# yinjunbo/IS-Fusion

Measured on AMD Instinct MI355X. Metric: nuScenes frames/sec forward (0.075 voxel), LiDAR branch voxelize+spconv->BEV, higher is better.
Workload: dtype f32 (f16x3 split-precision MFMA, fp32 accumulate); 1 GPU; BASELINE configs[1]: isfusion_0075voxel LiDAR-only branch (dynamic voxelize + DynamicVFE + 21-layer SparseEncoder -> BEV [B,512,180,180]), synthetic nuScenes-shaped 300000-pt sweeps, batch=4/GPU, random-init weights, eval BN, fp32; points_per_frame=300000, batch_per_gpu=4, parallelism=dp1, collectives=none (1 rank)

## Files before the change

include/isf_hip.h:

```cpp
#ifndef ISF_HIP_H
#define ISF_HIP_H

#include <stddef.h>
#include <stdint.h>

#ifdef __cplusplus
extern "C" {
#endif

#define ISF_OK 0
#define ISF_ERR_ARG (-1)
#define ISF_ERR_HIP (-2)
#define ISF_ERR_NOMEM (-3)
#define ISF_ERR_UNSUPPORTED (-4)
#define ISF_ERR_CAPACITY (-5)

#define ISF_REDUCE_SUM 0
#define ISF_REDUCE_MEAN 1
#define ISF_REDUCE_MAX 2

#define ISF_CONV_SUBM 0
#define ISF_CONV_SPARSE 1

typedef void* isf_stream_t;
// ... 162 lines not shown
int isf_sparse_conv_forward_dma_lines(const void* features_split, int num_in, int c_in, const void* packed16, int num_taps,
                                      int taps_per_line, int c_out, const int32_t* lines, const uint32_t* mask,
                                      int nbr_stride, int num_out, const float* scale, const float* shift,
                                      const void* residual_split, int relu, void* out_split, int mode,
                                      isf_stream_t stream);
typedef struct isf_conv_cu_plan {
  const int32_t* group_masks;
  const int32_t* units;
  const int32_t* num_units;
  int max_units;
  int num_out;
  int variant;
  int cap;
} isf_conv_cu_plan;
int isf_sparse_conv_cu_plan_ints(int num_out, size_t* num_ints);
int isf_sparse_conv_cu_plan(const int32_t* nbr, int nbr_stride, int num_taps, int num_out, int32_t* plan_buf,
                            isf_conv_cu_plan* plan, isf_stream_t stream);
int isf_sparse_conv_forward_cu(const void* features_split, int num_in, int c_in, const void* packed16, int num_taps,
                               int c_out, const int32_t* nbr, int nbr_stride, int num_out, const float* scale,
                               const float* shift, const void* residual_split, int relu, void* out_split,
                               const isf_conv_cu_plan* plan, isf_stream_t stream);
int isf_sparse_conv_cu_plan_host(const int32_t* work, int num_groups, int cus, int32_t* units, int max_units,
                                 int* num_units);
int isf_sparse_conv_cu_max_units(int num_groups, int cus);
int isf_stage_unit_rows(void);
int isf_stage_unit_cap(void);
int isf_rulebook_stage_tables(const int32_t* nbr, int nbr_stride, int num_taps, uint16_t* slots, int32_t* ulist,
                              int32_t* ucount, isf_stream_t stream);
int isf_sparse_conv_forward_staged(const void* features_split, int num_in, int c_in, const void* packed16,
                                   int num_taps, int c_out, const uint16_t* slots, int nbr_stride,
                                   const int32_t* ulist, const int32_t* ucount, int num_out, const float* scale,
                                   const float* shift, const void* residual_split, int relu, void* out_split,
                                   int stage_rows, int mode, isf_stream_t stream);
int isf_sparse_to_dense_bev(const float* features, const int32_t* indices, int num_rows, int channels,
                            int batch_size, int D, int H, int W, float* out, isf_stream_t stream);

typedef struct isf_conv_layer {
  int conv_type;
  int ksize[3], stride[3], padding[3];
  int c_in, c_out;
  const float* packed;
  const void* packed16;
  const float* scale;
  const float* shift;
  int relu;
  int residual_from;
} isf_conv_layer;

typedef struct isf_encoder_stats {
  int num_layers;
  int num_in[32], num_out[32];
  long long pairs[32];
  float ms[32];
  int precision;
} isf_encoder_stats;

#define ISF_ENC_DIAG_NO_GATHER 2
#define ISF_ENC_DIAG_NO_WEIGHTS 4
#define ISF_ENC_DIAG_NO_LOOP 8
#define ISF_ENC_DIAG_NO_SHARING 16
#define ISF_ENC_DIAG_UNIFORM_TILES 32
#define ISF_ENC_DIAG_LAUNCH_ORDER 64
#define ISF_ENC_DIAG_NARROW_GATHER 128
#define ISF_ENC_DIAG_VFE_FP32_ROWS 256
#define ISF_ENC_DIAG_CU_KERNEL 512
#define ISF_ENC_DIAG_CU_VARIANT_SHIFT 10
#define ISF_ENC_DIAG_CU_VARIANT_MASK 15360
#define ISF_ENC_DIAG_DENSE_TABLES 16384
#define ISF_ENC_DIAG_TILE_TABLES 32768
#define ISF_ENC_DIAG_VOXELIZE_PER_FRAME 65536
#define ISF_ENC_DIAG_COUNTS_MEMCPY 131072
#define ISF_ENC_DIAG_ONE_BLOCK_4W 262144
#define ISF_ENC_DIAG_ONE_BLOCK_8W 524288
#define ISF_ENC_DIAG_STAGGER 1048576
#define ISF_ENC_DIAG_R4_ISSUE 2097152
#define ISF_ENC_DIAG_TWO_AHEAD 4194304
#define ISF_ENC_DIAG_DEEP 8388608
#define ISF_ENC_DIAG_BAND_ORDER 16777216
#define ISF_ENC_DIAG_NO_ROW_SORT 33554432
#define ISF_ENC_DIAG_NARROW_ROW_SORT 67108864
#define ISF_ENC_DIAG_SORT_KEY_AB 134217728
#define ISF_ENC_DIAG_NARROW_TILES 268435456
#define ISF_ENC_DIAG_CHUNK_SPLIT 536870912
typedef struct isf_encoder_options {
  int precision;
  int diagnostic;
  int stage_rows;
  int stage_mask;
  int bev_format;
} isf_encoder_options;

int isf_sparse_encoder_forward(const float* voxel_features, const int32_t* coors, int num_voxels,
                               int batch_size, const int sparse_shape_host[3],
                               const isf_conv_layer* layers_host, int num_layers,
                               float* spatial_features,
                               int out_shape_host[4],
                               isf_encoder_stats* stats_host , int time_layers,
                               const isf_encoder_options* options , isf_stream_t stream);

typedef struct isf_vfe_params {
  int in_channels, c1, c2;
  const float *w1, *scale1, *shift1, *w2, *scale2, *shift2;
  float voxel_size[3], coors_range[6];
} isf_vfe_params;

int isf_lidar_branch_forward(const float* points, const int64_t* point_offsets_host, int batch_size,
                             const isf_vfe_params* vfe_host, const int sparse_shape_host[3],
                             const isf_conv_layer* layers_host, int num_layers,
                             float* spatial_features, int out_shape_host[4],
                             isf_encoder_stats* stats_host, int time_layers,
                             const isf_encoder_options* options , isf_stream_t stream);


size_t isf_packed_linear_bytes(int out_features, int in_features);
int isf_pack_linear(const float* weight, int out_features, int in_features, void* packed, isf_stream_t stream);
int isf_pack_linear_transposed(const float* weight_t, int out_features, int in_features, void* packed, isf_stream_t stream);
int isf_linear_forward(const float* x, int num_rows, int in_features, int ldx, const void* packed_weight,
                       int out_features, const float* bias, const float* row_table, const int32_t* row_table_index,
                       int activation, const float* residual, const float* ln_gamma, const float* ln_beta,
                       float ln_eps, float* y, int ldy, int x_hw, int residual_hw, int y_hw, isf_stream_t stream);

size_t isf_packed_window_block_bytes(int embed_dims);
int isf_pack_window_block(const float* in_proj_weight, const float* out_proj_weight, int embed_dims, int num_heads,
                          void* packed, isf_stream_t stream);
int isf_window_block_forward(const float* x, int batch_size, int grid_size, int embed_dims, int num_heads, int window,
                             int shift, const void* packed, const float* in_proj_bias, const float* pos_table,
                             const float* out_proj_bias, const float* ln_gamma, const float* ln_beta, float ln_eps,
                             float* y, isf_stream_t stream);

int isf_window_attention_forward(const float* qkv, int batch_size, int grid_size, int embed_dims, int num_heads,
                                 int window, int shift, float* out, isf_stream_t stream);

int isf_attention_forward(const float* q, int ldq, const float* k, const float* v, int ldkv, int batch_size,
                          int num_queries, int num_keys, int embed_dims, int num_heads, float* out, int ldo,
                          isf_stream_t stream);
int isf_attention_forward_dropout(const float* q, int ldq, const float* k, const float* v, int ldkv, int batch_size,
                                  int num_queries, int num_keys, int embed_dims, int num_heads, float dropout_p,
                                  unsigned long long seed, float* out, int ldo, isf_stream_t stream);

int isf_channel_attention_forward(const float* query_scene, const float* query_ins, int num_maps, int size,
                                  float* out, isf_stream_t stream);

int isf_p2g_forward(const float* pillars, int pillar_ld, int slots, const int32_t* pillar_coors, int num_pillars,
                    const float* img_nhwc, int batch_size, int num_cam, int feat_h, int feat_w, int channels,
                    const float* cam_params, int input_h, int input_w, int bev_size, float* out,
                    isf_stream_t stream);
int isf_p2g_forward_split(const float* pillars, int pillar_ld, int slots, const int32_t* pillar_coors, int num_pillars,
                          const float* img_nhwc, int batch_size, int num_cam, int feat_h, int feat_w, int channels,
                          const float* cam_params, int input_h, int input_w, int bev_size, void* out_split,
                          isf_stream_t stream);

int isf_instance_topk(const float* heatmap, int batch_size, int num_classes, int height, int width, int k,
                      unsigned pool1_class_mask, int32_t* top_index, int32_t* top_index_raw, float* masked_heatmap,
                      isf_stream_t stream);

int isf_ms_deform_attn_forward(const float* value, const int64_t* spatial_shapes, const int64_t* level_start_index,
                               const float* sampling_loc, const float* attn_weight, int batch_size, int num_keys,
                               int num_heads, int head_dim, int num_queries, int num_levels, int num_points,
                               float* out, isf_stream_t stream);

int isf_ms_deform_attn_backward(const float* value, const int64_t* spatial_shapes, const int64_t* level_start_index,
                                const float* sampling_loc, const float* attn_weight, const float* grad_output,
                                int batch_size, int num_keys, int num_heads, int head_dim, int num_queries,
                                int num_levels, int num_points, float* grad_value, float* grad_sampling_loc,
                                float* grad_attn_weight, isf_stream_t stream);

int isf_ingroup_indices(const int64_t* group_inds, int num, int64_t* out_inds, isf_stream_t stream);

int isf_msda_forward(const float* value, const float* sampling_offsets, const float* attention_logits,
                     const float* reference_points, int batch_size, int num_queries, int num_heads, int head_dim,
                     int num_points, int height, int width, float* out, isf_stream_t stream);

int isf_decode_boxes(const float* heatmap, const float* query_score, const int64_t* query_labels, const float* center,
                     const float* height, const float* dim, const float* rot, const float* vel, int batch_size,
                     int num_classes, int num_proposals, int ld, const float* coder, float* boxes, float* scores,
                     int32_t* labels, int32_t* counts, isf_stream_t stream);

int isf_head_query_init(const int32_t* top_index, const int32_t* top_raw, int batch_size, int num_proposals, int hw,
                        int embed, int num_classes, const float* feat_tok, const int64_t* tok_of_cell,
                        const float* class_table, const float* qpe_table, const float* bev_pos, const float* masked,
                        float* query, float* qpe, float* x, float* query_pos, int64_t* top_index64,
                        int64_t* query_labels, float* query_score, isf_stream_t stream);
int isf_head_scatter_predictions(int num_heads, const float* const* src, const int* src_ld, const int* col0,
                                 const int* channels, float* const* dst, int center_head, const float* query_pos,
                                 float* query_pos_next, int batch_size, int num_proposals, isf_stream_t stream);

int isf_instance_gather(const int32_t* top, int batch_size, int num_instances, int bev_size, int embed,
                        const float* scene, const float* qpe_table, int64_t* top64, int64_t* cell64, float* tokens,
                        float* qpe, float* tokens_pos, float* query_pos, float* ref, isf_stream_t stream);

int isf_transpose_rulebook(const int32_t* nbr, int nbr_stride, int num_out, int num_taps, int num_in,
                           int32_t* nbr_t, int nbr_t_stride, isf_stream_t stream);
int isf_sparse_conv_backward_input(const float* grad_out, int num_out, int c_out, const float* filters, int num_taps,
                                   int c_in, const int32_t* nbr_t, int nbr_t_stride, int num_in, float* grad_in,
// ... 231 lines not shown
```

is-fusion_amd/_lib.py:

```python
import ctypes
import os

_HERE = os.path.dirname(os.path.abspath(__file__))
LIB_PATH = os.path.join(_HERE, "libisf_hip.so")

c_int = ctypes.c_int
c_void_p = ctypes.c_void_p
c_float_p = ctypes.POINTER(ctypes.c_float)
c_int_p = ctypes.POINTER(ctypes.c_int)

ISF_OK = 0
REDUCE = {"sum": 0, "mean": 1, "max": 2}
CONV_SUBM, CONV_SPARSE = 0, 1


class ConvLayer(ctypes.Structure):
    _fields_ = [
        ("conv_type", c_int),
        ("ksize", c_int * 3), ("stride", c_int * 3), ("padding", c_int * 3),
        ("c_in", c_int), ("c_out", c_int),
        ("packed", c_void_p), ("packed16", c_void_p), ("scale", c_void_p), ("shift", c_void_p),
        ("relu", c_int), ("residual_from", c_int),
    ]

# ... 28 lines not shown
    _fields_ = [
        ("in_channels", c_int), ("c1", c_int), ("c2", c_int),
        ("w1", c_void_p), ("scale1", c_void_p), ("shift1", c_void_p),
        ("w2", c_void_p), ("scale2", c_void_p), ("shift2", c_void_p),
        ("voxel_size", ctypes.c_float * 3), ("coors_range", ctypes.c_float * 6),
    ]


class Sweep(ctypes.Structure):
    _fields_ = [
        ("first_point", ctypes.c_int64), ("num_points", ctypes.c_int32), ("sample", ctypes.c_int32),
        ("is_sweep", ctypes.c_int32), ("remove_close", ctypes.c_int32), ("close_radius", ctypes.c_float),
        ("time_lag", ctypes.c_float), ("rotation", ctypes.c_double * 9), ("translation", ctypes.c_double * 3),
    ]


class PointAug(ctypes.Structure):
    _fields_ = [
        ("enabled", ctypes.c_int32), ("rot_mat_T", ctypes.c_float * 9), ("translation", ctypes.c_float * 3),
        ("scale", ctypes.c_float), ("flip_horizontal", ctypes.c_int32), ("flip_vertical", ctypes.c_int32),
    ]


class ImageView(ctypes.Structure):
    _fields_ = [
        ("src_offset", ctypes.c_int64), ("src_w", ctypes.c_int32), ("src_h", ctypes.c_int32),
        ("resize_w", ctypes.c_int32), ("resize_h", ctypes.c_int32), ("crop_x", ctypes.c_int32),
        ("crop_y", ctypes.c_int32), ("flip", ctypes.c_int32), ("rotate", ctypes.c_int32), ("rot", ctypes.c_int32 * 6),
        ("h_bounds", ctypes.c_int32), ("h_coeffs", ctypes.c_int32), ("h_ksize", ctypes.c_int32),
        ("v_bounds", ctypes.c_int32), ("v_coeffs", ctypes.c_int32), ("v_ksize", ctypes.c_int32),
    ]


class PasteView(ctypes.Structure):
    _fields_ = [
        ("src_offset", ctypes.c_int64), ("width", ctypes.c_int32), ("height", ctypes.c_int32),
        ("op_begin", ctypes.c_int32), ("op_end", ctypes.c_int32), ("box_x0", ctypes.c_int32),
        ("box_y0", ctypes.c_int32), ("box_x1", ctypes.c_int32), ("box_y1", ctypes.c_int32),
    ]


class PasteOp(ctypes.Structure):
    _fields_ = [
        ("patch_offset", ctypes.c_int64), ("kind", ctypes.c_int32), ("x0", ctypes.c_int32), ("y0", ctypes.c_int32),
        ("x1", ctypes.c_int32), ("y1", ctypes.c_int32), ("mask_x0", ctypes.c_int32), ("mask_y0", ctypes.c_int32),
        ("mask_x1", ctypes.c_int32), ("mask_y1", ctypes.c_int32), ("patch_pitch", ctypes.c_int32),
    ]


SWEEP_PASTED = 2
PASTE_MIX, PASTE_PATCH = 0, 1
PASTE_MAX_BOXES, PASTE_MAX_OPS = 64, 256


class SwinA(ctypes.Structure):
    _fields_ = [("x", c_void_p), ("x2", c_void_p), ("ln_stats", c_void_p), ("ln_gamma", c_void_p), ("ln_beta", c_void_p),
                ("mode", c_int), ("ldx", c_int), ("n", c_int), ("c", c_int), ("h", c_int), ("w", c_int),
                ("c2", c_int), ("h2", c_int), ("w2", c_int)]


SWIN_A_ROWS, SWIN_A_PATCH, SWIN_A_MERGE, SWIN_A_UPCAT = 0, 1, 2, 3


class AdamWHp(ctypes.Structure):
    _fields_ = [("decay", ctypes.c_float), ("w1", ctypes.c_float), ("b2", ctypes.c_float), ("w2", ctypes.c_float),
                ("eps", ctypes.c_float), ("neg_step_size", ctypes.c_float), ("bc2_sqrt", ctypes.c_float),
                ("pad", ctypes.c_float)]


OPTIM_CHUNK, OPTIM_MAX_HP_ARGS = 32768, 16
OPTIM_NO_CLIP, OPTIM_CLIP, OPTIM_SCALE_GRADS = 0, 1, 2

CONV_MODE_F16, CONV_MODE_NO_GATHER, CONV_MODE_NO_WEIGHTS, CONV_MODE_NO_LOOP, CONV_MODE_NO_SHARING = 1, 2, 4, 8, 16
CONV_MODE_UNIFORM_TILES, CONV_MODE_F16_ROWS, CONV_MODE_F16_STORAGE, CONV_MODE_DMA_PLAN = 32, 256, 257, 2048
CONV_MODE_ONE_BLOCK_4W, CONV_MODE_ONE_BLOCK_8W, CONV_MODE_DEEP, CONV_MODE_STAGGER = 4096, 8192, 32768, 65536
CONV_MODE_R4_ISSUE, CONV_MODE_TWO_AHEAD, CONV_MODE_CHUNK_SPLIT = 131072, 262144, 524288
ENC_DIAG_NO_GATHER, ENC_DIAG_NO_WEIGHTS, ENC_DIAG_NO_LOOP, ENC_DIAG_NO_SHARING, ENC_DIAG_UNIFORM_TILES = 2, 4, 8, 16, 32
ENC_DIAG_LAUNCH_ORDER, ENC_DIAG_NARROW_GATHER, ENC_DIAG_VFE_FP32_ROWS, ENC_DIAG_CU_KERNEL = 64, 128, 256, 512
ENC_DIAG_CU_VARIANT_SHIFT, ENC_DIAG_CU_VARIANT_MASK = 10, 15 << 10
ENC_DIAG_DENSE_TABLES, ENC_DIAG_TILE_TABLES, ENC_DIAG_VOXELIZE_PER_FRAME, ENC_DIAG_COUNTS_MEMCPY = 16384, 32768, 65536, 131072
ENC_DIAG_ONE_BLOCK_4W, ENC_DIAG_ONE_BLOCK_8W, ENC_DIAG_STAGGER, ENC_DIAG_R4_ISSUE = 262144, 524288, 1048576, 2097152
ENC_DIAG_TWO_AHEAD, ENC_DIAG_DEEP, ENC_DIAG_BAND_ORDER, ENC_DIAG_NO_ROW_SORT = 4194304, 8388608, 16777216, 33554432
ENC_DIAG_NARROW_ROW_SORT, ENC_DIAG_SORT_KEY_AB, ENC_DIAG_NARROW_TILES, ENC_DIAG_CHUNK_SPLIT = 67108864, 134217728, 268435456, 536870912
WGRAD_F16, WGRAD_FULL_TAPS = 1, 2


_F3 = ctypes.c_float * 3
_F6 = ctypes.c_float * 6
_I3 = c_int * 3
_I4 = c_int * 4
SIGNATURES = {
    "isf_version": (c_int, []),
    "isf_last_error": (ctypes.c_char_p, []),
    "isf_device_count": (c_int, [c_int_p]),
    "isf_release_workspace": (c_int, []),
    "isf_workspace_bytes": (c_int, [ctypes.POINTER(ctypes.c_size_t)]),
    "isf_debug_workspace_blocks": (c_int, [ctypes.POINTER(ctypes.c_ulonglong), c_int, c_int_p]),
    "isf_dynamic_voxelize": (c_int, [c_void_p, c_int, c_int, _F3, _F6, c_void_p, c_void_p]),
    "isf_dynamic_voxelize_batched": (c_int, [c_void_p, ctypes.POINTER(ctypes.c_int64), c_int, c_int, _F3,
                                             _F6, c_void_p, c_void_p]),
    "isf_hard_voxelize": (c_int, [c_void_p, c_int, c_int, _F3, _F6, c_int, c_int, c_void_p, c_void_p,
                                  c_void_p, c_int_p, c_void_p]),
    "isf_hard_voxelize_device": (c_int, [c_void_p, c_int, c_int, _F3, _F6, c_int, c_int, c_void_p, c_void_p,
                                         c_void_p, c_void_p, c_void_p]),
    "isf_hard_voxelize_batched_device": (c_int, [c_void_p, ctypes.POINTER(ctypes.c_int64), c_int, c_int, _F3, _F6, c_int,
                                                 c_int, c_void_p, c_void_p, c_void_p, c_void_p, c_void_p]),
    "isf_dynamic_point_to_voxel_forward": (c_int, [c_void_p, c_void_p, c_int, c_int, c_int, c_void_p,
                                                   c_void_p, c_void_p, c_void_p, c_int_p, c_void_p]),
    "isf_dynamic_point_to_voxel_backward": (c_int, [c_void_p, c_void_p, c_void_p, c_void_p, c_void_p,
                                                    c_void_p, c_int, c_int, c_int, c_int, c_void_p]),
    "isf_dynamic_vfe_forward": (c_int, [c_void_p, c_void_p, c_int, c_int, c_int, _F3, _F6, c_void_p,
                                        c_void_p, c_void_p, c_int, c_void_p, c_void_p, c_void_p, c_int,
                                        c_void_p, c_void_p, c_void_p, c_int_p, c_void_p]),
    "isf_hard_simple_vfe": (c_int, [c_void_p, c_void_p, c_int, c_int, c_int, c_int, c_void_p, c_void_p]),
    "isf_nbr_stride": (c_int, [c_int]),
    "isf_conv_out_shape": (c_int, [_I3, _I3, _I3, _I3, _I3]),
    "isf_build_rulebook": (c_int, [c_void_p, c_int, c_int, _I3, _I3, _I3, _I3, c_int, c_void_p, c_int,
                                   c_void_p, c_int, c_int_p, c_void_p]),
    "isf_rulebook_to_indice_pairs": (c_int, [c_void_p, c_int, c_int, c_int, c_int, c_void_p, c_void_p,
                                             c_void_p]),
    "isf_indice_pairs_to_rulebook": (c_int, [c_void_p, c_void_p, c_int, c_int, c_int, c_void_p, c_int,
                                             c_void_p]),
    "isf_sparse_conv_forward": (c_int, [c_void_p, c_int, c_int, c_void_p, c_int, c_int, c_void_p, c_int,
                                        c_int, c_void_p, c_void_p, c_void_p, c_int, c_void_p, c_void_p]),
    "isf_packed_filter_elems": (ctypes.c_size_t, [c_int, c_int, c_int]),
    "isf_pack_filters": (c_int, [c_void_p, c_int, c_int, c_int, c_void_p, c_void_p]),
    "isf_sparse_conv_forward_packed": (c_int, [c_void_p, c_int, c_int, c_void_p, c_int, c_int, c_void_p,
                                               c_int, c_int, c_void_p, c_void_p, c_void_p, c_int, c_void_p,
                                               c_void_p]),
    "isf_packed_filter16_bytes": (ctypes.c_size_t, [c_int, c_int, c_int]),
    "isf_pack_filters_f16x3": (c_int, [c_void_p, c_int, c_int, c_int, c_void_p, c_void_p]),
    "isf_pack_filters_f16x3_transposed": (c_int, [c_void_p, c_int, c_int, c_int, c_void_p, c_void_p]),
    "isf_f32_to_split": (c_int, [c_void_p, ctypes.c_size_t, c_void_p, c_void_p]),
    "isf_split_to_f32": (c_int, [c_void_p, ctypes.c_size_t, c_void_p, c_void_p]),
    "isf_f32_to_half": (c_int, [c_void_p, ctypes.c_size_t, c_void_p, c_void_p]),
    "isf_half_to_f32": (c_int, [c_void_p, ctypes.c_size_t, c_void_p, c_void_p]),
    "isf_sparse_conv_forward_f16x3": (c_int, [c_void_p, c_int, c_int, c_void_p, c_int, c_int, c_void_p, c_int,
                                              c_int, c_void_p, c_void_p, c_void_p, c_int, c_void_p, c_int, c_void_p]),
    "isf_sparse_conv_tile_order": (c_int, [c_void_p, c_int, c_int, c_int, c_int, c_int, c_int, c_void_p, c_void_p,
                                           ctypes.POINTER(c_int), c_void_p]),
    "isf_sparse_conv_forward_f16x3_ordered": (c_int, [c_void_p, c_int, c_int, c_void_p, c_int, c_int, c_void_p, c_int,
                                                      c_int, c_void_p, c_void_p, c_void_p, c_int, c_void_p, c_int,
                                                      c_void_p, c_void_p]),
    "isf_sparse_conv_forward_dma": (c_int, [c_void_p, c_int, c_int, c_void_p, c_int, c_int, c_void_p, c_int, c_int,
                                            c_void_p, c_void_p, c_void_p, c_int, c_void_p, c_int, c_void_p, c_void_p]),
    "isf_sparse_conv_tile_table": (c_int, [c_void_p, c_int, c_int, c_int, c_int, c_int, c_int, c_void_p, c_void_p,
                                           ctypes.POINTER(c_int), c_void_p]),
    "isf_sparse_conv_forward_f16x3_tiled": (c_int, [c_void_p, c_int, c_int, c_void_p, c_int, c_int, c_void_p, c_int,
                                                    c_int, c_void_p, c_void_p, c_void_p, c_int, c_void_p, c_int,
                                                    c_void_p, c_void_p]),
    "isf_sparse_conv_tile_table_host": (c_int, [c_void_p, c_int, c_int, c_int, c_int, c_int, c_int, c_void_p,
                                                ctypes.POINTER(c_int)]),
    "isf_sparse_conv_trace": (c_int, [c_void_p, c_int, c_int, c_void_p, c_int, c_int, c_void_p, c_int, c_int, c_void_p,
                                      c_void_p, c_void_p, c_int, c_void_p, c_void_p, c_void_p, c_int,
                                      ctypes.POINTER(c_int), c_void_p]),
    "isf_sparse_conv_phase_trace": (c_int, [c_void_p, c_int, c_int, c_void_p, c_int, c_int, c_void_p, c_int, c_int,
                                            c_void_p, c_void_p, c_void_p, c_int, c_void_p, c_void_p, c_void_p,
                                            ctypes.c_size_t, c_int_p, c_int_p, c_int_p, c_void_p]),
    "isf_rulebook_to_lines": (c_int, [c_void_p, c_int, c_int, c_int, c_int, c_void_p, c_void_p, c_void_p, c_void_p]),
    "isf_lines_to_rulebook": (c_int, [c_void_p, c_void_p, c_int, c_int, c_int, c_void_p, c_void_p]),
    "isf_sparse_conv_forward_dma_lines": (c_int, [c_void_p, c_int, c_int, c_void_p, c_int, c_int, c_int, c_void_p, c_void_p,
                                                  c_int, c_int, c_void_p, c_void_p, c_void_p, c_int, c_void_p, c_int,
                                                  c_void_p]),
    "isf_sparse_conv_cu_plan_ints": (c_int, [c_int, ctypes.POINTER(ctypes.c_size_t)]),
    "isf_sparse_conv_cu_plan": (c_int, [c_void_p, c_int, c_int, c_int, c_void_p, ctypes.POINTER(ConvCuPlan), c_void_p]),
    "isf_sparse_conv_forward_cu": (c_int, [c_void_p, c_int, c_int, c_void_p, c_int, c_int, c_void_p, c_int, c_int,
                                           c_void_p, c_void_p, c_void_p, c_int, c_void_p, ctypes.POINTER(ConvCuPlan),
                                           c_void_p]),
    "isf_sparse_conv_cu_plan_host": (c_int, [c_void_p, c_int, c_int, c_void_p, c_int, ctypes.POINTER(c_int)]),
    "isf_sparse_conv_cu_max_units": (c_int, [c_int, c_int]),
    "isf_stage_unit_rows": (c_int, []),
    "isf_stage_unit_cap": (c_int, []),
    "isf_rulebook_stage_tables": (c_int, [c_void_p, c_int, c_int, c_void_p, c_void_p, c_void_p, c_void_p]),
    "isf_sparse_conv_forward_staged": (c_int, [c_void_p, c_int, c_int, c_void_p, c_int, c_int, c_void_p, c_int,
                                               c_void_p, c_void_p, c_int, c_void_p, c_void_p, c_void_p, c_int, c_void_p,
                                               c_int, c_int, c_void_p]),
    "isf_ms_deform_attn_forward": (c_int, [c_void_p, c_void_p, c_void_p, c_void_p, c_void_p, c_int, c_int, c_int, c_int,
                                           c_int, c_int, c_int, c_void_p, c_void_p]),
    "isf_ms_deform_attn_backward": (c_int, [c_void_p, c_void_p, c_void_p, c_void_p, c_void_p, c_void_p, c_int, c_int,
                                            c_int, c_int, c_int, c_int, c_int, c_void_p, c_void_p, c_void_p, c_void_p]),
    "isf_ingroup_indices": (c_int, [c_void_p, c_int, c_void_p, c_void_p]),
    "isf_packed_window_block_bytes": (ctypes.c_size_t, [c_int]),
    "isf_pack_window_block": (c_int, [c_void_p, c_void_p, c_int, c_int, c_void_p, c_void_p]),
    "isf_window_block_forward": (c_int, [c_void_p, c_int, c_int, c_int, c_int, c_int, c_int, c_void_p, c_void_p,
                                         c_void_p, c_void_p, c_void_p, c_void_p, ctypes.c_float, c_void_p, c_void_p]),
    "isf_p2g_backward": (c_int, [c_void_p, c_int, c_int, c_void_p, c_int, c_int, c_int, c_int, c_int, c_int, c_void_p,
                                 c_int, c_int, c_int, c_void_p, c_void_p, c_void_p]),
    "isf_sparse_to_dense_bev": (c_int, [c_void_p, c_void_p, c_int, c_int, c_int, c_int, c_int, c_int,
                                        c_void_p, c_void_p]),
    "isf_sparse_encoder_forward": (c_int, [c_void_p, c_void_p, c_int, c_int, _I3,
                                           ctypes.POINTER(ConvLayer), c_int, c_void_p, _I4,
                                           ctypes.POINTER(EncoderStats), c_int, ctypes.POINTER(EncoderOptions),
                                           c_void_p]),
    "isf_lidar_branch_forward": (c_int, [c_void_p, ctypes.POINTER(ctypes.c_int64), c_int,
                                         ctypes.POINTER(VfeParams), _I3, ctypes.POINTER(ConvLayer), c_int,
                                         c_void_p, _I4, ctypes.POINTER(EncoderStats), c_int,
                                         ctypes.POINTER(EncoderOptions), c_void_p]),
    "isf_packed_linear_bytes": (ctypes.c_size_t, [c_int, c_int]),
    "isf_pack_linear": (c_int, [c_void_p, c_int, c_int, c_void_p, c_void_p]),
    "isf_pack_linear_transposed": (c_int, [c_void_p, c_int, c_int, c_void_p, c_void_p]),
    "isf_linear_forward": (c_int, [c_void_p, c_int, c_int, c_int, c_void_p, c_int, c_void_p, c_void_p, c_void_p,
                                   c_int, c_void_p, c_void_p, c_void_p, ctypes.c_float, c_void_p, c_int, c_int, c_int,
                                   c_int, c_void_p]),
    "isf_window_attention_forward": (c_int, [c_void_p, c_int, c_int, c_int, c_int, c_int, c_int, c_void_p,
                                             c_void_p]),
    "isf_attention_forward": (c_int, [c_void_p, c_int, c_void_p, c_void_p, c_int, c_int, c_int, c_int, c_int,
                                      c_int, c_void_p, c_int, c_void_p]),
    "isf_attention_forward_dropout": (c_int, [c_void_p, c_int, c_void_p, c_void_p, c_int, c_int, c_int, c_int, c_int,
                                              c_int, ctypes.c_float, ctypes.c_uint64, c_void_p, c_int, c_void_p]),
    "isf_channel_attention_forward": (c_int, [c_void_p, c_void_p, c_int, c_int, c_void_p, c_void_p]),
    "isf_p2g_forward": (c_int, [c_void_p, c_int, c_int, c_void_p, c_int, c_void_p, c_int, c_int, c_int, c_int,
                                c_int, c_void_p, c_int, c_int, c_int, c_void_p, c_void_p]),
    "isf_p2g_forward_split": (c_int, [c_void_p, c_int, c_int, c_void_p, c_int, c_void_p, c_int, c_int, c_int, c_int,
                                      c_int, c_void_p, c_int, c_int, c_int, c_void_p, c_void_p]),
    "isf_instance_topk": (c_int, [c_void_p, c_int, c_int, c_int, c_int, c_int, ctypes.c_uint, c_void_p, c_void_p,
                                  c_void_p, c_void_p]),
    "isf_msda_forward": (c_int, [c_void_p, c_void_p, c_void_p, c_void_p, c_int, c_int, c_int, c_int, c_int,
                                 c_int, c_int, c_void_p, c_void_p]),
    "isf_decode_boxes": (c_int, [c_void_p] * 8 + [c_int, c_int, c_int, c_int, ctypes.POINTER(ctypes.c_float)]
                         + [c_void_p] * 5),
    "isf_sparse_conv_dma_trace": (c_int, [c_void_p, c_int, c_int, c_void_p, c_int, c_int, c_int, c_void_p, c_void_p, c_int,
                                         c_int, c_void_p, c_void_p, c_void_p, c_int, c_void_p, c_void_p, c_int,
                                         ctypes.POINTER(c_int), c_void_p]),
    "isf_sparse_conv_dma_trace_parts": (c_int, [c_void_p, c_int, c_int, c_void_p, c_int, c_int, c_int, c_void_p, c_void_p,
                                               c_int, c_int, c_void_p, c_void_p, c_void_p, c_int, c_void_p, c_void_p,
                                               c_void_p, c_int, ctypes.POINTER(c_int), c_void_p]),
    "isf_sparse_conv_part_table": (c_int, [c_void_p, c_void_p, c_int, c_int, c_int, c_int, c_int, c_int, c_int, c_void_p,
                                           c_int, c_void_p, c_int, c_int * 4, c_void_p]),
    "isf_sparse_conv_forward_parts": (c_int, [c_void_p, c_int, c_int, c_void_p, c_int, c_int, c_int, c_void_p, c_void_p,
                                              c_int, c_int, c_void_p, c_void_p, c_void_p, c_int, c_void_p, c_int, c_void_p,
                                              c_void_p]),
    "isf_instance_gather": (c_int, [c_void_p, c_int, c_int, c_int, c_int] + [c_void_p] * 10),
    "isf_head_query_init": (c_int, [c_void_p, c_void_p, c_int, c_int, c_int, c_int, c_int] + [c_void_p] * 14),
    "isf_head_scatter_predictions": (c_int, [c_int, ctypes.POINTER(c_void_p), ctypes.POINTER(c_int),
                                            ctypes.POINTER(c_int), ctypes.POINTER(c_int), ctypes.POINTER(c_void_p),
                                            c_int, c_void_p, c_void_p, c_int, c_int, c_void_p]),
    "isf_assemble_points": (c_int, [c_void_p, ctypes.POINTER(Sweep), c_int, c_int, ctypes.POINTER(PointAug),
                                    ctypes.POINTER(ctypes.c_float), c_void_p, c_void_p,
                                    ctypes.POINTER(ctypes.c_int32), c_void_p]),
    "isf_image_prepass": (c_int, [c_void_p, c_void_p, c_int, c_void_p, c_void_p, c_int, c_int, c_void_p, c_void_p]),
    "isf_assemble_points_paste": (c_int, [c_void_p, ctypes.POINTER(Sweep), c_int, c_int, ctypes.POINTER(PointAug),
                                          ctypes.POINTER(ctypes.c_float), ctypes.POINTER(ctypes.c_float),
                                          ctypes.POINTER(ctypes.c_int32), c_void_p, c_void_p,
                                          ctypes.POINTER(ctypes.c_int32), c_void_p]),
    "isf_image_paste": (c_int, [c_void_p, c_void_p, c_int, c_void_p, c_int, c_int, c_int, ctypes.c_double,
                                ctypes.c_double, ctypes.c_float, c_void_p]),
    "isf_transpose_rulebook": (c_int, [c_void_p, c_int, c_int, c_int, c_int, c_void_p, c_int, c_void_p]),
    "isf_sparse_conv_backward_input": (c_int, [c_void_p, c_int, c_int, c_void_p, c_int, c_int, c_void_p, c_int, c_int,
                                               c_void_p, c_void_p]),
    "isf_sparse_conv_backward_filter": (c_int, [c_void_p, c_int, c_int, c_void_p, c_int, c_int, c_void_p, c_int,
                                                c_int, c_void_p, c_void_p]),
    "isf_bn1d_stats": (c_int, [c_void_p, c_int, c_int, c_void_p, c_void_p]),
    "isf_bn1d_apply": (c_int, [c_void_p, c_int, c_int, c_void_p, ctypes.c_float, c_void_p, c_void_p, ctypes.c_float,
                               ctypes.c_float, c_int, c_void_p, c_void_p, c_void_p, c_int, c_void_p, c_void_p, c_void_p]),
    "isf_bn1d_stats_pivot": (c_int, [c_void_p, c_int, c_int, c_void_p, c_void_p, c_void_p]),
    "isf_bn1d_apply_pivot": (c_int, [c_void_p, c_int, c_int, c_void_p, c_void_p, ctypes.c_float, c_void_p, c_void_p,
                                     ctypes.c_float, ctypes.c_float, c_int, c_void_p, c_void_p, c_void_p, c_int, c_void_p,
                                     c_void_p, c_void_p]),
    "isf_bn1d_apply_pivot_counted": (c_int, [c_void_p, c_int, c_int, c_void_p, c_void_p, ctypes.c_float, c_void_p, c_void_p,
                                             ctypes.c_float, ctypes.c_float, c_int, c_void_p, c_void_p, c_void_p, c_void_p,
                                             c_int, c_void_p, c_void_p, c_void_p]),
    "isf_bn1d_backward_sums": (c_int, [c_void_p, c_void_p, c_void_p, c_int, c_int, c_void_p, c_void_p, c_void_p]),
    "isf_bn1d_backward_apply": (c_int, [c_void_p, c_void_p, c_void_p, c_int, c_int, c_void_p, c_void_p, c_void_p,
                                        ctypes.c_float, c_void_p, c_void_p, c_void_p, c_void_p, c_void_p]),
    "isf_pair_list_capacity": (c_int, [c_int, c_int]),
    "isf_rulebook_pair_lists": (c_int, [c_void_p, c_int, c_int, c_int, c_int, c_void_p, c_void_p, c_void_p]),
    "isf_grad_to_split": (c_int, [c_void_p, ctypes.c_size_t, c_void_p, c_void_p, c_void_p]),
    "isf_grad_rescale": (c_int, [c_void_p, ctypes.c_size_t, c_void_p, c_void_p, c_void_p]),
    "isf_split_to_f32_scaled": (c_int, [c_void_p, ctypes.c_size_t, c_void_p, c_void_p, c_void_p]),
    "isf_sparse_conv_backward_filter_f16x3": (c_int, [c_void_p, c_int, c_int, c_void_p, c_int, c_int, c_void_p, c_void_p,
                                                      c_int, c_int, c_void_p, c_void_p, c_int, c_void_p]),
    "isf_msda_backward": (c_int, [c_void_p] * 5 + [c_int] * 7 + [c_void_p] * 4),
    "isf_attention_backward": (c_int, [c_void_p, c_int, c_void_p, c_void_p, c_int, c_void_p, c_void_p, c_int, c_int,
                                       c_int, c_int, c_int, c_int, c_void_p, c_int, c_void_p, c_void_p, c_int,
                                       c_void_p]),
    "isf_attention_backward_dropout": (c_int, [c_void_p, c_int, c_void_p, c_void_p, c_int, c_void_p, c_void_p, c_int, c_int,
                                               c_int, c_int, c_int, c_int, ctypes.c_float, ctypes.c_uint64, c_void_p, c_int,
                                               c_void_p, c_void_p, c_int, c_void_p]),
    "isf_window_attention_backward": (c_int, [c_void_p, c_void_p, c_int, c_int, c_int, c_int, c_int, c_int, c_void_p,
                                              c_void_p]),
# ... 121 lines not shown
```

is-fusion_amd/csrc/isf_common.h:

```cpp
#pragma once
#include <hip/hip_runtime.h>
#include <stdint.h>
#include <stdio.h>
#include <stdarg.h>
#include <string.h>
#include <vector>

#include "isf_hip.h"

namespace isf {

void set_error(const char* fmt, ...);

#define ISF_HIP_TRY(expr)                                                                   \
  do {                                                                                      \
    hipError_t _e = (expr);                                                                 \
    if (_e != hipSuccess) {                                                                 \
      ::isf::set_error("%s:%d: %s -> %s", __FILE__, __LINE__, #expr, hipGetErrorString(_e)); \
      return ISF_ERR_HIP;                                                                   \
    }                                                                                       \
  } while (0)

#define ISF_REQUIRE(cond, code, ...)  \
  do {                                \
    if (!(cond)) {                    \
      ::isf::set_error(__VA_ARGS__);  \
      return (code);                  \
    }                                 \
  } while (0)

#define ISF_TRY(expr)          \
  do {                         \
    int _r = (expr);           \
    if (_r != ISF_OK) return _r; \
  } while (0)

#define ISF_LAUNCH_CHECK() ISF_HIP_TRY(hipGetLastError())

struct ByteMaps {
  unsigned char* fine = nullptr;
  unsigned char* coarse = nullptr;
  size_t words = 0;
};

class Arena {
 public:
  int reset();
  int alloc(void** out, size_t bytes);
  template <typename T>
  int alloc_n(T** out, size_t n) { return alloc(reinterpret_cast<void**>(out), n * sizeof(T)); }
  int release();
  size_t capacity() const;
  int list_blocks(unsigned long long* base_cap, int max_pairs, int* num_pairs) const;
  hipStream_t side = nullptr;
  std::vector<hipEvent_t> events;
  size_t next_event = 0;
  ByteMaps bytemaps;
  int* mailbox_host = nullptr;
  int* mailbox_dev = nullptr;
  unsigned mailbox_seq = 0;
  int* zero_pool = nullptr;
  float* ks_scratch = nullptr;
  size_t ks_scratch_bytes = 0;
  unsigned* ks_count = nullptr;
  int ks_count_cap = 0;
 private:
  struct Block { char* base; size_t cap; size_t off; };
  std::vector<Block> blocks_;
};

Arena& arena_for_stream(hipStream_t st);

static inline hipStream_t as_stream(isf_stream_t s) { return reinterpret_cast<hipStream_t>(s); }
static inline int ceil_div(long long a, long long b) { return (int)((a + b - 1) / b); }
static inline size_t round_up(size_t a, size_t b) { return (a + b - 1) / b * b; }

struct OccIndex {
  int B, D, H, W;
  unsigned long long ncells;
  size_t nwords;
  unsigned long long* bits;
  uint32_t* prefix;
  int* total;
};

int occ_create(Arena& a, OccIndex* occ, int B, int D, int H, int W, hipStream_t st, bool zero = true);
size_t occ_bits_bytes(const OccIndex& occ);
int occ_mark_coords4_bytemap(Arena& a, const OccIndex& occ, const int32_t* coors4, int n, hipStream_t st);
int scan_u32_exclusive(Arena& a, const uint32_t* in, uint32_t* out, size_t n, hipStream_t st);
int occ_scan(Arena& a, const OccIndex& occ, hipStream_t st);
int occ_mark_coords4(const OccIndex& occ, const int32_t* coors4, int n, hipStream_t st);
int occ_compact_coords4(const OccIndex& occ, int32_t* out, hipStream_t st);
int fill_many(hipStream_t st, int n, void* const* ptrs, const size_t* bytes, const unsigned char* byte_values);
int read_int(const int* dev, int* host, hipStream_t st);
int post_int(Arena& a, const int* dev, hipStream_t st, unsigned* ticket);
int wait_int(Arena& a, unsigned ticket, hipStream_t st, int* value);
int side_stream(Arena& a, hipStream_t* out);
static constexpr int kZeroInts = 256;
int zero_ints(Arena& a, int** out);
int ksplit_buffers(Arena& a, size_t scratch_bytes, int counters, float** scratch, unsigned** count, hipStream_t st);
int stream_wait_stream(Arena& a, hipStream_t waiter, hipStream_t producer);
int pooled_event(Arena& a, hipEvent_t* out);

__device__ __forceinline__ int occ_lookup(const unsigned long long* __restrict__ bits,
                                          const uint32_t* __restrict__ prefix,
                                          unsigned long long cell) {
  const size_t w = (size_t)(cell >> 6);
  const unsigned long long word = bits[w];
  const unsigned long long bit = 1ull << (cell & 63);
  if (!(word & bit)) return -1;
  return (int)(prefix[w] + (uint32_t)__popcll(word & (bit - 1)));
}

struct AttnDrop {
  unsigned long long seed;
  unsigned thresh;
  float inv_keep;
};
__host__ __device__ inline bool attn_keep(unsigned long long seed, unsigned bh, unsigned i, unsigned j, unsigned thresh) {
  unsigned long long x = seed ^ (((unsigned long long)bh << 48) | ((unsigned long long)(i & 0xffffffu) << 24) |
                                 (unsigned long long)(j & 0xffffffu));
  x ^= x >> 33;
  x *= 0xff51afd7ed558ccdULL;
  x ^= x >> 33;
  x *= 0xc4ceb9fe1a85ec53ULL;
  x ^= x >> 33;
  return (unsigned)(x >> 32) >= thresh;
}
static inline AttnDrop attn_drop_of(float p, unsigned long long seed) {
  AttnDrop d{seed, 0u, 1.f};
  if (p > 0.f) {
    const double t = (double)p * 4294967296.0;
    d.thresh = t >= 4294967295.0 ? 4294967295u : (unsigned)t;
    d.inv_keep = 1.f / (1.f - p);
  }
  return d;
}

__host__ __device__ inline size_t split_hi_index(size_t row, int c_units, int u) {
  return (row * (size_t)c_units + (size_t)(u & ~3)) * 2 + (size_t)(u & 3);
}

__device__ __forceinline__ bool voxel_of_point(const float* __restrict__ p, float vx, float vy, float vz,
                                               float x0, float y0, float z0, int gx, int gy, int gz,
                                               int& cx, int& cy, int& cz) {
  const float fx = floorf(__fdiv_rn(__fsub_rn(p[0], x0), vx));
  const float fy = floorf(__fdiv_rn(__fsub_rn(p[1], y0), vy));
  const float fz = floorf(__fdiv_rn(__fsub_rn(p[2], z0), vz));
  if (!(fx >= 0.f && fx < (float)gx && fy >= 0.f && fy < (float)gy && fz >= 0.f && fz < (float)gz))
    return false;
  cx = (int)fx; cy = (int)fy; cz = (int)fz;
  return true;
}

struct VoxGeom {
  float vx, vy, vz, x0, y0, z0;
  int gx, gy, gz;
};

static inline VoxGeom make_geom(const float vs[3], const float range[6]) {
  VoxGeom g;
  g.vx = vs[0]; g.vy = vs[1]; g.vz = vs[2];
  g.x0 = range[0]; g.y0 = range[1]; g.z0 = range[2];
  g.gx = (int)roundf((range[3] - range[0]) / vs[0]);
  g.gy = (int)roundf((range[4] - range[1]) / vs[1]);
  g.gz = (int)roundf((range[5] - range[2]) / vs[2]);
  return g;
}


static constexpr int kVoxMaxBatch = 8;
struct VoxBatch {
  long long off[kVoxMaxBatch + 1];
  int B;
};
int occ_voxelize_mark_bytemap(Arena& a, const OccIndex& occ, const float* points, int P, int C, const VoxGeom& g,
                              const VoxBatch& vb, int32_t* coors4, hipStream_t st);

int dynamic_voxelize_impl(const float* points, int P, int C, const float vs[3], const float range[6],
                          int32_t* coors, int coors_stride, int coors_col0, int batch_idx,
                          hipStream_t st);
int dynamic_vfe_impl(Arena& a, const float* points, const int32_t* coors4, int P, int Cin, int B,
                     const float vs[3], const float range[6], const float* w1, const float* scale1,
                     const float* shift1, int c1, const float* w2, const float* scale2,
                     const float* shift2, int c2, float* voxel_feats, int32_t* voxel_coors,
                     int32_t* pt2vox, int* num_voxels_host, OccIndex* occ_out, int grid_d_alloc,
                     hipStream_t st, hipEvent_t* coords_ready = nullptr,
                     void* voxel_feats_split = nullptr ,
                     const VoxBatch* voxelize = nullptr );
int build_perm(Arena& a, const OccIndex& occ, const int32_t* coors4, int n, int32_t** perm_out,
               hipStream_t st);
int launch_nbr(Arena& a, const int32_t* out_coors4, int n_out, const int in_shape[3], const int ks[3],
               const int st[3], const int pd[3], bool subm, const OccIndex& in_occ, const int32_t* perm,
               int32_t* nbr, int nbr_stride, unsigned long long* pair_count, hipStream_t st_);
int launch_nbr_lines(Arena& a, const int32_t* out_coors4, int n_out, const int in_shape[3], const int ks[3],
                     const int st[3], const int pd[3], bool subm, const OccIndex& in_occ, int32_t* lines, uint32_t* mask,
                     int stride, unsigned long long* pair_count, hipStream_t st_);
int launch_mark_out(const int32_t* in_coors4, int n_in, const int in_shape[3], const int ks[3],
                    const int st[3], const int pd[3], const OccIndex& out_occ, hipStream_t st_);
bool sparse_conv_mfma_supported(int c_in, int c_out);
int pack_filters_impl(const float* w, int K, int cin, int cout, float* packed, hipStream_t st);
int sparse_conv_forward_packed_impl(const float* x, int n_in, int c_in, const float* packed, int K,
                                    int c_out, const int32_t* nbr, int nbr_stride, int n_out,
                                    const float* scale, const float* shift, const float* residual,
                                    int relu, float* y, hipStream_t st);
int sparse_conv_forward_generic_impl(const float* x, int c_in, const float* w, int K, int c_out,
                                     const int32_t* nbr, int nbr_stride, int n_out, const float* scale,
                                     const float* shift, const float* residual, int relu, float* y,
                                     hipStream_t st);
bool sparse_conv_f16x3_supported(int c_in, int c_out);
int sparse_conv_forward_f16x3_impl(const void* xs, int c_in, const void* packed16, int K, int c_out,
                                   const int32_t* nbr, int nbr_stride, int n_out, const float* scale,
                                   const float* shift, const void* residual, int relu, void* ys,
                                   int mode , hipStream_t st,
                                   const int32_t* order = nullptr, struct Conv16LaunchInfo* query = nullptr,
                                   const int32_t* rowmap = nullptr );
struct Conv16LaunchInfo {
  int full, half, part_rows;
  int TM, ncb, wgs_per_cu, cus_per_xcd;
};
static inline int conv16_order_parts(const Conv16LaunchInfo& i) { return i.ncb == 2 ? 4 : 8; }
static inline int conv16_order_tiles(const Conv16LaunchInfo& i) { return i.full + i.half; }
static inline bool conv16_order_applies(const Conv16LaunchInfo& i) {
  const int t = i.full + i.half;
  return t > i.cus_per_xcd && t <= i.wgs_per_cu * i.cus_per_xcd && t <= 255 && i.cus_per_xcd <= 64;
}
static inline bool conv16_table_applies(const Conv16LaunchInfo& i) {
  return i.TM > 0 && i.cus_per_xcd > 0 && i.part_rows / 16 <= i.cus_per_xcd * i.wgs_per_cu * (i.TM / 16);
}
static inline int conv16_table_ints(const Conv16LaunchInfo& i) {
  return conv16_order_parts(i) * 2 * i.wgs_per_cu * i.cus_per_xcd;
}
int conv16_tile_table_impl(const int32_t* group_work, int n_out, const Conv16LaunchInfo& info, int32_t* table,
                           hipStream_t st);
int conv_group_masks_impl(const int32_t* nbr, int nbr_stride, int K, int n_out, int32_t* masks, int32_t* work,
                          hipStream_t st);
bool sparse_conv_dma_supported(int c_in, int c_out);
int sparse_conv_forward_dma_impl(const void* xs, int c_in, const void* packed16, int K, int c_out, const int32_t* nbr,
                                 int nbr_stride, int n_out, const float* scale, const float* shift,
                                 const void* residual, int relu, void* ys, int mode, hipStream_t st,
                                 const int32_t* order = nullptr, Conv16LaunchInfo* query = nullptr,
                                 const uint32_t* lmask = nullptr , int nx = 0,
                                 const int32_t* rowmap = nullptr ,
                                 long long* trace = nullptr );
int conv16_tile_order_impl(const int32_t* nbr, int nbr_stride, int K, int n_out, const Conv16LaunchInfo& info,
                           int32_t* work , int32_t* order ,
                           hipStream_t st, const uint32_t* lmask = nullptr );
bool conv16_parts_apply(const Conv16LaunchInfo& info, bool several_rounds = false);
int conv16_part_table_impl(const int32_t* nbr, const uint32_t* lmask, int nbr_stride, int K, int n_out, int c_in, int c_out,
                           const Conv16LaunchInfo& info, bool raster, int32_t* work, int32_t* table, hipStream_t st,
                           bool equal_rows = false );
int stable_sort_u32_impl(Arena& a, const uint32_t* keys, int n, int key_bits, int* idx_sorted, hipStream_t st);
int conv_row_sort_impl(Arena& a, const int32_t* nbr, int nbr_stride, int K, int n_out, int part_rows, int32_t* rowmap,
                       int32_t* nbr_sorted, hipStream_t st,
                       int key_mode = 1 );
int conv_row_sort_lines_impl(Arena& a, const int32_t* lines, const uint32_t* lmask, int nbr_stride, int num_lines, int n_out,
                             int part_rows, bool full_key, int32_t* rowmap, int32_t* lines_sorted, uint32_t* lmask_sorted,
                             hipStream_t st);
bool conv16_band_order_applies(const Conv16LaunchInfo& info);
int conv16_band_order_impl(const int32_t* coors4, int n_out, const Conv16LaunchInfo& info, int band, int32_t* order ,
                           hipStream_t st);
bool sparse_conv_deep_supported(int c_in, int c_out);
int sparse_conv_forward_deep_impl(bool balance, bool table, const uint4* xs, int c_in, const uint4* wpk, const float* winv,
                                  int K, int c_out, const int32_t* nbr, int nbr_stride, int n_out, const float* scale,
                                  const float* shift, const uint4* residual, int relu, uint4* ys, hipStream_t st,
                                  const int32_t* order, Conv16LaunchInfo* query);
struct ConvCuPlan {
  const int32_t* group_masks = nullptr;
  const int2* units = nullptr;
  const int32_t* num_units = nullptr;
  int max_units = 0;
  int n_out = 0;
  int variant = 0;
  int cap = 16;
};
int conv_cu_variant_cap(int variant);
bool sparse_conv_cu_supported(int c_in, int c_out);
size_t conv_cu_plan_ints(int n_out);
int conv_cu_plan_impl(const int32_t* nbr, int nbr_stride, int K, int n_out, int32_t* buf ,
                      ConvCuPlan* plan, hipStream_t st, int cap = 16);
int sparse_conv_forward_cu_impl(const void* xs, int c_in, const void* packed16, int K, int c_out, const int32_t* nbr,
                                int nbr_stride, int n_out, const float* scale, const float* shift, const void* residual,
                                int relu, void* ys, const ConvCuPlan& plan, hipStream_t st);
int stage_tables_impl(const int32_t* nbr, int nbr_stride, int K, uint16_t* slots, int32_t* ulist, int32_t* ucount,
                      hipStream_t st);
int sparse_conv_forward_staged_impl(const void* xs, int c_in, const void* packed16, int K, int c_out,
                                    const uint16_t* slots, int nbr_stride, const int32_t* ulist,
                                    const int32_t* ucount, int n_out, const float* scale, const float* shift,
                                    const void* residual, int relu, void* ys, int stage_rows, int mode,
                                    hipStream_t st);
int pack_filters16_impl(Arena& a, const float* w, int K, int cin, int cout, void* packed16, hipStream_t st,
                        bool transposed = false );
int f32_to_split_impl(const float* x, size_t n_elems, void* xs, hipStream_t st);
int split_to_f32_impl(const void* xs, size_t n_elems, float* x, hipStream_t st);
int f32_to_half_impl(const float* x, size_t n_elems, void* xh, hipStream_t st);
int half_to_f32_impl(const void* xh, size_t n_elems, float* x, hipStream_t st);
int sparse_to_dense_bev_impl(Arena& a, const void* feats, int fmt, const int32_t* indices, int n, int C,
                             int B, int D, int H, int W, float* out, const OccIndex* occ,
                             hipStream_t st);

}
```

is-fusion_amd/csrc/isf_encoder.hip:

```cpp
#include "isf_common.h"
#include "isf_spconv16.h"

#include <algorithm>

namespace isf {

static constexpr int kDenseX = 64;

template <int FMT>
__global__ __launch_bounds__(256) void dense_bev_kernel(const void* __restrict__ feats_v, int C, int D,
                                                        int H, int W,
                                                        const unsigned long long* __restrict__ bits,
                                                        const uint32_t* __restrict__ prefix,
                                                        const int32_t* __restrict__ perm,
                                                        float* __restrict__ out) {
  __shared__ float tile[64][kDenseX + 1];
  __shared__ int rows[kDenseX];
  const int xt = blockIdx.x, y = blockIdx.y, b = blockIdx.z;
  const int x0 = xt * kDenseX;
  const int t = threadIdx.x;
  for (int z = 0; z < D; ++z) {
    __syncthreads();
    if (t < kDenseX) {
      int r = -1;
      const int x = x0 + t;
      if (x < W) {
        r = occ_lookup(bits, prefix, (((unsigned long long)b * D + z) * H + y) * W + x);
        if (r >= 0 && perm) r = perm[r];
      }
      rows[t] = r;
    }
    __syncthreads();
    for (int c0 = 0; c0 < C; c0 += 64) {
      if (FMT != 0) {
        const uint4* fs = reinterpret_cast<const uint4*>(feats_v);
        const int u = t & 7;
#pragma unroll
        for (int j = 0; j < 2; ++j) {
          const int xx = (t >> 3) + 32 * j;
          const int r = rows[xx];
          float v[8] = {0.f, 0.f, 0.f, 0.f, 0.f, 0.f, 0.f, 0.f};
          if (r >= 0 && c0 + u * 8 < C) {
            const size_t o = FMT == 2 ? (size_t)r * (C >> 3) + (c0 >> 3) + u : split_hi_index((size_t)r, C >> 3, (c0 >> 3) + u);
            const uint4 hi = fs[o], lo = FMT == 2 ? make_uint4(0, 0, 0, 0) : fs[o + 4];
            const _Float16* h = reinterpret_cast<const _Float16*>(&hi);
            const _Float16* l = reinterpret_cast<const _Float16*>(&lo);
#pragma unroll
            for (int q = 0; q < 8; ++q) v[q] = (float)h[q] + (float)l[q];
          }
#pragma unroll
          for (int q = 0; q < 8; ++q) tile[u * 8 + q][xx] = v[q];
        }
      } else {
        const float* feats = reinterpret_cast<const float*>(feats_v);
        const int c4 = (t & 15) * 4;
#pragma unroll
        for (int j = 0; j < 4; ++j) {
          const int xx = (t >> 4) + 16 * j;
          const int r = rows[xx];
          float4 v = make_float4(0.f, 0.f, 0.f, 0.f);
          if (r >= 0 && c0 + c4 < C) v = *reinterpret_cast<const float4*>(feats + (size_t)r * C + c0 + c4);
          tile[c4 + 0][xx] = v.x;
          tile[c4 + 1][xx] = v.y;
          tile[c4 + 2][xx] = v.z;
          tile[c4 + 3][xx] = v.w;
        }
      }
      __syncthreads();
      const int lane = t & 63, wv = t >> 6;
      if (x0 + lane < W) {
        for (int cc = wv; cc < 64 && c0 + cc < C; cc += 4) {
          const size_t ch = (size_t)(c0 + cc) * D + z;
          out[(((size_t)b * C * D + ch) * H + y) * W + x0 + lane] = tile[cc][lane];
        }
      }
      __syncthreads();
    }
  }
}

int sparse_to_dense_bev_impl(Arena& a, const void* feats, int fmt, const int32_t* indices, int n, int C,
                             int B, int D, int H, int W, float* out, const OccIndex* occ_in, hipStream_t st) {
  ISF_REQUIRE(C % (fmt ? 32 : 4) == 0, ISF_ERR_UNSUPPORTED, "dense: channels %d not a multiple of %d", C,
              fmt ? 32 : 4);
  OccIndex occ;
  const int32_t* perm = nullptr;
  if (occ_in) {
    occ = *occ_in;
  } else {
    ISF_TRY(occ_create(a, &occ, B, D, H, W, st));
    ISF_TRY(occ_mark_coords4(occ, indices, n, st));
    ISF_TRY(occ_scan(a, occ, st));
    int32_t* p = nullptr;
    ISF_TRY(build_perm(a, occ, indices, n, &p, st));
    perm = p;
  }
  dim3 grid(ceil_div(W, kDenseX), H, B);
  if (fmt == 1)
    hipLaunchKernelGGL(dense_bev_kernel<1>, grid, dim3(256), 0, st, feats, C, D, H, W, occ.bits, occ.prefix,
                       perm, out);
  else if (fmt == 2)
    hipLaunchKernelGGL(dense_bev_kernel<2>, grid, dim3(256), 0, st, feats, C, D, H, W, occ.bits, occ.prefix,
                       perm, out);
  else
    hipLaunchKernelGGL(dense_bev_kernel<0>, grid, dim3(256), 0, st, feats, C, D, H, W, occ.bits, occ.prefix,
                       perm, out);
  ISF_LAUNCH_CHECK();
  return ISF_OK;
}

__global__ __launch_bounds__(256) void bev_split_kernel(const uint4* __restrict__ fs, int C, int D, int H, int W,
                                                        const unsigned long long* __restrict__ bits,
                                                        const uint32_t* __restrict__ prefix, long long ntok,
                                                        uint4* __restrict__ out) {
  const int upt = C * D / 8;
  const long long t = (long long)blockIdx.x * 256 + threadIdx.x;
  if (t >= ntok * upt) return;
  const long long tok = t / upt;
  const int j = (int)(t - tok * upt);
  const int hw = H * W;
  const int b = (int)(tok / hw), pos = (int)(tok - (long long)b * hw);
  const int y = pos / W, x = pos - y * W;
  _Float16 hi[8], lo[8];
  if (D == 2) {
    const int r0 = occ_lookup(bits, prefix, (((unsigned long long)b * 2 + 0) * H + y) * W + x);
    const int r1 = occ_lookup(bits, prefix, (((unsigned long long)b * 2 + 1) * H + y) * W + x);
    uint2 h0 = make_uint2(0, 0), l0 = h0, h1 = h0, l1 = h0;
    const int uc = j >> 1, e = j & 1;
    if (r0 >= 0) {
      const uint2* p = reinterpret_cast<const uint2*>(fs + split_hi_index((size_t)r0, C >> 3, uc));
      h0 = p[e];
      l0 = p[8 + e];
    }
    if (r1 >= 0) {
      const uint2* p = reinterpret_cast<const uint2*>(fs + split_hi_index((size_t)r1, C >> 3, uc));
      h1 = p[e];
      l1 = p[8 + e];
    }
    const _Float16 *a0 = reinterpret_cast<const _Float16*>(&h0), *a1 = reinterpret_cast<const _Float16*>(&h1);
    const _Float16 *b0 = reinterpret_cast<const _Float16*>(&l0), *b1 = reinterpret_cast<const _Float16*>(&l1);
#pragma unroll
    for (int q = 0; q < 4; ++q) {
      hi[2 * q] = a0[q]; hi[2 * q + 1] = a1[q];
      lo[2 * q] = b0[q]; lo[2 * q + 1] = b1[q];
    }
  } else {
    for (int q = 0; q < 8; ++q) {
      const int ch = 8 * j + q, c = ch / D, z = ch - c * D;
      const int r = occ_lookup(bits, prefix, (((unsigned long long)b * D + z) * H + y) * W + x);
      hi[q] = lo[q] = (_Float16)0.f;
      if (r >= 0) {
        const _Float16* p = reinterpret_cast<const _Float16*>(fs + split_hi_index((size_t)r, C >> 3, c >> 3));
        hi[q] = p[c & 7];
        lo[q] = p[32 + (c & 7)];
      }
    }
  }
  const int g = j >> 5, ju = j & 31;
  uint4* o = out + (size_t)g * ntok * 64 + split_hi_index((size_t)tok, 32, ju);
  o[0] = *reinterpret_cast<const uint4*>(hi);
  o[4] = *reinterpret_cast<const uint4*>(lo);
}

int sparse_to_bev_split_impl(const void* feats_split, int C, int B, int D, int H, int W, const OccIndex& occ, void* out,
                             hipStream_t st) {
  ISF_REQUIRE(C % 32 == 0 && (C * D) % 256 == 0, ISF_ERR_UNSUPPORTED,
              "bev (split token matrices): %d x %d channels are not whole 256-channel groups", C, D);
  const long long ntok = (long long)B * H * W, total = ntok * (C * D / 8);
  hipLaunchKernelGGL(bev_split_kernel, dim3(ceil_div(total, 256)), dim3(256), 0, st, reinterpret_cast<const uint4*>(feats_split),
                     C, D, H, W, occ.bits, occ.prefix, ntok, reinterpret_cast<uint4*>(out));
  ISF_LAUNCH_CHECK();
  return ISF_OK;
}

__global__ void check_rank_order_kernel(const int32_t* __restrict__ coors4, int n, int B, int D, int H, int W,
                                        const unsigned long long* __restrict__ bits,
                                        const uint32_t* __restrict__ prefix, int* __restrict__ flag) {
  const int i = blockIdx.x * blockDim.x + threadIdx.x;
  if (i >= n) return;
  const int4 c = reinterpret_cast<const int4*>(coors4)[i];
  int r = -1;
// ... 69 lines not shown
      ISF_TRY(a.alloc_n(&work, (size_t)2 * T));
      ISF_TRY(a.alloc_n(&table, (size_t)conv16_part_table_ints(parts, conv16_parts_cap(T, parts))));
      ISF_TRY(conv16_part_table_impl(nbr, lmask, stride, K, n_out, ly.c_in, ly.c_out, info, !order_ok, work, table, sg,
                                     (mode & ISF_CONV_MODE_UNIFORM_TILES) != 0));
      *order = table;
      *kind = kOrderParts;
      return ISF_OK;
    }
  }
  if (!order_ok) return ISF_OK;
  if (dma)
    ISF_TRY(sparse_conv_forward_dma_impl(nullptr, ly.c_in, ly.packed16, K, ly.c_out, nbr, stride, n_out, nullptr,
                                         nullptr, nullptr, 0, nullptr, mode, sg, nullptr, &info));
  else
    ISF_TRY(sparse_conv_forward_f16x3_impl(nullptr, ly.c_in, ly.packed16, K, ly.c_out, nbr, stride, n_out, nullptr,
                                           nullptr, nullptr, 0, nullptr, mode, sg, nullptr, &info));
  if (!dma && kind && tables && !lmask && conv16_table_applies(info) && n_out >= 16 * info.cus_per_xcd) {
    const int ng = ceil_div(n_out, 16);
    int32_t *masks = nullptr, *work = nullptr, *table = nullptr;
    ISF_TRY(a.alloc_n(&masks, (size_t)ng));
    ISF_TRY(a.alloc_n(&work, (size_t)ng));
    ISF_TRY(a.alloc_n(&table, (size_t)conv16_table_ints(info)));
    ISF_TRY(conv_group_masks_impl(nbr, stride, K, n_out, masks, work, sg));
    ISF_TRY(conv16_tile_table_impl(work, n_out, info, table, sg));
    *order = table;
    *kind = kOrderTable;
    return ISF_OK;
  }
  if (!conv16_order_applies(info)) {
    if (band > 0 && coors_out && conv16_band_order_applies(info)) {
      int32_t* ord = nullptr;
      ISF_TRY(a.alloc_n(&ord, (size_t)conv16_order_parts(info) * conv16_order_tiles(info)));
      ISF_TRY(conv16_band_order_impl(coors_out, n_out, info, band, ord, sg));
      *order = ord;
    }
    return ISF_OK;
  }
  const size_t n = (size_t)conv16_order_parts(info) * conv16_order_tiles(info);
  int32_t *work = nullptr, *ord = nullptr;
  ISF_TRY(a.alloc_n(&work, n));
  ISF_TRY(a.alloc_n(&ord, n));
  ISF_TRY(conv16_tile_order_impl(nbr, stride, K, n_out, info, work, ord, sg, lmask));
  *order = ord;
  return ISF_OK;
}

static int build_stage_tables(Arena& a, const int32_t* nbr, int stride, int K, StageTables* t, hipStream_t sg) {
  const int units = stride / isf_stage_unit_rows();
  ISF_TRY(a.alloc_n(&t->slots, (size_t)K * stride));
  ISF_TRY(a.alloc_n(&t->ulist, (size_t)units * isf_stage_unit_cap()));
  ISF_TRY(a.alloc_n(&t->ucount, (size_t)units));
  return stage_tables_impl(nbr, stride, K, t->slots, t->ulist, t->ucount, sg);
}

static int default_stage_rows(const isf_conv_layer& ly) {
  (void)ly;
  return 0;
}

static int ensure_occ(Arena& a, LevelState& L, int B, hipStream_t st) {
  if (L.has_occ) return ISF_OK;
  ISF_TRY(occ_create(a, &L.occ, B, L.shape[0], L.shape[1], L.shape[2], st));
  ISF_TRY(occ_mark_coords4(L.occ, L.coors, L.n, st));
  ISF_TRY(occ_scan(a, L.occ, st));
  L.has_occ = true;
  return ISF_OK;
}

static constexpr int kKnockoutBits = ISF_ENC_DIAG_NO_GATHER | ISF_ENC_DIAG_NO_WEIGHTS | ISF_ENC_DIAG_NO_LOOP | ISF_ENC_DIAG_NO_SHARING;
static constexpr int kDeepOptBits = ISF_CONV_MODE_STAGGER | ISF_CONV_MODE_R4_ISSUE | ISF_CONV_MODE_TWO_AHEAD | ISF_CONV_MODE_DEEP | kConvModeNarrowTiles;
static constexpr struct { int diag, mode; } kDiagToConvMode[] = {
    {ISF_ENC_DIAG_NO_GATHER, ISF_CONV_MODE_NO_GATHER},       {ISF_ENC_DIAG_NO_WEIGHTS, ISF_CONV_MODE_NO_WEIGHTS},
    {ISF_ENC_DIAG_NO_LOOP, ISF_CONV_MODE_NO_LOOP},           {ISF_ENC_DIAG_NO_SHARING, ISF_CONV_MODE_NO_SHARING},
    {ISF_ENC_DIAG_UNIFORM_TILES, ISF_CONV_MODE_UNIFORM_TILES}, {ISF_ENC_DIAG_CHUNK_SPLIT, ISF_CONV_MODE_CHUNK_SPLIT},
    {ISF_ENC_DIAG_ONE_BLOCK_4W, ISF_CONV_MODE_ONE_BLOCK_4W}, {ISF_ENC_DIAG_ONE_BLOCK_8W, ISF_CONV_MODE_ONE_BLOCK_8W},
    {ISF_ENC_DIAG_STAGGER, ISF_CONV_MODE_STAGGER},           {ISF_ENC_DIAG_R4_ISSUE, ISF_CONV_MODE_R4_ISSUE},
    {ISF_ENC_DIAG_TWO_AHEAD, ISF_CONV_MODE_TWO_AHEAD},       {ISF_ENC_DIAG_DEEP, ISF_CONV_MODE_DEEP},
    {ISF_ENC_DIAG_NARROW_TILES, kConvModeNarrowTiles}};
static constexpr int kEncDiagKnown =
    kKnockoutBits | ISF_ENC_DIAG_UNIFORM_TILES | ISF_ENC_DIAG_CHUNK_SPLIT | ISF_ENC_DIAG_ONE_BLOCK_4W | ISF_ENC_DIAG_ONE_BLOCK_8W |
    ISF_ENC_DIAG_STAGGER | ISF_ENC_DIAG_R4_ISSUE | ISF_ENC_DIAG_TWO_AHEAD | ISF_ENC_DIAG_DEEP | ISF_ENC_DIAG_NARROW_TILES |
    ISF_ENC_DIAG_LAUNCH_ORDER | ISF_ENC_DIAG_NARROW_GATHER | ISF_ENC_DIAG_CU_KERNEL | ISF_ENC_DIAG_CU_VARIANT_MASK |
    ISF_ENC_DIAG_DENSE_TABLES | ISF_ENC_DIAG_TILE_TABLES | ISF_ENC_DIAG_COUNTS_MEMCPY | ISF_ENC_DIAG_BAND_ORDER | ISF_ENC_DIAG_NO_ROW_SORT |
    ISF_ENC_DIAG_NARROW_ROW_SORT | ISF_ENC_DIAG_SORT_KEY_AB | ISF_ENC_DIAG_VFE_FP32_ROWS | ISF_ENC_DIAG_VOXELIZE_PER_FRAME;

int sparse_encoder_forward_impl(Arena& a, const float* x0, const int32_t* coors0, int n0, int B,
                                const int shape0[3], const OccIndex* occ0, const isf_conv_layer* layers,
                                int num_layers, float* spatial_features, int out_shape[4],
                                isf_encoder_stats* stats, int time_layers, const isf_encoder_options* opt,
                                hipStream_t st, hipEvent_t geometry_ready = nullptr,
                                const void* x0_split = nullptr ) {
  const int precision = opt ? opt->precision : 0, diagnostic = opt ? opt->diagnostic : 0;
  const int dg = diagnostic & kKnockoutBits;
  ISF_REQUIRE(precision >= 0 && precision <= 2 && diagnostic >= 0 && (diagnostic & ~kEncDiagKnown) == 0 &&
                  (dg == 0 || conv_mode_is_knockout(dg) || dg == ISF_ENC_DIAG_NO_SHARING) && !(precision == 2 && dg != 0),
              ISF_ERR_ARG, "sparse_encoder: options (precision %d, diagnostic %d)", precision, diagnostic);
  int translated = 0;
  for (const auto& t : kDiagToConvMode)
    if (diagnostic & t.diag) translated |= t.mode;
  const bool f16io = precision == 2;
  const bool fp32_class = dg == 0 && !f16io;
  const int conv_mode = (f16io ? ISF_CONV_MODE_F16_STORAGE : dg) | (translated & ISF_CONV_MODE_UNIFORM_TILES);
  const int one_block = translated & (ISF_CONV_MODE_ONE_BLOCK_4W | ISF_CONV_MODE_ONE_BLOCK_8W);
  const int deep_opts = translated & kDeepOptBits;
  const bool chunk_split = (translated & ISF_CONV_MODE_CHUNK_SPLIT) && fp32_class && one_block == 0 && deep_opts == 0;
  auto on = [&](int bit) { return (diagnostic & bit) != 0; };
  const bool tile_order = !on(ISF_ENC_DIAG_LAUNCH_ORDER), dma_gather = !on(ISF_ENC_DIAG_NARROW_GATHER);
  const bool line_tables = !on(ISF_ENC_DIAG_DENSE_TABLES), mailbox = !on(ISF_ENC_DIAG_COUNTS_MEMCPY), row_sort = !on(ISF_ENC_DIAG_NO_ROW_SORT);
  const bool tile_tables = on(ISF_ENC_DIAG_TILE_TABLES), band_order = on(ISF_ENC_DIAG_BAND_ORDER);
  const bool narrow_sort = on(ISF_ENC_DIAG_NARROW_ROW_SORT), cu_units = on(ISF_ENC_DIAG_CU_KERNEL);
  const int sort_key = on(ISF_ENC_DIAG_SORT_KEY_AB) ? 2 : 1;
  const int cu_variant = (diagnostic & ISF_ENC_DIAG_CU_VARIANT_MASK) >> ISF_ENC_DIAG_CU_VARIANT_SHIFT;
  auto band_of = [&](const int shape[3]) -> int { return band_order ? std::max(8, shape[1] / 45) : 0; };
  constexpr int sort_min_rows = 4096;
  const int cu_cap = conv_cu_variant_cap(cu_variant);
  const int stage_opt = opt ? opt->stage_rows : 0;
  const unsigned stage_mask = opt ? (unsigned)opt->stage_mask : 0u;
  ISF_REQUIRE(stage_opt >= -1, ISF_ERR_ARG, "sparse_encoder: stage_rows %d", stage_opt);
  ISF_REQUIRE(num_layers > 0 && num_layers <= 32, ISF_ERR_ARG, "sparse_encoder: %d layers (1..32)", num_layers);
  hipStream_t sg = nullptr;
  ISF_TRY(side_stream(a, &sg));
  if (geometry_ready) ISF_HIP_TRY(hipStreamWaitEvent(sg, geometry_ready, 0));
  else ISF_TRY(stream_wait_stream(a, sg, st));
  LevelState L;
  for (int j = 0; j < 3; ++j) L.shape[j] = shape0[j];
  L.n = n0;
  L.coors = coors0;
  L.has_occ = false;
  if (occ0) { L.occ = *occ0; L.has_occ = true; }
  L.cache_nbr = nullptr;
  L.cache_order = nullptr;
  L.cache_order_cin = L.cache_order_cout = 0;
  L.cache_order_kind = kOrderPerm;
  L.cache_cu = ConvCuPlan();
  L.cache_lmask = nullptr;
  L.cache_rowmap = L.cache_nbr_sorted = nullptr;
  L.cache_lmask_sorted = nullptr;
  L.cache_sort_part_rows = 0;
  bool use16 = precision != 1;
  for (int i = 0; i < num_layers; ++i)
    use16 = use16 && layers[i].packed16 && sparse_conv_f16x3_supported(layers[i].c_in, layers[i].c_out);
  const void* outputs[32];
  int out_rows[32];
  const void* x = x0;
  const void* x_in0 = x0;
  ISF_REQUIRE(!x0_split || (use16 && !f16io), ISF_ERR_ARG, "sparse_encoder: split input without the split kernels");
  if (x0_split) {
    x = x0_split;
    x_in0 = x0_split;
  } else if (use16) {
    void* xs0 = nullptr;
    ISF_TRY(a.alloc(&xs0, (size_t)std::max(n0, 1) * layers[0].c_in * 4));
    if (f16io) ISF_TRY(f32_to_half_impl(x0, (size_t)n0 * layers[0].c_in, xs0, st));
    else ISF_TRY(f32_to_split_impl(x0, (size_t)n0 * layers[0].c_in, xs0, st));
    x = xs0;
    x_in0 = xs0;
  }
  unsigned long long* pair_counts = nullptr;
  if (stats) {
    ISF_TRY(a.alloc_n(&pair_counts, 32));
    ISF_HIP_TRY(hipMemsetAsync(pair_counts, 0, 32 * sizeof(unsigned long long), sg));
  }
  std::vector<hipEvent_t> ev;
  if (time_layers && stats) {
    ev.resize((size_t)num_layers * 2);
    for (auto& e : ev) ISF_HIP_TRY(hipEventCreate(&e));
  }
  int c_last = layers[0].c_in;
  for (int i = 0; i < num_layers; ++i) {
    const isf_conv_layer& ly = layers[i];
    const int K = ly.ksize[0] * ly.ksize[1] * ly.ksize[2];
    ISF_REQUIRE(K >= 1 && K <= 27, ISF_ERR_UNSUPPORTED, "sparse_encoder: layer %d has %d taps", i, K);
    ISF_REQUIRE(ly.c_in == c_last, ISF_ERR_ARG, "sparse_encoder: layer %d expects %d channels, got %d", i, ly.c_in, c_last);
    int32_t* nbr = nullptr;
    int stride = 0;
    int n_out = L.n;
    int n_in = L.n;
    int srows = 0;
    if (use16 && dg == 0 && !f16io && stage_opt >= 0 && sparse_conv_f16x3_supported(ly.c_in, ly.c_out))
      srows = stage_opt == 0 ? default_stage_rows(ly)
                             : ((stage_mask == 0 || ((stage_mask >> i) & 1u)) ? stage_opt : 0);
    StageTables stg;
    const int32_t* order = nullptr;
    int order_kind = kOrderPerm;
    const bool cu = use16 && cu_units && srows == 0 && conv_mode == 0 && sparse_conv_cu_supported(ly.c_in, ly.c_out);
    ConvCuPlan cu_plan;
    const bool plan_ok = use16 && srows == 0 && !cu;
    const bool want_tile_order = plan_ok && tile_order;
    const int layer_mode = conv_mode | (fp32_class && ly.c_out >= 128 ? deep_opts : 0) |
                           (chunk_split && use16 && !cu && srows == 0 && ly.c_out == 256 && ly.c_in >= 128 ? ISF_CONV_MODE_CHUNK_SPLIT : 0);
    const bool dma = use16 && dma_gather && srows == 0 && dg == 0 && sparse_conv_dma_supported(ly.c_in, ly.c_out);
    const bool parts_ok = plan_ok && dg == 0 && !((conv_mode & ISF_CONV_MODE_UNIFORM_TILES) && !tile_order) && !band_order && !(dma && narrow_sort) &&
                          (dma || (layer_mode & (ISF_CONV_MODE_DEEP | ISF_CONV_MODE_CHUNK_SPLIT)) == 0);
    const bool want_order = want_tile_order || parts_ok;
    const uint32_t* lmask = nullptr;
    const int nx = ly.ksize[2];
    auto lines_ok = [&](int first) -> bool {
      if (!use16 || !dma_gather || !line_tables || dg != 0 || stage_opt > 0 || (nx != 1 && nx != 3) ||
          ly.ksize[0] * ly.ksize[1] > 9)
        return false;
      for (int j = first; j < num_layers; ++j) {
        const isf_conv_layer& q = layers[j];
        if (q.conv_type != ISF_CONV_SUBM) break;
        if (q.ksize[0] != ly.ksize[0] || q.ksize[1] != ly.ksize[1] || q.ksize[2] != ly.ksize[2]) continue;
        if (!sparse_conv_dma_supported(q.c_in, q.c_out)) return false;
      }
      return true;
    };
    const bool sort_mode_ok = dg == 0 && one_block == 0 && (deep_opts & ~kConvModeNarrowTiles) == 0;
    const bool sort_ok = row_sort && use16 && !cu && srows == 0 && ly.conv_type == ISF_CONV_SUBM && K == 27 &&
                         sort_mode_ok && L.n >= sort_min_rows && (dma ? narrow_sort : ly.c_out >= 128);
    const int32_t* rowmap = nullptr;
    auto launch_info = [&](const int32_t* table, int tstride, int rows, Conv16LaunchInfo* info) -> int {
      if (dma)
        return sparse_conv_forward_dma_impl(nullptr, ly.c_in, ly.packed16, K, ly.c_out, table, tstride, rows, nullptr, nullptr,
                                            nullptr, 0, nullptr, conv_mode, sg, nullptr, info);
      return sparse_conv_forward_f16x3_impl(nullptr, ly.c_in, ly.packed16, K, ly.c_out, table, tstride, rows, nullptr, nullptr,
                                            nullptr, 0, nullptr, layer_mode, sg, nullptr, info);
    };
    auto ensure_row_sort = [&](const int32_t* table, int tstride, int rows, bool* built) -> int {
      *built = false;
      if (!sort_ok || L.cache_rowmap) return ISF_OK;
      Conv16LaunchInfo info;
      ISF_TRY(launch_info(table, tstride, rows, &info));
// ... 95 lines not shown
          ISF_TRY(build_cu_plan(a, nbr, stride, K, n_out, &L.cache_cu, sg, cu_cap));
          ISF_TRY(stream_wait_stream(a, st, sg));
        }
      }
      cu_plan = L.cache_cu;
      lmask = L.cache_lmask;
      if (sort_applies(nbr, stride, n_out)) {
        nbr = const_cast<int32_t*>(L.cache_nbr_sorted);
        if (lmask) lmask = L.cache_lmask_sorted;
        rowmap = L.cache_rowmap;
      }
      ISF_REQUIRE(!lmask || dma, ISF_ERR_UNSUPPORTED, "sparse_encoder: layer %d cannot read a line-compressed table", i);
      stg = L.cache_stage;
      if (want_order) {
        order = L.cache_order;
        order_kind = L.cache_order_kind;
      }
      if (stats) stats->pairs[i] = hit ? L.cache_pairs : -(long long)i - 1;
    } else {
      ISF_TRY(ensure_occ(a, L, B, sg));
      LevelState Nx;
      ISF_TRY(isf_conv_out_shape(L.shape, ly.ksize, ly.stride, ly.padding, Nx.shape));
      ISF_REQUIRE(Nx.shape[0] > 0 && Nx.shape[1] > 0 && Nx.shape[2] > 0, ISF_ERR_ARG,
                  "sparse_encoder: layer %d output shape empty", i);
      ISF_TRY(occ_create(a, &Nx.occ, B, Nx.shape[0], Nx.shape[1], Nx.shape[2], sg));
      ISF_TRY(launch_mark_out(L.coors, L.n, L.shape, ly.ksize, ly.stride, ly.padding, Nx.occ, sg));
      ISF_TRY(occ_scan(a, Nx.occ, sg));
      if (mailbox) {
        unsigned ticket = 0;
        ISF_TRY(post_int(a, Nx.occ.total, sg, &ticket));
        ISF_TRY(wait_int(a, ticket, sg, &Nx.n));
      } else {
        ISF_TRY(read_int(Nx.occ.total, &Nx.n, sg));
      }
      Nx.has_occ = true;
      int32_t* nc = nullptr;
      ISF_TRY(a.alloc_n(&nc, (size_t)std::max(Nx.n, 1) * 4));
      if (Nx.n > 0) ISF_TRY(occ_compact_coords4(Nx.occ, nc, sg));
      Nx.coors = nc;
      stride = isf_nbr_stride(Nx.n);
      if (dma && lines_ok(num_layers)) {
        uint32_t* lm = nullptr;
        ISF_TRY(a.alloc_n(&nbr, (size_t)ly.ksize[0] * ly.ksize[1] * stride));
        ISF_TRY(a.alloc_n(&lm, (size_t)stride));
        ISF_TRY(launch_nbr_lines(a, Nx.coors, Nx.n, L.shape, ly.ksize, ly.stride, ly.padding, false, L.occ, nbr, lm, stride,
                                 stats ? pair_counts + i : nullptr, sg));
        lmask = lm;
      } else {
        ISF_TRY(a.alloc_n(&nbr, (size_t)K * stride));
        ISF_TRY(launch_nbr(a, Nx.coors, Nx.n, L.shape, ly.ksize, ly.stride, ly.padding, false, L.occ, nullptr, nbr,
                           stride, stats ? pair_counts + i : nullptr, sg));
      }
      if (srows > 0) ISF_TRY(build_stage_tables(a, nbr, stride, K, &stg, sg));
      if (row_sort && use16 && !dma && !cu && srows == 0 && !lmask && ly.c_out >= 128 && K == 27 && sort_mode_ok &&
          Nx.n >= sort_min_rows) {
        Conv16LaunchInfo info;
        ISF_TRY(sparse_conv_forward_f16x3_impl(nullptr, ly.c_in, ly.packed16, K, ly.c_out, nbr, stride, Nx.n, nullptr, nullptr,
                                               nullptr, 0, nullptr, layer_mode, sg, nullptr, &info));
        int32_t *rm = nullptr, *ns = nullptr;
        ISF_TRY(a.alloc_n(&rm, (size_t)stride));
        ISF_TRY(a.alloc_n(&ns, (size_t)K * stride));
        ISF_TRY(conv_row_sort_impl(a, nbr, stride, K, Nx.n, info.part_rows, rm, ns, sg, 1));
        nbr = ns;
        rowmap = rm;
      }
      if (want_order)
        ISF_TRY(build_tile_order(a, ly, K, nbr, stride, Nx.n, layer_mode, dma, &order, sg, lmask, &order_kind, tile_tables,
                                 Nx.coors, band_of(Nx.shape), tile_order, parts_ok));
      if (cu && Nx.n > 0) ISF_TRY(build_cu_plan(a, nbr, stride, K, Nx.n, &cu_plan, sg, cu_cap));
      if (stats) stats->pairs[i] = -(long long)i - 1;
      Nx.cache_cu = ConvCuPlan();
      Nx.cache_lmask = nullptr;
      Nx.cache_rowmap = Nx.cache_nbr_sorted = nullptr;
      Nx.cache_lmask_sorted = nullptr;
      Nx.cache_sort_part_rows = 0;
      Nx.cache_nbr = nullptr;
      Nx.cache_order = nullptr;
      Nx.cache_order_cin = Nx.cache_order_cout = 0;
      Nx.cache_order_kind = kOrderPerm;
      n_out = Nx.n;
      L = Nx;
      ISF_TRY(stream_wait_stream(a, st, sg));
    }
    void* y = nullptr;
    ISF_TRY(a.alloc(&y, (size_t)std::max(n_out, 1) * ly.c_out * 4));
    const void* res = nullptr;
    if (ly.residual_from == -1) res = x_in0;
    else if (ly.residual_from >= 0) {
      ISF_REQUIRE(ly.residual_from < i && out_rows[ly.residual_from] == n_out, ISF_ERR_ARG,
                  "sparse_encoder: layer %d residual source %d incompatible", i, ly.residual_from);
      res = outputs[ly.residual_from];
    }
    if (!ev.empty()) ISF_HIP_TRY(hipEventRecord(ev[2 * i], st));
    if (use16 && srows > 0)
      ISF_TRY(sparse_conv_forward_staged_impl(x, ly.c_in, ly.packed16, K, ly.c_out, stg.slots, stride, stg.ulist,
                                              stg.ucount, n_out, ly.scale, ly.shift, res, ly.relu, y, srows, conv_mode,
                                              st));
    else if (cu && n_out > 0 && ((cu_plan.variant = cu_variant), true))
      ISF_TRY(sparse_conv_forward_cu_impl(x, ly.c_in, ly.packed16, K, ly.c_out, nbr, stride, n_out, ly.scale, ly.shift, res,
                                          ly.relu, y, cu_plan, st));
    else if (dma)
      ISF_TRY(sparse_conv_forward_dma_impl(x, ly.c_in, ly.packed16, K, ly.c_out, nbr, stride, n_out, ly.scale, ly.shift,
                                           res, ly.relu, y, conv_mode | order_mode_bit(order_kind), st, order, nullptr, lmask,
                                           nx, rowmap));
    else if (use16)
      ISF_TRY(sparse_conv_forward_f16x3_impl(x, ly.c_in, ly.packed16, K, ly.c_out, nbr, stride, n_out, ly.scale,
                                             ly.shift, res, ly.relu, y,
                                             layer_mode | order_mode_bit(order_kind) |
                                                 (ly.c_out == 256 && fp32_class ? one_block : 0),
                                             st, order, nullptr, rowmap));
    else if (sparse_conv_mfma_supported(ly.c_in, ly.c_out))
      ISF_TRY(sparse_conv_forward_packed_impl(reinterpret_cast<const float*>(x), n_in, ly.c_in, ly.packed, K,
                                              ly.c_out, nbr, stride, n_out, ly.scale, ly.shift,
                                              reinterpret_cast<const float*>(res), ly.relu,
                                              reinterpret_cast<float*>(y), st));
    else
      ISF_TRY(sparse_conv_forward_generic_impl(reinterpret_cast<const float*>(x), ly.c_in, ly.packed, K, ly.c_out,
                                               nbr, stride, n_out, ly.scale, ly.shift,
                                               reinterpret_cast<const float*>(res), ly.relu,
                                               reinterpret_cast<float*>(y), st));
    if (!ev.empty()) ISF_HIP_TRY(hipEventRecord(ev[2 * i + 1], st));
    outputs[i] = y;
    out_rows[i] = n_out;
    if (stats) { stats->num_in[i] = n_in; stats->num_out[i] = n_out; stats->ms[i] = 0.f; }
    x = y;
    c_last = ly.c_out;
  }
  ISF_TRY(ensure_occ(a, L, B, sg));
  ISF_TRY(stream_wait_stream(a, st, sg));
  if (opt && opt->bev_format == 1) {
    ISF_REQUIRE(use16 && !f16io, ISF_ERR_UNSUPPORTED, "sparse_encoder: bev_format 1 needs the split-precision path");
    ISF_TRY(sparse_to_bev_split_impl(x, c_last, B, L.shape[0], L.shape[1], L.shape[2], L.occ, spatial_features, st));
  } else {
    ISF_REQUIRE(!opt || opt->bev_format == 0, ISF_ERR_ARG, "sparse_encoder: bev_format %d (0 fp32 map, 1 split token matrices)",
                opt->bev_format);
    ISF_TRY(sparse_to_dense_bev_impl(a, x, use16 ? (f16io ? 2 : 1) : 0, L.coors, L.n, c_last, B, L.shape[0], L.shape[1],
                                     L.shape[2], spatial_features, &L.occ, st));
  }
  if (stats) stats->precision = use16 ? 1 : 0;
  if (out_shape) { out_shape[0] = c_last * L.shape[0]; out_shape[1] = L.shape[1]; out_shape[2] = L.shape[2]; out_shape[3] = L.n; }
  if (stats) {
    unsigned long long h_pairs[32];
    ISF_HIP_TRY(hipMemcpyAsync(h_pairs, pair_counts, sizeof(h_pairs), hipMemcpyDeviceToHost, st));
    ISF_HIP_TRY(hipStreamSynchronize(st));
    stats->num_layers = num_layers;
    for (int i = 0; i < num_layers; ++i)
      if (stats->pairs[i] < 0) stats->pairs[i] = (long long)h_pairs[-(stats->pairs[i] + 1)];
    for (int i = 0; i < num_layers && !ev.empty(); ++i)
      ISF_HIP_TRY(hipEventElapsedTime(&stats->ms[i], ev[2 * i], ev[2 * i + 1]));
  }
  for (auto& e : ev) (void)hipEventDestroy(e);
  return ISF_OK;
}

}

extern "C" {

int isf_sparse_to_dense_bev(const float* features, const int32_t* indices, int num_rows, int channels,
                            int batch_size, int D, int H, int W, float* out, isf_stream_t stream) {
  ISF_REQUIRE(num_rows >= 0 && channels > 0 && batch_size > 0 && D > 0 && H > 0 && W > 0 && out, ISF_ERR_ARG,
              "sparse_to_dense_bev: bad arguments");
  ISF_REQUIRE(num_rows == 0 || (features && indices), ISF_ERR_ARG, "sparse_to_dense_bev: null pointer");
  isf::Arena& a = isf::arena_for_stream(isf::as_stream(stream));
  ISF_TRY(a.reset());
  return isf::sparse_to_dense_bev_impl(a, features, 0, indices, num_rows, channels, batch_size, D, H, W, out,
                                       nullptr, isf::as_stream(stream));
}

int isf_sparse_encoder_forward(const float* voxel_features, const int32_t* coors, int num_voxels,
                               int batch_size, const int sparse_shape_host[3],
                               const isf_conv_layer* layers_host, int num_layers, float* spatial_features,
                               int out_shape_host[4], isf_encoder_stats* stats_host, int time_layers,
                               const isf_encoder_options* options, isf_stream_t stream) {
  using namespace isf;
  ISF_REQUIRE(num_voxels > 0 && batch_size > 0 && sparse_shape_host && layers_host && spatial_features &&
                  voxel_features && coors && num_layers > 0,
              ISF_ERR_ARG, "sparse_encoder_forward: bad arguments");
  hipStream_t st = as_stream(stream);
  Arena& a = arena_for_stream(as_stream(stream));
  ISF_TRY(a.reset());
  OccIndex occ0;
  ISF_TRY(occ_create(a, &occ0, batch_size, sparse_shape_host[0], sparse_shape_host[1], sparse_shape_host[2], st));
  ISF_TRY(occ_mark_coords4(occ0, coors, num_voxels, st));
  ISF_TRY(occ_scan(a, occ0, st));
  int* flag = nullptr;
  ISF_TRY(a.alloc_n(&flag, 64));
  ISF_HIP_TRY(hipMemsetAsync(flag, 0, sizeof(int), st));
  hipLaunchKernelGGL(check_rank_order_kernel, dim3(ceil_div(num_voxels, 256)), dim3(256), 0, st, coors,
                     num_voxels, occ0.B, occ0.D, occ0.H, occ0.W, occ0.bits, occ0.prefix, flag);
  ISF_LAUNCH_CHECK();
  int h[2] = {0, 0};
  ISF_HIP_TRY(hipMemcpyAsync(&h[0], flag, sizeof(int), hipMemcpyDeviceToHost, st));
  ISF_HIP_TRY(hipMemcpyAsync(&h[1], occ0.total, sizeof(int), hipMemcpyDeviceToHost, st));
  ISF_HIP_TRY(hipStreamSynchronize(st));
  const float* x = voxel_features;
  const int32_t* c = coors;
  int n = num_voxels;
  if (h[0] != 0 || h[1] != num_voxels) {
    n = h[1];
    ISF_REQUIRE(n > 0, ISF_ERR_ARG, "sparse_encoder_forward: no coordinate inside sparse_shape");
    int32_t* perm = nullptr;
    ISF_TRY(build_perm(a, occ0, coors, num_voxels, &perm, st));
    int32_t* cs = nullptr;
    float* xs = nullptr;
    const int C = layers_host[0].c_in;
    ISF_TRY(a.alloc_n(&cs, (size_t)n * 4));
    ISF_TRY(a.alloc_n(&xs, (size_t)n * C));
    ISF_TRY(occ_compact_coords4(occ0, cs, st));
    hipLaunchKernelGGL(gather_rows_kernel, dim3(ceil_div((long long)n * C, 256)), dim3(256), 0, st,
                       voxel_features, perm, n, C, xs);
    ISF_LAUNCH_CHECK();
    x = xs;
    c = cs;
  }
  return sparse_encoder_forward_impl(a, x, c, n, batch_size, sparse_shape_host, &occ0, layers_host, num_layers,
                                     spatial_features, out_shape_host, stats_host, time_layers, options, st);
}

static bool encoder_takes_split_input(const isf_conv_layer* layers, int num_layers, const isf_encoder_options* opt) {
  if ((opt ? opt->precision : 0) != 0 || num_layers <= 0 || num_layers > 32) return false;
  for (int i = 0; i < num_layers; ++i)
    if (!layers[i].packed16 || !isf::sparse_conv_f16x3_supported(layers[i].c_in, layers[i].c_out)) return false;
  return true;
}

int isf_lidar_branch_forward(const float* points, const int64_t* point_offsets_host, int batch_size,
                             const isf_vfe_params* vfe_host, const int sparse_shape_host[3],
                             const isf_conv_layer* layers_host, int num_layers, float* spatial_features,
                             int out_shape_host[4], isf_encoder_stats* stats_host, int time_layers,
                             const isf_encoder_options* options, isf_stream_t stream) {
  using namespace isf;
  ISF_REQUIRE(points && point_offsets_host && batch_size > 0 && vfe_host && sparse_shape_host && layers_host &&
                  spatial_features,
              ISF_ERR_ARG, "lidar_branch_forward: bad arguments");
  hipStream_t st = as_stream(stream);
  Arena& a = arena_for_stream(as_stream(stream));
  ISF_TRY(a.reset());
  const int64_t P64 = point_offsets_host[batch_size];
  ISF_REQUIRE(P64 > 0 && P64 < (1ll << 31), ISF_ERR_ARG, "lidar_branch_forward: bad point count");
  const int P = (int)P64;
  const int Cin = vfe_host->in_channels;
  int32_t* coors4 = nullptr;
  ISF_TRY(a.alloc_n(&coors4, (size_t)P * 4));
  VoxBatch vb;
  vb.B = batch_size;
  const bool fused_vox = batch_size <= kVoxMaxBatch && !(options && (options->diagnostic & ISF_ENC_DIAG_VOXELIZE_PER_FRAME));
  for (int b = 0; b < batch_size; ++b) {
    const int64_t lo = point_offsets_host[b], hi = point_offsets_host[b + 1];
    ISF_REQUIRE(hi >= lo, ISF_ERR_ARG, "lidar_branch_forward: bad offsets");
    if (fused_vox) {
      vb.off[b] = lo;
      vb.off[b + 1] = hi;
    } else {
      ISF_TRY(dynamic_voxelize_impl(points + lo * Cin, (int)(hi - lo), Cin, vfe_host->voxel_size,
                                    vfe_host->coors_range, coors4 + lo * 4, 4, 1, b, st));
    }
  }
  float* vf = nullptr;
  int32_t* vc = nullptr;
  ISF_TRY(a.alloc_n(&vf, (size_t)P * vfe_host->c2));
  ISF_TRY(a.alloc_n(&vc, (size_t)P * 4));
  int n0 = 0;
  OccIndex occ0;
  hipEvent_t coords_ready = nullptr;
  void* vf_split = nullptr;
  if (encoder_takes_split_input(layers_host, num_layers, options) && vfe_host->c2 == layers_host[0].c_in &&
      !(options && (options->diagnostic & ISF_ENC_DIAG_VFE_FP32_ROWS)))
    ISF_TRY(a.alloc(&vf_split, (size_t)P * vfe_host->c2 * 4));
  ISF_TRY(dynamic_vfe_impl(a, points, coors4, P, Cin, batch_size, vfe_host->voxel_size, vfe_host->coors_range,
                           vfe_host->w1, vfe_host->scale1, vfe_host->shift1, vfe_host->c1, vfe_host->w2,
                           vfe_host->scale2, vfe_host->shift2, vfe_host->c2, vf, vc, nullptr, &n0, &occ0,
                           sparse_shape_host[0], st, &coords_ready, vf_split, fused_vox ? &vb : nullptr));
  ISF_REQUIRE(n0 > 0, ISF_ERR_ARG, "lidar_branch_forward: no point falls inside the voxel grid");
  const bool occ_ok = occ0.D == sparse_shape_host[0] && occ0.H == sparse_shape_host[1] &&
                      occ0.W == sparse_shape_host[2];
  return sparse_encoder_forward_impl(a, vf, vc, n0, batch_size, sparse_shape_host, occ_ok ? &occ0 : nullptr,
                                     layers_host, num_layers, spatial_features, out_shape_host, stats_host,
                                     time_layers, options, st, occ_ok ? coords_ready : nullptr, vf_split);
}

}
```

is-fusion_amd/csrc/isf_runtime.hip:

```cpp
#include <atomic>
#include <thread>

#include "isf_common.h"

#include <map>
#include <memory>
#include <mutex>

namespace isf {

static thread_local char g_err[512] = "";

void set_error(const char* fmt, ...) {
  va_list ap;
  va_start(ap, fmt);
  vsnprintf(g_err, sizeof(g_err), fmt, ap);
  va_end(ap);
}

static const size_t kMinBlock = (size_t)64 << 20;

int Arena::reset() {
  if (blocks_.size() > 1) {
    size_t total = 0;
// ... 239 lines not shown
#pragma unroll
  for (int d = 1; d < 64; d <<= 1) {
    uint32_t t = __shfl_up(inc, d, 64);
    if (lane >= d) inc += t;
  }
  if (lane == 63) lds[wave] = inc;
  __syncthreads();
  uint32_t base = 0, tot = 0;
#pragma unroll
  for (int w = 0; w < kScanThreads / 64; ++w) {
    uint32_t s = lds[w];
    if (w < wave) base += s;
    tot += s;
  }
  __syncthreads();
  *total = tot;
  return base + inc - v;
}

__global__ __launch_bounds__(kScanThreads) void occ_block_count_kernel(
    const unsigned long long* __restrict__ bits, size_t nwords, uint32_t* __restrict__ block_sums) {
  __shared__ uint32_t lds[kScanThreads / 64];
  const size_t w0 = (size_t)blockIdx.x * kWordsPerBlock + (size_t)threadIdx.x * kWordsPerThread;
  uint32_t c = 0;
  if (w0 + kWordsPerThread <= nwords) {
    const ulonglong2* p = reinterpret_cast<const ulonglong2*>(bits + w0);
    ulonglong2 a = p[0], b = p[1];
    c = __popcll(a.x) + __popcll(a.y) + __popcll(b.x) + __popcll(b.y);
  } else {
    for (int i = 0; i < kWordsPerThread; ++i)
      if (w0 + i < nwords) c += __popcll(bits[w0 + i]);
  }
  uint32_t tot;
  (void)block_exclusive_scan(c, lds, &tot);
  if (threadIdx.x == 0) block_sums[blockIdx.x] = tot;
}

__global__ __launch_bounds__(1024) void occ_scan_sums_kernel(uint32_t* __restrict__ block_sums,
                                                             int nblocks, int* __restrict__ total) {
  __shared__ uint32_t lds[1024];
  __shared__ uint32_t carry_s;
  if (threadIdx.x == 0) carry_s = 0;
  __syncthreads();
  for (int base = 0; base < nblocks; base += 1024) {
    const int i = base + threadIdx.x;
    uint32_t v = i < nblocks ? block_sums[i] : 0;
    lds[threadIdx.x] = v;
    __syncthreads();
    for (int d = 1; d < 1024; d <<= 1) {
      uint32_t t = threadIdx.x >= d ? lds[threadIdx.x - d] : 0;
      __syncthreads();
      lds[threadIdx.x] += t;
      __syncthreads();
    }
    const uint32_t carry = carry_s;
    const uint32_t inc = lds[threadIdx.x];
    if (i < nblocks) block_sums[i] = carry + inc - v;
    __syncthreads();
    if (threadIdx.x == 1023) carry_s = carry + inc;
    __syncthreads();
  }
  if (threadIdx.x == 0) *total = (int)carry_s;
}

static constexpr int kLookBehindBlocks = 2048;
__device__ __forceinline__ uint32_t scan_look_behind(const uint32_t* __restrict__ block_sums, uint32_t* lds) {
  uint32_t s = 0;
  for (int i = threadIdx.x; i < (int)blockIdx.x; i += kScanThreads) s += block_sums[i];
#pragma unroll
  for (int d = 32; d >= 1; d >>= 1) s += __shfl_xor(s, d, 64);
  __syncthreads();
  if ((threadIdx.x & 63) == 0) lds[threadIdx.x >> 6] = s;
  __syncthreads();
  uint32_t t = 0;
#pragma unroll
  for (int w = 0; w < kScanThreads / 64; ++w) t += lds[w];
  __syncthreads();
  return t;
}

template <bool SUMS>
__global__ __launch_bounds__(kScanThreads) void occ_write_prefix_kernel(
    const unsigned long long* __restrict__ bits, size_t nwords,
    const uint32_t* __restrict__ block_offsets, uint32_t* __restrict__ prefix, int* __restrict__ total) {
  __shared__ uint32_t lds[kScanThreads / 64];
  const size_t w0 = (size_t)blockIdx.x * kWordsPerBlock + (size_t)threadIdx.x * kWordsPerThread;
  uint32_t pc[kWordsPerThread];
#pragma unroll
  for (int i = 0; i < kWordsPerThread; ++i) pc[i] = (w0 + i < nwords) ? __popcll(bits[w0 + i]) : 0;
  uint32_t c = pc[0] + pc[1] + pc[2] + pc[3];
  uint32_t tot;
  const uint32_t base = SUMS ? scan_look_behind(block_offsets, lds) : block_offsets[blockIdx.x];
  uint32_t ex = block_exclusive_scan(c, lds, &tot) + base;
  if (SUMS && blockIdx.x == gridDim.x - 1 && threadIdx.x == 0) *total = (int)(base + tot);
#pragma unroll
  for (int i = 0; i < kWordsPerThread; ++i) {
    if (w0 + i < nwords) prefix[w0 + i] = ex;
    ex += pc[i];
  }
}

size_t occ_bits_bytes(const OccIndex& occ) {
  return round_up(occ.nwords, kWordsPerBlock) * sizeof(unsigned long long);
}

int occ_create(Arena& a, OccIndex* occ, int B, int D, int H, int W, hipStream_t st, bool zero) {
  occ->B = B; occ->D = D; occ->H = H; occ->W = W;
  occ->ncells = (unsigned long long)B * D * H * W;
  occ->nwords = (size_t)((occ->ncells + 63) / 64);
  const size_t alloc_words = round_up(occ->nwords, kWordsPerBlock);
  ISF_TRY(a.alloc_n(&occ->bits, alloc_words));
  ISF_TRY(a.alloc_n(&occ->prefix, alloc_words));
  ISF_TRY(a.alloc_n(&occ->total, 64));
  if (zero) ISF_HIP_TRY(hipMemsetAsync(occ->bits, 0, alloc_words * sizeof(unsigned long long), st));
  return ISF_OK;
}


__global__ void occ_bytemap_mark_kernel(const int32_t* __restrict__ coors4, int n, int B, int D, int H, int W,
                                        unsigned char* __restrict__ fine, unsigned char* __restrict__ coarse) {
  const int i = blockIdx.x * blockDim.x + threadIdx.x;
  if (i >= n) return;
  const int4 c = reinterpret_cast<const int4*>(coors4)[i];
  if (c.x < 0 || c.y < 0 || c.z < 0 || c.w < 0 || c.x >= B || c.y >= D || c.z >= H || c.w >= W) return;
  const unsigned long long cell = (((unsigned long long)c.x * D + c.y) * H + c.z) * W + c.w;
  fine[cell] = 1;
  coarse[cell >> 6] = 1;
}

__global__ __launch_bounds__(256) void occ_bytemap_pack_kernel(unsigned char* __restrict__ fine,
                                                               unsigned char* __restrict__ coarse,
                                                               size_t nwords_alloc,
                                                               unsigned long long* __restrict__ bits) {
  const size_t w0 = ((size_t)blockIdx.x * blockDim.x + threadIdx.x) * 4;
  if (w0 >= nwords_alloc) return;
  const unsigned int c4 = *reinterpret_cast<const unsigned int*>(coarse + w0);
  unsigned long long out[4] = {0ull, 0ull, 0ull, 0ull};
  if (c4) {
#pragma unroll
    for (int j = 0; j < 4; ++j) {
      if (!((c4 >> (8 * j)) & 0xffu)) continue;
      uint4* f = reinterpret_cast<uint4*>(fine + (w0 + j) * 64);
      unsigned long long m = 0;
#pragma unroll
      for (int q = 0; q < 4; ++q) {
        const uint4 v = f[q];
        const unsigned int d[4] = {v.x, v.y, v.z, v.w};
#pragma unroll
        for (int e = 0; e < 4; ++e)
#pragma unroll
          for (int b = 0; b < 4; ++b)
            if ((d[e] >> (8 * b)) & 0xffu) m |= 1ull << (q * 16 + e * 4 + b);
        f[q] = make_uint4(0, 0, 0, 0);
      }
      out[j] = m;
    }
    *reinterpret_cast<unsigned int*>(coarse + w0) = 0u;
  }
  reinterpret_cast<ulonglong2*>(bits + w0)[0] = make_ulonglong2(out[0], out[1]);
  reinterpret_cast<ulonglong2*>(bits + w0)[1] = make_ulonglong2(out[2], out[3]);
}

__global__ __launch_bounds__(256) void occ_voxelize_mark_kernel(const float* __restrict__ points, int P, int C, VoxGeom g,
                                                                VoxBatch vb, int D, int32_t* __restrict__ coors4,
                                                                unsigned char* __restrict__ fine,
                                                                unsigned char* __restrict__ coarse) {
  const int i = blockIdx.x * blockDim.x + threadIdx.x;
  if (i >= P) return;
  int b = 0;
#pragma unroll
  for (int k = 1; k < kVoxMaxBatch; ++k) b += (k < vb.B && (long long)i >= vb.off[k]) ? 1 : 0;
  int cx, cy, cz;
  const bool ok = voxel_of_point(points + (size_t)i * C, g.vx, g.vy, g.vz, g.x0, g.y0, g.z0, g.gx, g.gy, g.gz, cx, cy, cz);
  reinterpret_cast<int4*>(coors4)[i] = ok ? make_int4(b, cz, cy, cx) : make_int4(b, -1, -1, -1);
  if (ok && cz < D) {
    const unsigned long long cell = (((unsigned long long)b * D + cz) * g.gy + cy) * g.gx + cx;
    fine[cell] = 1;
    coarse[cell >> 6] = 1;
  }
}

static int occ_bytemaps_ensure(Arena& a, const OccIndex& occ, hipStream_t st, size_t* alloc_words_out) {
  ByteMaps& bm = a.bytemaps;
  const size_t alloc_words = round_up(occ.nwords, kWordsPerBlock);
  *alloc_words_out = alloc_words;
  if (bm.words < alloc_words) {
    ISF_HIP_TRY(hipStreamSynchronize(st));
    if (bm.fine) { ISF_HIP_TRY(hipFree(bm.fine)); ISF_HIP_TRY(hipFree(bm.coarse)); bm = ByteMaps(); }
    if (hipMalloc(&bm.fine, alloc_words * 64) != hipSuccess || hipMalloc(&bm.coarse, alloc_words) != hipSuccess) {
      (void)hipGetLastError();
      set_error("occupancy byte maps: hipMalloc(%zu) failed", alloc_words * 65);
      return ISF_ERR_NOMEM;
    }
    ISF_HIP_TRY(hipMemsetAsync(bm.fine, 0, alloc_words * 64, st));
    ISF_HIP_TRY(hipMemsetAsync(bm.coarse, 0, alloc_words, st));
    bm.words = alloc_words;
  }
  return ISF_OK;
}

int occ_voxelize_mark_bytemap(Arena& a, const OccIndex& occ, const float* points, int P, int C, const VoxGeom& g,
                              const VoxBatch& vb, int32_t* coors4, hipStream_t st) {
  ISF_REQUIRE(vb.B >= 1 && vb.B <= kVoxMaxBatch && vb.B == occ.B && g.gy == occ.H && g.gx == occ.W && g.gz <= occ.D,
              ISF_ERR_ARG, "voxelize + mark: %d frames, grid %d x %d x %d vs index %d x %d x %d", vb.B, g.gz, g.gy, g.gx,
              occ.D, occ.H, occ.W);
  size_t alloc_words = 0;
  ISF_TRY(occ_bytemaps_ensure(a, occ, st, &alloc_words));
  ByteMaps& bm = a.bytemaps;
  if (P > 0)
    hipLaunchKernelGGL(occ_voxelize_mark_kernel, dim3(ceil_div(P, 256)), dim3(256), 0, st, points, P, C, g, vb, occ.D, coors4,
                       bm.fine, bm.coarse);
  hipLaunchKernelGGL(occ_bytemap_pack_kernel, dim3(ceil_div((long long)(alloc_words / 4), 256)), dim3(256), 0, st,
                     bm.fine, bm.coarse, alloc_words, occ.bits);
  ISF_LAUNCH_CHECK();
  return ISF_OK;
}

int occ_mark_coords4_bytemap(Arena& a, const OccIndex& occ, const int32_t* coors4, int n, hipStream_t st) {
  ByteMaps& bm = a.bytemaps;
  const size_t alloc_words = round_up(occ.nwords, kWordsPerBlock);
  if (bm.words < alloc_words) {
    ISF_HIP_TRY(hipStreamSynchronize(st));
    if (bm.fine) { ISF_HIP_TRY(hipFree(bm.fine)); ISF_HIP_TRY(hipFree(bm.coarse)); bm = ByteMaps(); }
    if (hipMalloc(&bm.fine, alloc_words * 64) != hipSuccess || hipMalloc(&bm.coarse, alloc_words) != hipSuccess) {
      (void)hipGetLastError();
      set_error("occupancy byte maps: hipMalloc(%zu) failed", alloc_words * 65);
      return ISF_ERR_NOMEM;
    }
    ISF_HIP_TRY(hipMemsetAsync(bm.fine, 0, alloc_words * 64, st));
    ISF_HIP_TRY(hipMemsetAsync(bm.coarse, 0, alloc_words, st));
    bm.words = alloc_words;
  }
  if (n > 0)
    hipLaunchKernelGGL(occ_bytemap_mark_kernel, dim3(ceil_div(n, 256)), dim3(256), 0, st, coors4, n, occ.B, occ.D,
                       occ.H, occ.W, bm.fine, bm.coarse);
  hipLaunchKernelGGL(occ_bytemap_pack_kernel, dim3(ceil_div((long long)(alloc_words / 4), 256)), dim3(256), 0, st,
                     bm.fine, bm.coarse, alloc_words, occ.bits);
  ISF_LAUNCH_CHECK();
  return ISF_OK;
}

struct FillJobs {
  unsigned long long* ptr[4];
  unsigned long long words[4];
  unsigned long long value[4];
  unsigned long long first[5];
};
__global__ __launch_bounds__(256) void fill_many_kernel(FillJobs j) {
  const unsigned long long total = j.first[4];
  for (unsigned long long i = (unsigned long long)blockIdx.x * blockDim.x + threadIdx.x; i < total;
       i += (unsigned long long)gridDim.x * blockDim.x) {
    int k = 0;
#pragma unroll
    for (int q = 1; q < 4; ++q) k += i >= j.first[q] ? 1 : 0;
    j.ptr[k][i - j.first[k]] = j.value[k];
  }
}

int fill_many(hipStream_t st, int n, void* const* ptrs, const size_t* bytes, const unsigned char* byte_values) {
  ISF_REQUIRE(n >= 1 && n <= 4, ISF_ERR_ARG, "fill_many: %d jobs (1..4)", n);
  FillJobs j;
  unsigned long long at = 0;
  for (int k = 0; k < 4; ++k) {
    const bool on = k < n && bytes[k] > 0;
    j.ptr[k] = on ? reinterpret_cast<unsigned long long*>(ptrs[k]) : nullptr;
    j.words[k] = on ? (bytes[k] + 7) / 8 : 0;
    j.value[k] = on ? 0x0101010101010101ull * byte_values[k] : 0;
    j.first[k] = at;
    at += j.words[k];
  }
  j.first[4] = at;
  if (at == 0) return ISF_OK;
  const unsigned long long blocks = (at + 256 * 8 - 1) / (256 * 8);
  hipLaunchKernelGGL(fill_many_kernel, dim3((unsigned)(blocks < 4096 ? blocks : 4096)), dim3(256), 0, st, j);
  ISF_LAUNCH_CHECK();
  return ISF_OK;
}

int occ_scan(Arena& a, const OccIndex& occ, hipStream_t st) {
  const int nblocks = ceil_div((long long)occ.nwords, kWordsPerBlock);
  uint32_t* sums = nullptr;
  ISF_TRY(a.alloc_n(&sums, (size_t)nblocks + 1));
  hipLaunchKernelGGL(occ_block_count_kernel, dim3(nblocks), dim3(kScanThreads), 0, st, occ.bits,
                     occ.nwords, sums);
  if (nblocks <= kLookBehindBlocks) {
    hipLaunchKernelGGL(occ_write_prefix_kernel<true>, dim3(nblocks), dim3(kScanThreads), 0, st, occ.bits, occ.nwords, sums,
                       occ.prefix, occ.total);
  } else {
    hipLaunchKernelGGL(occ_scan_sums_kernel, dim3(1), dim3(1024), 0, st, sums, nblocks, occ.total);
    hipLaunchKernelGGL(occ_write_prefix_kernel<false>, dim3(nblocks), dim3(kScanThreads), 0, st, occ.bits, occ.nwords, sums,
                       occ.prefix, occ.total);
  }
  ISF_LAUNCH_CHECK();
  return ISF_OK;
}

__global__ __launch_bounds__(kScanThreads) void scan_u32_block_kernel(const uint32_t* __restrict__ in, size_t n,
                                                                      uint32_t* __restrict__ block_sums) {
  __shared__ uint32_t lds[kScanThreads / 64];
  const size_t i0 = (size_t)blockIdx.x * kWordsPerBlock + (size_t)threadIdx.x * kWordsPerThread;
  uint32_t c = 0;
#pragma unroll
  for (int i = 0; i < kWordsPerThread; ++i)
    if (i0 + i < n) c += in[i0 + i];
  uint32_t tot;
  (void)block_exclusive_scan(c, lds, &tot);
  if (threadIdx.x == 0) block_sums[blockIdx.x] = tot;
}

template <bool SUMS>
__global__ __launch_bounds__(kScanThreads) void scan_u32_write_kernel(const uint32_t* __restrict__ in, size_t n,
                                                                      const uint32_t* __restrict__ block_offsets,
                                                                      uint32_t* __restrict__ out) {
  __shared__ uint32_t lds[kScanThreads / 64];
  const size_t i0 = (size_t)blockIdx.x * kWordsPerBlock + (size_t)threadIdx.x * kWordsPerThread;
  uint32_t v[kWordsPerThread];
#pragma unroll
  for (int i = 0; i < kWordsPerThread; ++i) v[i] = (i0 + i < n) ? in[i0 + i] : 0;
  uint32_t tot;
  const uint32_t base = SUMS ? scan_look_behind(block_offsets, lds) : block_offsets[blockIdx.x];
  uint32_t ex = block_exclusive_scan(v[0] + v[1] + v[2] + v[3], lds, &tot) + base;
#pragma unroll
  for (int i = 0; i < kWordsPerThread; ++i) {
    if (i0 + i < n) out[i0 + i] = ex;
    ex += v[i];
    if (i0 + i + 1 == n) out[n] = ex;
  }
}

int scan_u32_exclusive(Arena& a, const uint32_t* in, uint32_t* out, size_t n, hipStream_t st) {
  if (n == 0) {
    ISF_HIP_TRY(hipMemsetAsync(out, 0, sizeof(uint32_t), st));
    return ISF_OK;
  }
  const int nblocks = ceil_div((long long)n, kWordsPerBlock);
  uint32_t* sums = nullptr;
  int* total = nullptr;
  ISF_TRY(a.alloc_n(&sums, (size_t)nblocks + 1));
  ISF_TRY(a.alloc_n(&total, 64));
  hipLaunchKernelGGL(scan_u32_block_kernel, dim3(nblocks), dim3(kScanThreads), 0, st, in, n, sums);
  if (nblocks <= kLookBehindBlocks) {
    hipLaunchKernelGGL(scan_u32_write_kernel<true>, dim3(nblocks), dim3(kScanThreads), 0, st, in, n, sums, out);
  } else {
    hipLaunchKernelGGL(occ_scan_sums_kernel, dim3(1), dim3(1024), 0, st, sums, nblocks, total);
    hipLaunchKernelGGL(scan_u32_write_kernel<false>, dim3(nblocks), dim3(kScanThreads), 0, st, in, n, sums, out);
  }
  ISF_LAUNCH_CHECK();
  return ISF_OK;
}

__global__ void occ_mark_coords4_kernel(unsigned long long* __restrict__ bits,
                                        const int32_t* __restrict__ coors4, int n, int B, int D, int H,
                                        int W) {
  const int i = blockIdx.x * blockDim.x + threadIdx.x;
  if (i >= n) return;
  const int4 c = reinterpret_cast<const int4*>(coors4)[i];
  if (c.x < 0 || c.y < 0 || c.z < 0 || c.w < 0 || c.x >= B || c.y >= D || c.z >= H || c.w >= W) return;
  const unsigned long long cell = (((unsigned long long)c.x * D + c.y) * H + c.z) * W + c.w;
  const unsigned long long bit = 1ull << (cell & 63);
  unsigned long long* p = bits + (cell >> 6);
  if (!(__builtin_nontemporal_load(p) & bit)) atomicOr(p, bit);
}

int occ_mark_coords4(const OccIndex& occ, const int32_t* coors4, int n, hipStream_t st) {
  if (n <= 0) return ISF_OK;
  hipLaunchKernelGGL(occ_mark_coords4_kernel, dim3(ceil_div(n, 256)), dim3(256), 0, st, occ.bits,
                     coors4, n, occ.B, occ.D, occ.H, occ.W);
  ISF_LAUNCH_CHECK();
  return ISF_OK;
}

__global__ void occ_compact_coords4_kernel(const unsigned long long* __restrict__ bits,
                                           const uint32_t* __restrict__ prefix, size_t nwords, int D,
                                           int H, int W, int32_t* __restrict__ out) {
// ... 102 lines not shown
```

is-fusion_amd/csrc/isf_vfe.hip:

```cpp
#include "isf_common.h"

namespace isf {

typedef _Float16 h8 __attribute__((ext_vector_type(8)));
typedef float f32x4 __attribute__((ext_vector_type(4)));
typedef float f32x8 __attribute__((ext_vector_type(8)));

static constexpr int kC = 64;
static constexpr int kL1Threads = 128;
static constexpr double kFix = 16777216.0;

struct VfeGeom {
  float vx, vy, vz, ox, oy, oz;
};

__device__ __forceinline__ void vfe_split2(float x0, float x1, uint32_t& hi, uint32_t& lo) {
  asm("v_cvt_pk_f16_f32 %0, %2, %3\n\t"
      "v_fma_mixlo_f16 %1, %0, -1.0, %2 op_sel_hi:[1,0,0]\n\t"
      "v_fma_mixhi_f16 %1, %0, -1.0, %3 op_sel:[1,0,0] op_sel_hi:[1,0,0]"
      : "=&v"(hi), "=&v"(lo)
      : "v"(x0), "v"(x1));
}

__device__ __forceinline__ void vfe_split8(const f32x8 v, uint4& hi, uint4& lo) {
// ... 12 lines not shown
                                uint4* __restrict__ w2p, float* __restrict__ sc2) {
  __shared__ float amax_s;
  __shared__ float amax1_s;
  const int t = threadIdx.x;
  {
    float m1 = 0.f;
    for (int i = t; i < kC * F; i += 256) m1 = fmaxf(m1, fabsf(w1[i]));
#pragma unroll
    for (int d = 32; d >= 1; d >>= 1) m1 = fmaxf(m1, __shfl_xor(m1, d, 64));
    if (t == 0) amax1_s = 0.f;
    __syncthreads();
    if ((t & 63) == 0) atomicMax(reinterpret_cast<unsigned*>(&amax1_s), __float_as_uint(m1));
    __syncthreads();
    int e1 = 0;
    if (amax1_s > 0.f) (void)frexpf(amax1_s, &e1);
    const int sw1 = amax1_s > 0.f ? 13 - e1 : 0;
    const float s1 = ldexpf(1.f, sw1), inv1 = ldexpf(1.f, -sw1);
    if (t < kC) sc1[t] = scale1[t] * inv1;
    for (int i = t; i < 4 * 64; i += 256) {
      const int lane = i & 63, nt = i >> 6;
      _Float16 hi[4], lo[4];
#pragma unroll
      for (int jj = 0; jj < 4; ++jj) {
        const int k = 4 * (lane >> 4) + jj;
        const float x = k < F ? w1[(size_t)(16 * nt + (lane & 15)) * F + k] * s1 : 0.f;
        hi[jj] = (_Float16)x;
        lo[jj] = (_Float16)(x - (float)hi[jj]);
      }
      w1p[(nt * 2 + 0) * 64 + lane] = *reinterpret_cast<const uint2*>(hi);
      w1p[(nt * 2 + 1) * 64 + lane] = *reinterpret_cast<const uint2*>(lo);
    }
  }
  float m = 0.f;
  for (int i = t; i < kC * 2 * kC; i += 256) m = fmaxf(m, fabsf(w2[i]));
#pragma unroll
  for (int d = 32; d >= 1; d >>= 1) m = fmaxf(m, __shfl_xor(m, d, 64));
  if (t == 0) amax_s = 0.f;
  __syncthreads();
  if ((t & 63) == 0) atomicMax(reinterpret_cast<unsigned*>(&amax_s), __float_as_uint(m));
  __syncthreads();
  const float amax = amax_s;
  int e = 0;
  if (amax > 0.f) (void)frexpf(amax, &e);
  const int sw = amax > 0.f ? 13 - e : 0;
  const float s = ldexpf(1.f, sw), inv = ldexpf(1.f, -sw);
  if (t < kC) sc2[t] = scale2[t] * inv;
  for (int i = t; i < 4 * 4 * 64; i += 256) {
    const int lane = i & 63, nt = (i >> 6) & 3, kc = i >> 8;
    f32x8 v;
#pragma unroll
    for (int jj = 0; jj < 8; ++jj)
      v[jj] = w2[(size_t)(16 * nt + (lane & 15)) * (2 * kC) + vfe_k2(kc, lane >> 4, jj)] * s;
    uint4 hi, lo;
    vfe_split8(v, hi, lo);
    w2p[(size_t)(kc * 4 + nt) * 128 + lane] = hi;
    w2p[(size_t)(kc * 4 + nt) * 128 + 64 + lane] = lo;
  }
}

__global__ __launch_bounds__(256) void vfe_count_kernel(const int32_t* __restrict__ coors4, int P, int D,
                                                        int H, int W,
                                                        const unsigned long long* __restrict__ bits,
                                                        const uint32_t* __restrict__ prefix,
                                                        int32_t* __restrict__ pt2vox,
                                                        int32_t* __restrict__ slot,
                                                        uint32_t* __restrict__ cnt,
                                                        int32_t* __restrict__ voxel_coors) {
  const int i = blockIdx.x * blockDim.x + threadIdx.x;
  if (i >= P) return;
  const int4 c = reinterpret_cast<const int4*>(coors4)[i];
  int v = -1;
  if (c.y >= 0 && c.z >= 0 && c.w >= 0)
    v = occ_lookup(bits, prefix, (((unsigned long long)c.x * D + c.y) * H + c.z) * W + c.w);
  pt2vox[i] = v;
  if (v >= 0) {
    const uint32_t s = atomicAdd(&cnt[v], 1u);
    slot[i] = (int32_t)s;
    if (s == 0) reinterpret_cast<int4*>(voxel_coors)[v] = c;
  }
}

static constexpr int kRec = 8;
template <int CIN>
__global__ __launch_bounds__(256) void vfe_order_kernel(const float* __restrict__ points,
                                                        const int32_t* __restrict__ pt2vox,
                                                        const int32_t* __restrict__ slot, int P,
                                                        const uint32_t* __restrict__ start,
                                                        float* __restrict__ recs) {
  static_assert(CIN + 1 <= kRec, "record too small");
  const int i = blockIdx.x * blockDim.x + threadIdx.x;
  if (i >= P) return;
  const int v = pt2vox[i];
  if (v < 0) return;
  float r[kRec];
#pragma unroll
  for (int k = 0; k < kRec; ++k) r[k] = 0.f;
#pragma unroll
  for (int k = 0; k < CIN; ++k) r[k] = points[(size_t)i * CIN + k];
  r[kRec - 1] = __int_as_float(v);
  float4* o = reinterpret_cast<float4*>(recs + (size_t)(start[v] + slot[i]) * kRec);
  o[0] = make_float4(r[0], r[1], r[2], r[3]);
  o[1] = make_float4(r[4], r[5], r[6], r[7]);
}

template <int CIN>
__global__ __launch_bounds__(256) void vfe_mean_kernel(const float* __restrict__ recs,
                                                       const uint32_t* __restrict__ start, int N,
                                                       float4* __restrict__ mean4) {
  const int lane = threadIdx.x & 63;
  const long long j0 = ((long long)blockIdx.x * 4 + (threadIdx.x >> 6)) * 64;
  const long long nv = start[N];
  if (j0 >= nv) return;
  auto load = [&](long long j, int& v, long long& sx, long long& sy, long long& sz) {
    v = -1;
    sx = sy = sz = 0;
    if (j < nv) {
      const float4 a = reinterpret_cast<const float4*>(recs + (size_t)j * kRec)[0];
      v = __float_as_int(recs[(size_t)j * kRec + kRec - 1]);
      sx = __double2ll_rn((double)a.x * kFix);
      sy = __double2ll_rn((double)a.y * kFix);
      sz = __double2ll_rn((double)a.z * kFix);
    }
  };
  auto write = [&](int v, long long sx, long long sy, long long sz) {
    const uint32_t cnt = start[v + 1] - start[v];
    const double d = kFix * (double)cnt;
    mean4[v] = make_float4((float)((double)sx / d), (float)((double)sy / d), (float)((double)sz / d), (float)cnt);
  };
  int v;
  long long sx, sy, sz;
  load(j0 + lane, v, sx, sy, sz);
  const int vprev = j0 > 0 ? __float_as_int(recs[(size_t)(j0 - 1) * kRec + kRec - 1]) : -1;
  const int vnext = j0 + 64 < nv ? __float_as_int(recs[(size_t)(j0 + 64) * kRec + kRec - 1]) : -1;
#pragma unroll
  for (int d = 1; d < 64; d <<= 1) {
    const int ov = __shfl_up(v, d, 64);
    const long long ox = __shfl_up(sx, d, 64), oy = __shfl_up(sy, d, 64), oz = __shfl_up(sz, d, 64);
    if (lane >= d && ov == v) {
      sx += ox;
      sy += oy;
      sz += oz;
    }
  }
  const int v0 = __builtin_amdgcn_readlane(v, 0), v63 = __builtin_amdgcn_readlane(v, 63);
  const int vn = __shfl_down(v, 1, 64);
  const bool end = v >= 0 && (lane == 63 || vn != v);
  const bool owned = !(v == v0 && vprev == v0);
  const bool leaves = lane == 63 && v >= 0 && vnext == v;
  if (end && owned && !leaves) write(v, sx, sy, sz);
  const bool follow = v63 >= 0 && vnext == v63 && !(v63 == v0 && vprev == v0);
  if (!follow) return;
  long long tx = __shfl(sx, 63, 64), ty = __shfl(sy, 63, 64), tz = __shfl(sz, 63, 64);
  for (long long j = j0 + 64; j < nv; j += 64) {
    int w;
    long long ax, ay, az;
    load(j + lane, w, ax, ay, az);
    if (w != v63) ax = ay = az = 0;
#pragma unroll
    for (int d = 32; d >= 1; d >>= 1) {
      ax += __shfl_xor(ax, d, 64);
      ay += __shfl_xor(ay, d, 64);
      az += __shfl_xor(az, d, 64);
    }
    tx += ax;
    ty += ay;
    tz += az;
    if (__builtin_amdgcn_readlane(w, 63) != v63) break;
  }
  if (lane == 0) write(v63, tx, ty, tz);
}

template <int CIN>
__device__ __forceinline__ void vfe_point_features(const float* __restrict__ p, int4 c, float4 mean, VfeGeom g,
                                                   float (&f)[CIN + 6]) {
#pragma unroll
  for (int k = 0; k < CIN; ++k) f[k] = p[k];
  f[CIN + 0] = __fsub_rn(p[0], mean.x);
  f[CIN + 1] = __fsub_rn(p[1], mean.y);
  f[CIN + 2] = __fsub_rn(p[2], mean.z);
  f[CIN + 3] = __fsub_rn(p[0], __fadd_rn(__fmul_rn((float)c.w, g.vx), g.ox));
  f[CIN + 4] = __fsub_rn(p[1], __fadd_rn(__fmul_rn((float)c.z, g.vy), g.oy));
// ... 294 lines not shown

    f32x4 acc[4][4];
#pragma unroll
    for (int pg = 0; pg < 4; ++pg)
#pragma unroll
      for (int ct = 0; ct < 4; ++ct) acc[pg][ct] = f32x4{0.f, 0.f, 0.f, 0.f};

    auto chunk = [&](int c, const uint4 (&bh)[4], const uint4 (&bl)[4]) {
#pragma unroll
      for (int ct = 0; ct < 4; ++ct) {
        const uint4 ahu = w2s[((c * 4 + ct) * 2 + 0) * 64 + lane];
        const uint4 alu = w2s[((c * 4 + ct) * 2 + 1) * 64 + lane];
        const h8 a_h = *reinterpret_cast<const h8*>(&ahu);
        const h8 a_l = *reinterpret_cast<const h8*>(&alu);
#pragma unroll
        for (int pg = 0; pg < 4; ++pg) {
          const h8 b_h = *reinterpret_cast<const h8*>(&bh[pg]);
          const h8 b_l = *reinterpret_cast<const h8*>(&bl[pg]);
          acc[pg][ct] = __builtin_amdgcn_mfma_f32_16x16x32_f16(a_h, b_l, acc[pg][ct], 0, 0, 0);
          acc[pg][ct] = __builtin_amdgcn_mfma_f32_16x16x32_f16(a_l, b_h, acc[pg][ct], 0, 0, 0);
          acc[pg][ct] = __builtin_amdgcn_mfma_f32_16x16x32_f16(a_h, b_h, acc[pg][ct], 0, 0, 0);
        }
      }
    };
#pragma unroll
    for (int c = 0; c < 2; ++c) {
      uint4 bh[4], bl[4];
#pragma unroll
      for (int pg = 0; pg < 4; ++pg) {
        f32x4 c1[2];
        vfe_layer1_pair(stage, pg, lane, w1, c, c1);
        const f32x4 a = bn.relu(c1[0], 2 * c), b = bn.relu(c1[1], 2 * c + 1);
        vfe_split8(f32x8{a[0], a[1], a[2], a[3], b[0], b[1], b[2], b[3]}, bh[pg], bl[pg]);
      }
      chunk(c, bh, bl);
    }
    __builtin_amdgcn_sched_barrier(0);
    int vrow = rn.row();
    asm volatile("" : "+v"(vrow));
    const int vn = rn.live ? vrow : -1;
    const int4 cn = reinterpret_cast<const int4*>(voxel_coors)[vrow];
    const float4 mn = mean4[vrow];
    {
      f32x8 vm3[4];
      vmax_rows(1, vm3);
      __builtin_amdgcn_sched_barrier(0);
      uint4 bh[4], bl[4];
#pragma unroll
      for (int pg = 0; pg < 4; ++pg) vfe_split8(vm2[pg], bh[pg], bl[pg]);
      chunk(2, bh, bl);
#pragma unroll
      for (int pg = 0; pg < 4; ++pg) vfe_split8(vm3[pg], bh[pg], bl[pg]);
      chunk(3, bh, bl);
    }
    __builtin_amdgcn_sched_barrier(0);
    __builtin_amdgcn_fence(__ATOMIC_RELEASE, "wavefront");
    asm volatile("" : "+v"(rn.a.x), "+v"(rn.a.y), "+v"(rn.a.z), "+v"(rn.a.w), "+v"(rn.b.x));
    vfe_stage_record<CIN>(rn, cn, mn, g, stage, lane);

    vfe_segmented_max(v, vfe_record_voxel(recs, (long long)j0 - 1, nv), vfe_record_voxel(recs, (long long)j0 + 64, nv),
                      lane, out,
                      [&](int pg) {
                        switch (pg) {
                          case 0: vfe_store_tile(acc[0], ftile, lane); break;
                          case 1: vfe_store_tile(acc[1], ftile, lane); break;
                          case 2: vfe_store_tile(acc[2], ftile, lane); break;
                          default: vfe_store_tile(acc[3], ftile, lane); break;
                        }
                      },
                      [&](int p) { return fmaxf(fmaf(ftile[(p % kTilePts) * kTileStride + lane], sc, sh), 0.f); },
                      out_split);
    if (!more) break;
    __builtin_amdgcn_fence(__ATOMIC_RELEASE, "wavefront");
    v = vn;
    j0 = jn;
  }
}

template <int CIN>
static int vfe_run(Arena& a, const float* points, const int32_t* coors4, int P, int B, const int grid[3],
                   VfeGeom g, const float* w1, const float* scale1, const float* shift1, const float* w2,
                   const float* scale2, const float* shift2, float* voxel_feats, int32_t* voxel_coors,
                   int32_t* pt2vox_out, int* n_host, OccIndex* occ_out, int d_alloc, hipStream_t st,
                   hipEvent_t* coords_ready, void* voxel_feats_split, const VoxBatch* voxelize, const VoxGeom* vgeom) {
  const int F = CIN + 6;
  OccIndex occ;
  ISF_TRY(occ_create(a, &occ, B, d_alloc > grid[2] ? d_alloc : grid[2], grid[1], grid[0], st, false));
  if (voxelize)
    ISF_TRY(occ_voxelize_mark_bytemap(a, occ, points, P, CIN, *vgeom, *voxelize, const_cast<int32_t*>(coors4), st));
  else
    ISF_TRY(occ_mark_coords4_bytemap(a, occ, coors4, P, st));
  ISF_TRY(occ_scan(a, occ, st));
  float *sc1, *sc2;
  uint2* w1p;
  uint4* w2p;
  ISF_TRY(a.alloc_n(&sc1, (size_t)kC));
  ISF_TRY(a.alloc_n(&sc2, (size_t)kC));
  ISF_TRY(a.alloc_n(&w1p, (size_t)4 * 2 * 64));
  ISF_TRY(a.alloc_n(&w2p, (size_t)4 * 4 * 128));
  hipStream_t sprep = nullptr;
  ISF_TRY(side_stream(a, &sprep));
  ISF_TRY(stream_wait_stream(a, sprep, st));
  hipLaunchKernelGGL(vfe_prep_kernel, dim3(1), dim3(256), 0, sprep, w1, F, w2, scale1, scale2, w1p, sc1, w2p, sc2);
  hipEvent_t prep_done;
  ISF_TRY(pooled_event(a, &prep_done));
  ISF_HIP_TRY(hipEventRecord(prep_done, sprep));
  int N = 0;
  unsigned n_ticket = 0;
  ISF_TRY(post_int(a, occ.total, st, &n_ticket));
  int32_t* pt2vox = pt2vox_out;
  if (!pt2vox) ISF_TRY(a.alloc_n(&pt2vox, (size_t)P));
  int32_t* slot;
  float* recs;
  uint32_t *cnt, *start;
  float4* mean4;
  float* vmax1;
  ISF_TRY(a.alloc_n(&slot, (size_t)P));
  ISF_TRY(a.alloc_n(&recs, (size_t)P * kRec));
  ISF_TRY(a.alloc_n(&cnt, (size_t)P + 1));
  ISF_HIP_TRY(hipMemsetAsync(cnt, 0, ((size_t)P + 1) * sizeof(uint32_t), st));
  hipLaunchKernelGGL(vfe_count_kernel, dim3(ceil_div(P, 256)), dim3(256), 0, st, coors4, P, occ.D, occ.H, occ.W,
                     occ.bits, occ.prefix, pt2vox, slot, cnt, voxel_coors);
  ISF_LAUNCH_CHECK();
  if (coords_ready) {
    ISF_TRY(pooled_event(a, coords_ready));
    ISF_HIP_TRY(hipEventRecord(*coords_ready, st));
  }
  ISF_TRY(wait_int(a, n_ticket, st, &N));
  *n_host = N;
  if (occ_out) *occ_out = occ;
  ISF_HIP_TRY(hipStreamWaitEvent(st, prep_done, 0));
  if (N == 0) return ISF_OK;
  ISF_TRY(a.alloc_n(&start, (size_t)N + 2));
  ISF_TRY(a.alloc_n(&mean4, (size_t)N));
  ISF_TRY(a.alloc_n(&vmax1, (size_t)N * kC));
  ISF_TRY(scan_u32_exclusive(a, cnt, start, (size_t)N, st));
  hipLaunchKernelGGL(vfe_order_kernel<CIN>, dim3(ceil_div(P, 256)), dim3(256), 0, st, points, pt2vox, slot, P, start,
                     recs);
  hipLaunchKernelGGL(vfe_mean_kernel<CIN>, dim3(ceil_div(P, 256)), dim3(256), 0, st, recs, start, N, mean4);
  const int* n_valid = reinterpret_cast<const int*>(start + N);
  static_assert(kRec == 8 && kC == 64, "vfe_zero_cut_rows_kernel indexes records / rows with these sizes");
  hipLaunchKernelGGL(vfe_zero_cut_rows_kernel, dim3(ceil_div(ceil_div(P, 64), 4)), dim3(256), 0, st, recs, n_valid, vmax1,
                     voxel_feats);
  hipLaunchKernelGGL(vfe_layer1_kernel<CIN>, dim3(ceil_div(P, kL1Threads)), dim3(kL1Threads), 0, st, recs,
                     voxel_coors, n_valid, mean4, g, w1p, sc1, shift1, vmax1);
  {
    static bool lds_set[2] = {false, false};
    if (!lds_set[CIN - 4]) {
      ISF_HIP_TRY(hipFuncSetAttribute(reinterpret_cast<const void*>(&vfe_layer2_kernel<CIN>),
                                      hipFuncAttributeMaxDynamicSharedMemorySize, kL2Lds));
      lds_set[CIN - 4] = true;
    }
    const int tiles = ceil_div(P, 64 * kL2Waves);
    hipLaunchKernelGGL(vfe_layer2_kernel<CIN>, dim3(tiles < 512 ? tiles : 512), dim3(64 * kL2Waves), kL2Lds, st, recs,
                       voxel_coors, n_valid, mean4, g, w1p, sc1, shift1, vmax1, w2p, sc2, shift2, voxel_feats,
                       reinterpret_cast<_Float16*>(voxel_feats_split));
  }
  if (voxel_feats_split)
    hipLaunchKernelGGL(vfe_cut_rows_split_kernel, dim3(ceil_div(ceil_div(P, 64), 4)), dim3(256), 0, st, recs, n_valid,
                       voxel_feats, reinterpret_cast<_Float16*>(voxel_feats_split));
  ISF_LAUNCH_CHECK();
  return ISF_OK;
}

int dynamic_vfe_impl(Arena& a, const float* points, const int32_t* coors4, int P, int Cin, int B,
                     const float vs[3], const float range[6], const float* w1, const float* scale1,
                     const float* shift1, int c1, const float* w2, const float* scale2,
                     const float* shift2, int c2, float* voxel_feats, int32_t* voxel_coors,
                     int32_t* pt2vox, int* num_voxels_host, OccIndex* occ_out, int grid_d_alloc,
                     hipStream_t st, hipEvent_t* coords_ready, void* voxel_feats_split, const VoxBatch* voxelize) {
  ISF_REQUIRE(c1 == kC && c2 == kC, ISF_ERR_UNSUPPORTED,
              "dynamic_vfe: feat_channels (%d,%d) not built; this build has (64,64)", c1, c2);
  ISF_REQUIRE(Cin == 4 || Cin == 5, ISF_ERR_UNSUPPORTED, "dynamic_vfe: in_channels %d not built (4|5)", Cin);
  *num_voxels_host = 0;
  if (P <= 0) return ISF_OK;
  int grid[3];
  for (int j = 0; j < 3; ++j) grid[j] = (int)roundf((range[3 + j] - range[j]) / vs[j]);
  VfeGeom g;
  g.vx = vs[0]; g.vy = vs[1]; g.vz = vs[2];
  g.ox = vs[0] / 2 + range[0]; g.oy = vs[1] / 2 + range[1]; g.oz = vs[2] / 2 + range[2];
  const VoxGeom vg = make_geom(vs, range);
  if (Cin == 5)
    return vfe_run<5>(a, points, coors4, P, B, grid, g, w1, scale1, shift1, w2, scale2, shift2,
                      voxel_feats, voxel_coors, pt2vox, num_voxels_host, occ_out, grid_d_alloc, st, coords_ready,
                      voxel_feats_split, voxelize, &vg);
  return vfe_run<4>(a, points, coors4, P, B, grid, g, w1, scale1, shift1, w2, scale2, shift2, voxel_feats,
                    voxel_coors, pt2vox, num_voxels_host, occ_out, grid_d_alloc, st, coords_ready, voxel_feats_split,
                    voxelize, &vg);
}

}

extern "C" {

int isf_dynamic_vfe_forward(const float* points, const int32_t* coors4, int num_points, int in_channels,
                            int batch_size, const float voxel_size_host[3],
                            const float coors_range_host[6], const float* w1, const float* scale1,
                            const float* shift1, int c1, const float* w2, const float* scale2,
                            const float* shift2, int c2, float* voxel_feats, int32_t* voxel_coors,
                            int32_t* pt2vox, int* num_voxels_host, isf_stream_t stream) {
  ISF_REQUIRE(num_points >= 0 && batch_size > 0 && num_voxels_host && voxel_size_host && coors_range_host,
              ISF_ERR_ARG, "dynamic_vfe_forward: bad arguments");
  ISF_REQUIRE(num_points == 0 || (points && coors4 && w1 && scale1 && shift1 && w2 && scale2 && shift2 &&
                                  voxel_feats && voxel_coors),
              ISF_ERR_ARG, "dynamic_vfe_forward: null pointer");
  isf::Arena& a = isf::arena_for_stream(isf::as_stream(stream));
  ISF_TRY(a.reset());
  return isf::dynamic_vfe_impl(a, points, coors4, num_points, in_channels, batch_size, voxel_size_host,
                               coors_range_host, w1, scale1, shift1, c1, w2, scale2, shift2, c2,
                               voxel_feats, voxel_coors, pt2vox, num_voxels_host, nullptr, 0,
                               isf::as_stream(stream));
}

}
```

is-fusion_amd/lidar_branch.py:

```python
import ctypes

import torch
from torch import nn

from . import _lib
from .norm import fold_bn
from .sparse_encoder import SparseEncoder
from .voxel_encoder import DynamicVFE

ISFUSION_0075 = dict(
    voxel_size=[0.075, 0.075, 0.2],
    point_cloud_range=[-54.0, -54.0, -5.0, 54.0, 54.0, 3.0],
    pts_voxel_encoder=dict(in_channels=5, feat_channels=[64, 64], with_distance=False, with_cluster_center=True,
                           with_voxel_center=True, norm_cfg=dict(type="naiveSyncBN1d", eps=1e-3, momentum=0.01)),
    pts_middle_encoder=dict(in_channels=64, sparse_shape=[41, 1440, 1440], base_channels=32, output_channels=256,
                            order=("conv", "norm", "act"),
                            encoder_channels=((32, 32, 64), (64, 64, 128), (128, 128, 256), (256, 256)),
                            encoder_paddings=((0, 0, 1), (0, 0, 1), (0, 0, [0, 1, 1]), (0, 0)),
                            block_type="basicblock"),
)


class LidarBranch(nn.Module):

    def __init__(self, voxel_size=None, point_cloud_range=None, pts_voxel_encoder=None, pts_middle_encoder=None):
        super().__init__()
        cfg = ISFUSION_0075
        self.voxel_size = list(voxel_size or cfg["voxel_size"])
        self.point_cloud_range = list(point_cloud_range or cfg["point_cloud_range"])
        ve = dict(pts_voxel_encoder or cfg["pts_voxel_encoder"])
        ve.pop("type", None)
        ve.setdefault("voxel_size", self.voxel_size)
        ve.setdefault("point_cloud_range", self.point_cloud_range)
        me = dict(pts_middle_encoder or cfg["pts_middle_encoder"])
        me.pop("type", None)
        self.pts_voxel_encoder = DynamicVFE(**ve)
        self.pts_middle_encoder = SparseEncoder(**me)
        self.last_stats = None
        self._vfe_cache = None
        self._vfe_key = None

    def randomize_bn_(self, seed=0):
        g = torch.Generator().manual_seed(seed)
        for m in self.modules():
            if isinstance(m, nn.modules.batchnorm._BatchNorm):
                with torch.no_grad():
                    m.running_mean.copy_(torch.randn(m.num_features, generator=g) * 0.1)
                    m.running_var.copy_(torch.rand(m.num_features, generator=g) * 0.5 + 0.75)
                    m.weight.copy_(torch.rand(m.num_features, generator=g) * 0.5 + 0.75)
                    m.bias.copy_(torch.randn(m.num_features, generator=g) * 0.1)
        return self

    def randomize_weights_(self, seed=0, fan_taps=9.0):
        g = torch.Generator().manual_seed(seed)
        from .spconv import SparseConvolution
        for m in self.modules():
            if isinstance(m, SparseConvolution):
                std = (1.0 / (fan_taps * m.in_channels)) ** 0.5
                with torch.no_grad():
                    m.weight.copy_(torch.randn(m.weight.shape, generator=g) * std)
            elif isinstance(m, nn.Linear):
                std = 0.02 if m.in_features < 32 else (1.0 / m.in_features) ** 0.5
                with torch.no_grad():
                    m.weight.copy_(torch.randn(m.weight.shape, generator=g) * std)
        return self

    def freeze(self, flag=True):
        from . import fusion_ops as ops
        self._frozen = bool(flag)
        ops.freeze(self, flag)
        return self

    def _vfe_params(self):
        vfe = self.pts_voxel_encoder
        from .fusion_ops import frozen
        if self._vfe_cache is not None and getattr(self, "_frozen", False) and frozen(self):
            return self._vfe_cache
        key = tuple((p._version, p.data_ptr()) for p in list(vfe.parameters()) + list(vfe.buffers()))
        if self._vfe_cache is not None and self._vfe_key == key:
            return self._vfe_cache
        l1, l2 = vfe.vfe_layers
        s1, b1 = fold_bn(l1.norm)
        s2, b2 = fold_bn(l2.norm)
        w1 = l1.linear.weight.detach().float().contiguous()
        w2 = l2.linear.weight.detach().float().contiguous()
        p = _lib.VfeParams()
        p.in_channels, p.c1, p.c2 = vfe.raw_in_channels, w1.size(0), w2.size(0)
        p.w1, p.scale1, p.shift1 = w1.data_ptr(), s1.data_ptr(), b1.data_ptr()
        p.w2, p.scale2, p.shift2 = w2.data_ptr(), s2.data_ptr(), b2.data_ptr()
        for j in range(3):
            p.voxel_size[j] = float(self.voxel_size[j])
        for j in range(6):
            p.coors_range[j] = float(self.point_cloud_range[j])
        self._vfe_cache = (p, (w1, w2, s1, b1, s2, b2))
        self._vfe_key = key
        return self._vfe_cache

    def forward_train(self, points):
        from .voxelize import dynamic_voxelize_batched
        pts, coors = dynamic_voxelize_batched(points, self.voxel_size, self.point_cloud_range)
        keep = (coors[:, 1:] >= 0).all(1)
        vf, vc = self.pts_voxel_encoder(pts[keep].float(), coors[keep])
        return self.pts_middle_encoder.forward_modules(vf, vc, len(points))[0]

    def forward(self, points, time_layers=False, want_stats=False, precision=0, conv_diag=0, stage_rows=0,
                stage_mask=0, out=None, bev_split=False):
        if self.training:
            return self.forward_train(points)
        with torch.no_grad():
            return self.forward_eval(points, time_layers, want_stats, precision, conv_diag, stage_rows, stage_mask, out,
                                     bev_split)

    def forward_eval(self, points, time_layers=False, want_stats=False, precision=0, conv_diag=0, stage_rows=0,
                     stage_mask=0, out=None, bev_split=False):
        pts = torch.cat(points, dim=0).contiguous().float()
        _lib.require_cuda(pts)
        vfe = self.pts_voxel_encoder
        if pts.size(1) != vfe.raw_in_channels:
            raise _lib.IsfError(f"LidarBranch: points have {pts.size(1)} columns, the voxel encoder expects "
                                f"{vfe.raw_in_channels}")
        if not vfe._fusable():
            raise _lib.IsfError("LidarBranch: the one-call engine implements the IS-Fusion DynamicVFE configuration "
                                "(2 layers of 64, cluster + voxel centre, max pooling, no distance feature); build the "
                                "path from the sub-modules for anything else")
        offs = [0]
        for p in points:
            offs.append(offs[-1] + p.size(0))
        B = len(points)
        me = self.pts_middle_encoder
        arr, n, _keep, _plan = me._c_plan()
        vp, _keep2 = self._vfe_params()
        cd, H, W = me.out_channels_and_shape()
        if out is None:
            out = torch.empty((B, cd, H, W), dtype=torch.float32, device=pts.device)
        assert tuple(out.shape) == (B, cd, H, W) and out.is_contiguous() and out.dtype == torch.float32
        oshape = (ctypes.c_int * 4)()
        stats = _lib.EncoderStats() if (want_stats or time_layers) else None
        lib = _lib.load()
        _lib.check(lib.isf_lidar_branch_forward(
            _lib.ptr(pts), (ctypes.c_int64 * len(offs))(*offs), B, ctypes.byref(vp), _lib.i3(me.sparse_shape),
            arr, n, _lib.ptr(out), oshape, ctypes.byref(stats) if stats is not None else None,
            int(bool(time_layers)), _lib.encoder_options(precision, conv_diag, stage_rows, stage_mask, int(bool(bev_split))),
            _lib.stream()), "isf_lidar_branch_forward")
        self.last_stats = stats
        if bev_split:
            from .dense_conv import SplitMap
            if cd % 256:
                raise _lib.IsfError(f"LidarBranch: bev_split needs whole 256-channel groups, the BEV map has {cd} channels")
            raw = out.view(torch.uint8).view(-1)
            step = B * H * W * 256 * 4
            return [SplitMap(raw[g * step:(g + 1) * step], B, 256, H, W) for g in range(cd // 256)]
        return out

    def conv_layer_table(self):
        plan = self.pts_middle_encoder.export_plan()
        return [(L["kind"], L["c_in"], L["c_out"], L["ksize"][0] * L["ksize"][1] * L["ksize"][2])
                for L in plan["layers"]]
```

Before: 1048 frames/s.

## Read per-frame point buffers directly and zero empty BEV segments early

Adds a per-frame pointer entry point so the LiDAR branch reads each frame's points in place, which removes the host-side torch.cat concatenation copy of 1.2M points. The dense BEV scatter becomes two passes: a kernel zeroes empty output segments, judged from the occupancy bitmap, on a side stream before the last conv layer, and the scatter kernel then skips wholly empty segments. Occupancy scan block sums are now produced during marking, and a count buffer is reused so one memset goes away. The cost is more complex indexing (frame lookup per point) and a dependency on bitmap alignment logic for correctness.

New measurement: 1061 frames/s, median of 6. 1.01x the previous value.

```diff
diff --git a/include/isf_hip.h b/include/isf_hip.h
--- a/include/isf_hip.h
+++ b/include/isf_hip.h
@@ -268,6 +268,7 @@
 #define ISF_ENC_DIAG_SORT_KEY_AB 134217728
 #define ISF_ENC_DIAG_NARROW_TILES 268435456
 #define ISF_ENC_DIAG_CHUNK_SPLIT 536870912
+#define ISF_ENC_DIAG_BEV_ONE_PASS (1 << 30)
 typedef struct isf_encoder_options {
   int precision;
   int diagnostic;
@@ -296,6 +297,13 @@
                              float* spatial_features, int out_shape_host[4],
                              isf_encoder_stats* stats_host, int time_layers,
                              const isf_encoder_options* options , isf_stream_t stream);
+
+int isf_lidar_branch_forward_frames(const float* const* frame_points_host, const int64_t* point_offsets_host, int batch_size,
+                                    const isf_vfe_params* vfe_host, const int sparse_shape_host[3],
+                                    const isf_conv_layer* layers_host, int num_layers,
+                                    float* spatial_features, int out_shape_host[4],
+                                    isf_encoder_stats* stats_host, int time_layers,
+                                    const isf_encoder_options* options , isf_stream_t stream);
 
 
 size_t isf_packed_linear_bytes(int out_features, int in_features);
diff --git a/is-fusion_amd/_lib.py b/is-fusion_amd/_lib.py
--- a/is-fusion_amd/_lib.py
+++ b/is-fusion_amd/_lib.py
@@ -134,6 +134,7 @@
 ENC_DIAG_ONE_BLOCK_4W, ENC_DIAG_ONE_BLOCK_8W, ENC_DIAG_STAGGER, ENC_DIAG_R4_ISSUE = 262144, 524288, 1048576, 2097152
 ENC_DIAG_TWO_AHEAD, ENC_DIAG_DEEP, ENC_DIAG_BAND_ORDER, ENC_DIAG_NO_ROW_SORT = 4194304, 8388608, 16777216, 33554432
 ENC_DIAG_NARROW_ROW_SORT, ENC_DIAG_SORT_KEY_AB, ENC_DIAG_NARROW_TILES, ENC_DIAG_CHUNK_SPLIT = 67108864, 134217728, 268435456, 536870912
+BEV_ONE_PASS_DIAG = 1 << 30
 WGRAD_F16, WGRAD_FULL_TAPS = 1, 2
 
 
@@ -248,6 +249,10 @@
                                          ctypes.POINTER(VfeParams), _I3, ctypes.POINTER(ConvLayer), c_int,
                                          c_void_p, _I4, ctypes.POINTER(EncoderStats), c_int,
                                          ctypes.POINTER(EncoderOptions), c_void_p]),
+    "isf_lidar_branch_forward_frames": (c_int, [ctypes.POINTER(c_void_p), ctypes.POINTER(ctypes.c_int64), c_int,
+                                                ctypes.POINTER(VfeParams), _I3, ctypes.POINTER(ConvLayer), c_int,
+                                                c_void_p, _I4, ctypes.POINTER(EncoderStats), c_int,
+                                                ctypes.POINTER(EncoderOptions), c_void_p]),
     "isf_packed_linear_bytes": (ctypes.c_size_t, [c_int, c_int]),
     "isf_pack_linear": (c_int, [c_void_p, c_int, c_int, c_void_p, c_void_p]),
     "isf_pack_linear_transposed": (c_int, [c_void_p, c_int, c_int, c_void_p, c_void_p]),
diff --git a/is-fusion_amd/csrc/isf_common.h b/is-fusion_amd/csrc/isf_common.h
--- a/is-fusion_amd/csrc/isf_common.h
+++ b/is-fusion_amd/csrc/isf_common.h
@@ -86,9 +86,11 @@
 
 int occ_create(Arena& a, OccIndex* occ, int B, int D, int H, int W, hipStream_t st, bool zero = true);
 size_t occ_bits_bytes(const OccIndex& occ);
-int occ_mark_coords4_bytemap(Arena& a, const OccIndex& occ, const int32_t* coors4, int n, hipStream_t st);
+int occ_mark_coords4_bytemap(Arena& a, const OccIndex& occ, const int32_t* coors4, int n, hipStream_t st,
+                             uint32_t* block_sums = nullptr );
 int scan_u32_exclusive(Arena& a, const uint32_t* in, uint32_t* out, size_t n, hipStream_t st);
-int occ_scan(Arena& a, const OccIndex& occ, hipStream_t st);
+int occ_scan(Arena& a, const OccIndex& occ, hipStream_t st, uint32_t* block_sums = nullptr, uint32_t* clear = nullptr);
+int occ_scan_block_sums(Arena& a, const OccIndex& occ, uint32_t** sums);
 int occ_mark_coords4(const OccIndex& occ, const int32_t* coors4, int n, hipStream_t st);
 int occ_compact_coords4(const OccIndex& occ, int32_t* out, hipStream_t st);
 int fill_many(hipStream_t st, int n, void* const* ptrs, const size_t* bytes, const unsigned char* byte_values);
@@ -172,10 +174,37 @@
 static constexpr int kVoxMaxBatch = 8;
 struct VoxBatch {
   long long off[kVoxMaxBatch + 1];
+  const float* base[kVoxMaxBatch];
   int B;
 };
-int occ_voxelize_mark_bytemap(Arena& a, const OccIndex& occ, const float* points, int P, int C, const VoxGeom& g,
-                              const VoxBatch& vb, int32_t* coors4, hipStream_t st);
+struct VoxFrame {
+  const float* base;
+  long long first, end;
+  int b;
+};
+__device__ __forceinline__ VoxFrame vox_frame(const VoxBatch& vb, long long i) {
+  VoxFrame f = {vb.base[0], vb.off[0], vb.off[1], 0};
+#pragma unroll
+  for (int k = 1; k < kVoxMaxBatch; ++k)
+    if (k < vb.B && i >= vb.off[k])
+      f = VoxFrame{vb.base[k], vb.off[k], vb.off[k + 1], k};
+  return f;
+}
+__device__ __forceinline__ const float* vox_point(const VoxBatch& vb, long long i, int C, int& b) {
+  VoxFrame f = vox_frame(vb, (long long)blockIdx.x * blockDim.x);
+  if (i >= f.end) f = vox_frame(vb, i);
+  b = f.b;
+  return f.base + (size_t)(i - f.first) * C;
+}
+static inline VoxBatch vox_one_block(const float* points, long long P) {
+  VoxBatch vb = {};
+  vb.off[1] = P;
+  vb.base[0] = points;
+  vb.B = 1;
+  return vb;
+}
+int occ_voxelize_mark_bytemap(Arena& a, const OccIndex& occ, int P, int C, const VoxGeom& g, const VoxBatch& vb,
+                              int32_t* coors4, hipStream_t st, uint32_t* block_sums = nullptr );
 
 int dynamic_voxelize_impl(const float* points, int P, int C, const float vs[3], const float range[6],
                           int32_t* coors, int coors_stride, int coors_col0, int batch_idx,
@@ -187,7 +216,8 @@
                      int32_t* pt2vox, int* num_voxels_host, OccIndex* occ_out, int grid_d_alloc,
                      hipStream_t st, hipEvent_t* coords_ready = nullptr,
                      void* voxel_feats_split = nullptr ,
-                     const VoxBatch* voxelize = nullptr );
+                     const VoxBatch* voxelize = nullptr ,
+                     const VoxBatch* frames = nullptr );
 int build_perm(Arena& a, const OccIndex& occ, const int32_t* coors4, int n, int32_t** perm_out,
                hipStream_t st);
 int launch_nbr(Arena& a, const int32_t* out_coors4, int n_out, const int in_shape[3], const int ks[3],
@@ -297,6 +327,7 @@
 int half_to_f32_impl(const void* xh, size_t n_elems, float* x, hipStream_t st);
 int sparse_to_dense_bev_impl(Arena& a, const void* feats, int fmt, const int32_t* indices, int n, int C,
                              int B, int D, int H, int W, float* out, const OccIndex* occ,
-                             hipStream_t st);
-
-}
+                             hipStream_t st,
+                             bool skip_empty = false );
+
+}
diff --git a/is-fusion_amd/csrc/isf_encoder.hip b/is-fusion_amd/csrc/isf_encoder.hip
--- a/is-fusion_amd/csrc/isf_encoder.hip
+++ b/is-fusion_amd/csrc/isf_encoder.hip
@@ -6,8 +6,67 @@
 namespace isf {
 
 static constexpr int kDenseX = 64;
-
-template <int FMT>
+static constexpr int kBevSeg = 32;
+static constexpr int kBevZeroBlocks = 256;
+
+__device__ __forceinline__ int bev_plane_shift(const float* out, size_t plane0) {
+  return (int)(((reinterpret_cast<uintptr_t>(out) >> 2) + plane0) & (kBevSeg - 1));
+}
+
+__device__ __forceinline__ bool bev_segment_empty(const unsigned long long* __restrict__ bits,
+                                                  unsigned long long plane_cell0, int HW, int shift, int k) {
+  const int lo = kBevSeg * k - shift < 0 ? 0 : kBevSeg * k - shift;
+  const int hi = kBevSeg * k - shift + kBevSeg > HW ? HW : kBevSeg * k - shift + kBevSeg;
+  if (lo >= hi) return false;
+  const unsigned long long cell0 = plane_cell0 + lo;
+  const int len = hi - lo;
+  const size_t w = (size_t)(cell0 >> 6);
+  const int s = (int)(cell0 & 63);
+  unsigned long long m = bits[w] >> s;
+  if (s + len > 64) m |= bits[w + 1] << (64 - s);
+  m &= (1ull << len) - 1;
+  return m == 0;
+}
+
+__global__ __launch_bounds__(256) void bev_zero_empty_kernel(int B, int C, int D, int HW,
+                                                             const unsigned long long* __restrict__ bits,
+                                                             float* __restrict__ out) {
+  const int lane = threadIdx.x & 63, wv = threadIdx.x >> 6;
+  const int groups = ((HW + 2 * kBevSeg - 2) / kBevSeg + 7) / 8;
+  const long long units = (long long)B * D * groups;
+  const bool vec_ok = ((size_t)D * HW) % 4 == 0;
+  for (long long u = blockIdx.x; u < units; u += gridDim.x) {
+    const int g = (int)(u % groups);
+    const long long bz = u / groups;
+    const int z = (int)(bz % D);
+    const size_t plane0 = ((size_t)(bz / D) * C * D + z) * HW;
+    const int shift = bev_plane_shift(out, plane0);
+    const int k = g * 8 + (lane >> 3);
+    const int p0 = kBevSeg * k - shift + 4 * (lane & 7);
+    if (p0 + 4 <= 0 || p0 >= HW) continue;
+    if (!bev_segment_empty(bits, (unsigned long long)bz * HW, HW, shift, k)) continue;
+    const bool whole = vec_ok && p0 >= 0 && p0 + 4 <= HW;
+    for (int c = wv; c < C; c += 4) {
+      float* o = out + plane0 + (size_t)c * D * HW;
+      if (whole) {
+        *reinterpret_cast<float4*>(o + p0) = make_float4(0.f, 0.f, 0.f, 0.f);
+      } else {
+#pragma unroll
+        for (int e = 0; e < 4; ++e)
+          if (p0 + e >= 0 && p0 + e < HW) o[p0 + e] = 0.f;
+      }
+    }
+  }
+}
+
+static int bev_zero_empty_impl(const OccIndex& occ, int C, float* out, hipStream_t st) {
+  hipLaunchKernelGGL(bev_zero_empty_kernel, dim3(kBevZeroBlocks), dim3(256), 0, st, occ.B, C, occ.D, occ.H * occ.W, occ.bits,
+                     out);
+  ISF_LAUNCH_CHECK();
+  return ISF_OK;
+}
+
+template <int FMT, bool SKIP = false>
 __global__ __launch_bounds__(256) void dense_bev_kernel(const void* __restrict__ feats_v, int C, int D,
                                                         int H, int W,
                                                         const unsigned long long* __restrict__ bits,
@@ -16,6 +75,7 @@
                                                         float* __restrict__ out) {
   __shared__ float tile[64][kDenseX + 1];
   __shared__ int rows[kDenseX];
+  __shared__ int keep[kDenseX + 1];
   const int xt = blockIdx.x, y = blockIdx.y, b = blockIdx.z;
   const int x0 = xt * kDenseX;
   const int t = threadIdx.x;
@@ -23,14 +83,25 @@
     __syncthreads();
     if (t < kDenseX) {
       int r = -1;
+      bool kp = false;
       const int x = x0 + t;
       if (x < W) {
         r = occ_lookup(bits, prefix, (((unsigned long long)b * D + z) * H + y) * W + x);
         if (r >= 0 && perm) r = perm[r];
+        if (SKIP) {
+          const int shift = bev_plane_shift(out, ((size_t)b * C * D + z) * H * W);
+          kp = !bev_segment_empty(bits, ((unsigned long long)b * D + z) * H * W, H * W, shift, (y * W + x + shift) / kBevSeg);
+        }
       }
       rows[t] = r;
+      if (SKIP) {
+        keep[t] = kp;
+        const unsigned long long any = __ballot(kp);
+        if (t == 0) keep[kDenseX] = any != 0;
+      }
     }
     __syncthreads();
+    if (SKIP && !keep[kDenseX]) continue;
     for (int c0 = 0; c0 < C; c0 += 64) {
       if (FMT != 0) {
         const uint4* fs = reinterpret_cast<const uint4*>(feats_v);
@@ -68,7 +139,7 @@
       }
       __syncthreads();
       const int lane = t & 63, wv = t >> 6;
-      if (x0 + lane < W) {
+      if (x0 + lane < W && !(SKIP && !keep[lane])) {
         for (int cc = wv; cc < 64 && c0 + cc < C; cc += 4) {
           const size_t ch = (size_t)(c0 + cc) * D + z;
           out[(((size_t)b * C * D + ch) * H + y) * W + x0 + lane] = tile[cc][lane];
@@ -80,7 +151,8 @@
 }
 
 int sparse_to_dense_bev_impl(Arena& a, const void* feats, int fmt, const int32_t* indices, int n, int C,
-                             int B, int D, int H, int W, float* out, const OccIndex* occ_in, hipStream_t st) {
+                             int B, int D, int H, int W, float* out, const OccIndex* occ_in, hipStream_t st,
+                             bool skip_empty ) {
   ISF_REQUIRE(C % (fmt ? 32 : 4) == 0, ISF_ERR_UNSUPPORTED, "dense: channels %d not a multiple of %d", C,
               fmt ? 32 : 4);
   OccIndex occ;
@@ -96,7 +168,12 @@
     perm = p;
   }
   dim3 grid(ceil_div(W, kDenseX), H, B);
-  if (fmt == 1)
+  ISF_REQUIRE(!skip_empty || (fmt == 1 && occ_in && (long long)H * W < (1ll << 30)), ISF_ERR_ARG,
+              "dense: two passes need split rows + index");
+  if (fmt == 1 && skip_empty)
+    hipLaunchKernelGGL((dense_bev_kernel<1, true>), grid, dim3(256), 0, st, feats, C, D, H, W, occ.bits, occ.prefix,
+                       perm, out);
+  else if (fmt == 1)
     hipLaunchKernelGGL(dense_bev_kernel<1>, grid, dim3(256), 0, st, feats, C, D, H, W, occ.bits, occ.prefix,
                        perm, out);
   else if (fmt == 2)
@@ -332,7 +409,8 @@
     ISF_ENC_DIAG_STAGGER | ISF_ENC_DIAG_R4_ISSUE | ISF_ENC_DIAG_TWO_AHEAD | ISF_ENC_DIAG_DEEP | ISF_ENC_DIAG_NARROW_TILES |
     ISF_ENC_DIAG_LAUNCH_ORDER | ISF_ENC_DIAG_NARROW_GATHER | ISF_ENC_DIAG_CU_KERNEL | ISF_ENC_DIAG_CU_VARIANT_MASK |
     ISF_ENC_DIAG_DENSE_TABLES | ISF_ENC_DIAG_TILE_TABLES | ISF_ENC_DIAG_COUNTS_MEMCPY | ISF_ENC_DIAG_BAND_ORDER | ISF_ENC_DIAG_NO_ROW_SORT |
-    ISF_ENC_DIAG_NARROW_ROW_SORT | ISF_ENC_DIAG_SORT_KEY_AB | ISF_ENC_DIAG_VFE_FP32_ROWS | ISF_ENC_DIAG_VOXELIZE_PER_FRAME;
+    ISF_ENC_DIAG_NARROW_ROW_SORT | ISF_ENC_DIAG_SORT_KEY_AB | ISF_ENC_DIAG_VFE_FP32_ROWS | ISF_ENC_DIAG_VOXELIZE_PER_FRAME |
+    ISF_ENC_DIAG_BEV_ONE_PASS;
 
 int sparse_encoder_forward_impl(Arena& a, const float* x0, const int32_t* coors0, int n0, int B,
                                 const int shape0[3], const OccIndex* occ0, const isf_conv_layer* layers,
@@ -390,6 +468,9 @@
   bool use16 = precision != 1;
   for (int i = 0; i < num_layers; ++i)
     use16 = use16 && layers[i].packed16 && sparse_conv_f16x3_supported(layers[i].c_in, layers[i].c_out);
+  const bool bev_two_pass = !on(ISF_ENC_DIAG_BEV_ONE_PASS) && use16 && !f16io && (!opt || opt->bev_format == 0) &&
+                            spatial_features != nullptr;
+  bool bev_zeroed = false;
   const void* outputs[32];
   int out_rows[32];
   const void* x = x0;
@@ -651,6 +732,11 @@
       L = Nx;
       ISF_TRY(stream_wait_stream(a, st, sg));
     }
+    if (bev_two_pass && i == num_layers - 1 && (long long)L.shape[1] * L.shape[2] < (1ll << 30)) {
+      ISF_TRY(ensure_occ(a, L, B, sg));
+      ISF_TRY(bev_zero_empty_impl(L.occ, ly.c_out, spatial_features, sg));
+      bev_zeroed = true;
+    }
     void* y = nullptr;
     ISF_TRY(a.alloc(&y, (size_t)std::max(n_out, 1) * ly.c_out * 4));
     const void* res = nullptr;
@@ -704,7 +790,7 @@
     ISF_REQUIRE(!opt || opt->bev_format == 0, ISF_ERR_ARG, "sparse_encoder: bev_format %d (0 fp32 map, 1 split token matrices)",
                 opt->bev_format);
     ISF_TRY(sparse_to_dense_bev_impl(a, x, use16 ? (f16io ? 2 : 1) : 0, L.coors, L.n, c_last, B, L.shape[0], L.shape[1],
-                                     L.shape[2], spatial_features, &L.occ, st));
+                                     L.shape[2], spatial_features, &L.occ, st, bev_zeroed));
   }
   if (stats) stats->precision = use16 ? 1 : 0;
   if (out_shape) { out_shape[0] = c_last * L.shape[0]; out_shape[1] = L.shape[1]; out_shape[2] = L.shape[2]; out_shape[3] = L.n; }
@@ -794,15 +880,12 @@
   return true;
 }
 
-int isf_lidar_branch_forward(const float* points, const int64_t* point_offsets_host, int batch_size,
-                             const isf_vfe_params* vfe_host, const int sparse_shape_host[3],
+static int lidar_branch_impl(const float* points, const float* const* frame_points, const int64_t* point_offsets_host,
+                             int batch_size, const isf_vfe_params* vfe_host, const int sparse_shape_host[3],
                              const isf_conv_layer* layers_host, int num_layers, float* spatial_features,
                              int out_shape_host[4], isf_encoder_stats* stats_host, int time_layers,
                              const isf_encoder_options* options, isf_stream_t stream) {
   using namespace isf;
-  ISF_REQUIRE(points && point_offsets_host && batch_size > 0 && vfe_host && sparse_shape_host && layers_host &&
-                  spatial_features,
-              ISF_ERR_ARG, "lidar_branch_forward: bad arguments");
   hipStream_t st = as_stream(stream);
   Arena& a = arena_for_stream(as_stream(stream));
   ISF_TRY(a.reset());
@@ -812,19 +895,23 @@
   const int Cin = vfe_host->in_channels;
   int32_t* coors4 = nullptr;
   ISF_TRY(a.alloc_n(&coors4, (size_t)P * 4));
-  VoxBatch vb;
-  vb.B = batch_size;
-  const bool fused_vox = batch_size <= kVoxMaxBatch && !(options && (options->diagnostic & ISF_ENC_DIAG_VOXELIZE_PER_FRAME));
+  const bool table = batch_size <= kVoxMaxBatch;
+  VoxBatch vb = table ? VoxBatch() : vox_one_block(points, P);
+  if (table) vb.B = batch_size;
+  const bool fused_vox = table && !(options && (options->diagnostic & ISF_ENC_DIAG_VOXELIZE_PER_FRAME));
   for (int b = 0; b < batch_size; ++b) {
     const int64_t lo = point_offsets_host[b], hi = point_offsets_host[b + 1];
     ISF_REQUIRE(hi >= lo, ISF_ERR_ARG, "lidar_branch_forward: bad offsets");
-    if (fused_vox) {
+    const float* base = frame_points ? frame_points[b] : points + lo * Cin;
+    ISF_REQUIRE(base || hi == lo, ISF_ERR_ARG, "lidar_branch_forward: frame %d has no points pointer", b);
+    if (table) {
       vb.off[b] = lo;
       vb.off[b + 1] = hi;
-    } else {
-      ISF_TRY(dynamic_voxelize_impl(points + lo * Cin, (int)(hi - lo), Cin, vfe_host->voxel_size,
-                                    vfe_host->coors_range, coors4 + lo * 4, 4, 1, b, st));
-    }
+      vb.base[b] = base;
+    }
+    if (!fused_vox && hi > lo)
+      ISF_TRY(dynamic_voxelize_impl(base, (int)(hi - lo), Cin, vfe_host->voxel_size, vfe_host->coors_range, coors4 + lo * 4,
+                                    4, 1, b, st));
   }
   float* vf = nullptr;
   int32_t* vc = nullptr;
@@ -837,10 +924,10 @@
   if (encoder_takes_split_input(layers_host, num_layers, options) && vfe_host->c2 == layers_host[0].c_in &&
       !(options && (options->diagnostic & ISF_ENC_DIAG_VFE_FP32_ROWS)))
     ISF_TRY(a.alloc(&vf_split, (size_t)P * vfe_host->c2 * 4));
-  ISF_TRY(dynamic_vfe_impl(a, points, coors4, P, Cin, batch_size, vfe_host->voxel_size, vfe_host->coors_range,
+  ISF_TRY(dynamic_vfe_impl(a, nullptr, coors4, P, Cin, batch_size, vfe_host->voxel_size, vfe_host->coors_range,
                            vfe_host->w1, vfe_host->scale1, vfe_host->shift1, vfe_host->c1, vfe_host->w2,
                            vfe_host->scale2, vfe_host->shift2, vfe_host->c2, vf, vc, nullptr, &n0, &occ0,
-                           sparse_shape_host[0], st, &coords_ready, vf_split, fused_vox ? &vb : nullptr));
+                           sparse_shape_host[0], st, &coords_ready, vf_split, fused_vox ? &vb : nullptr, &vb));
   ISF_REQUIRE(n0 > 0, ISF_ERR_ARG, "lidar_branch_forward: no point falls inside the voxel grid");
   const bool occ_ok = occ0.D == sparse_shape_host[0] && occ0.H == sparse_shape_host[1] &&
                       occ0.W == sparse_shape_host[2];
@@ -849,4 +936,30 @@
                                      time_layers, options, st, occ_ok ? coords_ready : nullptr, vf_split);
 }
 
-}
+int isf_lidar_branch_forward(const float* points, const int64_t* point_offsets_host, int batch_size,
+                             const isf_vfe_params* vfe_host, const int sparse_shape_host[3],
+                             const isf_conv_layer* layers_host, int num_layers, float* spatial_features,
+                             int out_shape_host[4], isf_encoder_stats* stats_host, int time_layers,
+                             const isf_encoder_options* options, isf_stream_t stream) {
+  ISF_REQUIRE(points && point_offsets_host && batch_size > 0 && vfe_host && sparse_shape_host && layers_host &&
+                  spatial_features,
+              ISF_ERR_ARG, "lidar_branch_forward: bad arguments");
+  return lidar_branch_impl(points, nullptr, point_offsets_host, batch_size, vfe_host, sparse_shape_host, layers_host,
+                           num_layers, spatial_features, out_shape_host, stats_host, time_layers, options, stream);
+}
+
+int isf_lidar_branch_forward_frames(const float* const* frame_points_host, const int64_t* point_offsets_host, int batch_size,
+                                    const isf_vfe_params* vfe_host, const int sparse_shape_host[3],
+                                    const isf_conv_layer* layers_host, int num_layers, float* spatial_features,
+                                    int out_shape_host[4], isf_encoder_stats* stats_host, int time_layers,
+                                    const isf_encoder_options* options, isf_stream_t stream) {
+  ISF_REQUIRE(frame_points_host && point_offsets_host && batch_size > 0 && vfe_host && sparse_shape_host && layers_host &&
+                  spatial_features,
+              ISF_ERR_ARG, "lidar_branch_forward_frames: bad arguments");
+  ISF_REQUIRE(batch_size <= isf::kVoxMaxBatch, ISF_ERR_UNSUPPORTED,
+              "lidar_branch_forward_frames: %d frames (at most %d; concatenate larger batches)", batch_size, isf::kVoxMaxBatch);
+  return lidar_branch_impl(nullptr, frame_points_host, point_offsets_host, batch_size, vfe_host, sparse_shape_host,
+                           layers_host, num_layers, spatial_features, out_shape_host, stats_host, time_layers, options, stream);
+}
+
+}
diff --git a/is-fusion_amd/csrc/isf_runtime.hip b/is-fusion_amd/csrc/isf_runtime.hip
--- a/is-fusion_amd/csrc/isf_runtime.hip
+++ b/is-fusion_amd/csrc/isf_runtime.hip
@@ -345,7 +345,8 @@
 template <bool SUMS>
 __global__ __launch_bounds__(kScanThreads) void occ_write_prefix_kernel(
     const unsigned long long* __restrict__ bits, size_t nwords,
-    const uint32_t* __restrict__ block_offsets, uint32_t* __restrict__ prefix, int* __restrict__ total) {
+    const uint32_t* __restrict__ block_offsets, uint32_t* __restrict__ prefix, int* __restrict__ total,
+    uint32_t* __restrict__ clear ) {
   __shared__ uint32_t lds[kScanThreads / 64];
   const size_t w0 = (size_t)blockIdx.x * kWordsPerBlock + (size_t)threadIdx.x * kWordsPerThread;
   uint32_t pc[kWordsPerThread];
@@ -356,6 +357,10 @@
   const uint32_t base = SUMS ? scan_look_behind(block_offsets, lds) : block_offsets[blockIdx.x];
   uint32_t ex = block_exclusive_scan(c, lds, &tot) + base;
   if (SUMS && blockIdx.x == gridDim.x - 1 && threadIdx.x == 0) *total = (int)(base + tot);
+  if (clear) {
+    const uint32_t n = tot + (blockIdx.x == gridDim.x - 1 ? 1u : 0u);
+    for (uint32_t i = threadIdx.x; i < n; i += kScanThreads) clear[base + i] = 0u;
+  }
 #pragma unroll
   for (int i = 0; i < kWordsPerThread; ++i) {
     if (w0 + i < nwords) prefix[w0 + i] = ex;
@@ -394,9 +399,11 @@
 __global__ __launch_bounds__(256) void occ_bytemap_pack_kernel(unsigned char* __restrict__ fine,
                                                                unsigned char* __restrict__ coarse,
                                                                size_t nwords_alloc,
-                                                               unsigned long long* __restrict__ bits) {
+                                                               unsigned long long* __restrict__ bits,
+                                                               uint32_t* __restrict__ block_sums) {
+  static_assert(kWordsPerBlock == 256 * 4, "the pack kernel's workgroup is one scan block");
+  __shared__ uint32_t wave_sums[4];
   const size_t w0 = ((size_t)blockIdx.x * blockDim.x + threadIdx.x) * 4;
-  if (w0 >= nwords_alloc) return;
   const unsigned int c4 = *reinterpret_cast<const unsigned int*>(coarse + w0);
   unsigned long long out[4] = {0ull, 0ull, 0ull, 0ull};
   if (c4) {
@@ -422,19 +429,26 @@
   }
   reinterpret_cast<ulonglong2*>(bits + w0)[0] = make_ulonglong2(out[0], out[1]);
   reinterpret_cast<ulonglong2*>(bits + w0)[1] = make_ulonglong2(out[2], out[3]);
-}
-
-__global__ __launch_bounds__(256) void occ_voxelize_mark_kernel(const float* __restrict__ points, int P, int C, VoxGeom g,
-                                                                VoxBatch vb, int D, int32_t* __restrict__ coors4,
+  if (block_sums) {
+    uint32_t c = __popcll(out[0]) + __popcll(out[1]) + __popcll(out[2]) + __popcll(out[3]);
+#pragma unroll
+    for (int d = 32; d >= 1; d >>= 1) c += __shfl_xor(c, d, 64);
+    if ((threadIdx.x & 63) == 0) wave_sums[threadIdx.x >> 6] = c;
+    __syncthreads();
+    if (threadIdx.x == 0) block_sums[blockIdx.x] = wave_sums[0] + wave_sums[1] + wave_sums[2] + wave_sums[3];
+  }
+}
+
+__global__ __launch_bounds__(256) void occ_voxelize_mark_kernel(int P, int C, VoxGeom g, VoxBatch vb, int D,
+                                                                int32_t* __restrict__ coors4,
                                                                 unsigned char* __restrict__ fine,
                                                                 unsigned char* __restrict__ coarse) {
   const int i = blockIdx.x * blockDim.x + threadIdx.x;
   if (i >= P) return;
-  int b = 0;
-#pragma unroll
-  for (int k = 1; k < kVoxMaxBatch; ++k) b += (k < vb.B && (long long)i >= vb.off[k]) ? 1 : 0;
+  int b;
+  const float* p = vox_point(vb, i, C, b);
   int cx, cy, cz;
-  const bool ok = voxel_of_point(points + (size_t)i * C, g.vx, g.vy, g.vz, g.x0, g.y0, g.z0, g.gx, g.gy, g.gz, cx, cy, cz);
+  const bool ok = voxel_of_point(p, g.vx, g.vy, g.vz, g.x0, g.y0, g.z0, g.gx, g.gy, g.gz, cx, cy, cz);
   reinterpret_cast<int4*>(coors4)[i] = ok ? make_int4(b, cz, cy, cx) : make_int4(b, -1, -1, -1);
   if (ok && cz < D) {
     const unsigned long long cell = (((unsigned long long)b * D + cz) * g.gy + cy) * g.gx + cx;
@@ -462,8 +476,8 @@
   return ISF_OK;
 }
 
-int occ_voxelize_mark_bytemap(Arena& a, const OccIndex& occ, const float* points, int P, int C, const VoxGeom& g,
-                              const VoxBatch& vb, int32_t* coors4, hipStream_t st) {
+int occ_voxelize_mark_bytemap(Arena& a, const OccIndex& occ, int P, int C, const VoxGeom& g, const VoxBatch& vb,
+                              int32_t* coors4, hipStream_t st, uint32_t* block_sums) {
   ISF_REQUIRE(vb.B >= 1 && vb.B <= kVoxMaxBatch && vb.B == occ.B && g.gy == occ.H && g.gx == occ.W && g.gz <= occ.D,
               ISF_ERR_ARG, "voxelize + mark: %d frames, grid %d x %d x %d vs index %d x %d x %d", vb.B, g.gz, g.gy, g.gx,
               occ.D, occ.H, occ.W);
@@ -471,15 +485,16 @@
   ISF_TRY(occ_bytemaps_ensure(a, occ, st, &alloc_words));
   ByteMaps& bm = a.bytemaps;
   if (P > 0)
-    hipLaunchKernelGGL(occ_voxelize_mark_kernel, dim3(ceil_div(P, 256)), dim3(256), 0, st, points, P, C, g, vb, occ.D, coors4,
-                       bm.fine, bm.coarse);
+    hipLaunchKernelGGL(occ_voxelize_mark_kernel, dim3(ceil_div(P, 256)), dim3(256), 0, st, P, C, g, vb, occ.D, coors4, bm.fine,
+                       bm.coarse);
   hipLaunchKernelGGL(occ_bytemap_pack_kernel, dim3(ceil_div((long long)(alloc_words / 4), 256)), dim3(256), 0, st,
-                     bm.fine, bm.coarse, alloc_words, occ.bits);
+                     bm.fine, bm.coarse, alloc_words, occ.bits, block_sums);
   ISF_LAUNCH_CHECK();
   return ISF_OK;
 }
 
-int occ_mark_coords4_bytemap(Arena& a, const OccIndex& occ, const int32_t* coors4, int n, hipStream_t st) {
+int occ_mark_coords4_bytemap(Arena& a, const OccIndex& occ, const int32_t* coors4, int n, hipStream_t st,
+                             uint32_t* block_sums) {
   ByteMaps& bm = a.bytemaps;
   const size_t alloc_words = round_up(occ.nwords, kWordsPerBlock);
   if (bm.words < alloc_words) {
@@ -498,7 +513,7 @@
     hipLaunchKernelGGL(occ_bytemap_mark_kernel, dim3(ceil_div(n, 256)), dim3(256), 0, st, coors4, n, occ.B, occ.D,
                        occ.H, occ.W, bm.fine, bm.coarse);
   hipLaunchKernelGGL(occ_bytemap_pack_kernel, dim3(ceil_div((long long)(alloc_words / 4), 256)), dim3(256), 0, st,
-                     bm.fine, bm.coarse, alloc_words, occ.bits);
+                     bm.fine, bm.coarse, alloc_words, occ.bits, block_sums);
   ISF_LAUNCH_CHECK();
   return ISF_OK;
 }
@@ -540,19 +555,25 @@
   return ISF_OK;
 }
 
-int occ_scan(Arena& a, const OccIndex& occ, hipStream_t st) {
+int occ_scan_block_sums(Arena& a, const OccIndex& occ, uint32_t** sums) {
+  return a.alloc_n(sums, (size_t)ceil_div((long long)occ.nwords, kWordsPerBlock) + 1);
+}
+
+int occ_scan(Arena& a, const OccIndex& occ, hipStream_t st, uint32_t* block_sums, uint32_t* clear) {
   const int nblocks = ceil_div((long long)occ.nwords, kWordsPerBlock);
-  uint32_t* sums = nullptr;
-  ISF_TRY(a.alloc_n(&sums, (size_t)nblocks + 1));
-  hipLaunchKernelGGL(occ_block_count_kernel, dim3(nblocks), dim3(kScanThreads), 0, st, occ.bits,
-                     occ.nwords, sums);
+  uint32_t* sums = block_sums;
+  if (!sums) {
+    ISF_TRY(occ_scan_block_sums(a, occ, &sums));
+    hipLaunchKernelGGL(occ_block_count_kernel, dim3(nblocks), dim3(kScanThreads), 0, st, occ.bits,
+                       occ.nwords, sums);
+  }
   if (nblocks <= kLookBehindBlocks) {
     hipLaunchKernelGGL(occ_write_prefix_kernel<true>, dim3(nblocks), dim3(kScanThreads), 0, st, occ.bits, occ.nwords, sums,
-                       occ.prefix, occ.total);
+                       occ.prefix, occ.total, clear);
   } else {
     hipLaunchKernelGGL(occ_scan_sums_kernel, dim3(1), dim3(1024), 0, st, sums, nblocks, occ.total);
     hipLaunchKernelGGL(occ_write_prefix_kernel<false>, dim3(nblocks), dim3(kScanThreads), 0, st, occ.bits, occ.nwords, sums,
-                       occ.prefix, occ.total);
+                       occ.prefix, occ.total, clear);
   }
   ISF_LAUNCH_CHECK();
   return ISF_OK;
diff --git a/is-fusion_amd/csrc/isf_vfe.hip b/is-fusion_amd/csrc/isf_vfe.hip
--- a/is-fusion_amd/csrc/isf_vfe.hip
+++ b/is-fusion_amd/csrc/isf_vfe.hip
@@ -118,7 +118,7 @@
 
 static constexpr int kRec = 8;
 template <int CIN>
-__global__ __launch_bounds__(256) void vfe_order_kernel(const float* __restrict__ points,
+__global__ __launch_bounds__(256) void vfe_order_kernel(VoxBatch frames ,
                                                         const int32_t* __restrict__ pt2vox,
                                                         const int32_t* __restrict__ slot, int P,
                                                         const uint32_t* __restrict__ start,
@@ -131,8 +131,10 @@
   float r[kRec];
 #pragma unroll
   for (int k = 0; k < kRec; ++k) r[k] = 0.f;
-#pragma unroll
-  for (int k = 0; k < CIN; ++k) r[k] = points[(size_t)i * CIN + k];
+  int b;
+  const float* p = vox_point(frames, i, CIN, b);
+#pragma unroll
+  for (int k = 0; k < CIN; ++k) r[k] = p[k];
   r[kRec - 1] = __int_as_float(v);
   float4* o = reinterpret_cast<float4*>(recs + (size_t)(start[v] + slot[i]) * kRec);
   o[0] = make_float4(r[0], r[1], r[2], r[3]);
@@ -593,15 +595,20 @@
                    VfeGeom g, const float* w1, const float* scale1, const float* shift1, const float* w2,
                    const float* scale2, const float* shift2, float* voxel_feats, int32_t* voxel_coors,
                    int32_t* pt2vox_out, int* n_host, OccIndex* occ_out, int d_alloc, hipStream_t st,
-                   hipEvent_t* coords_ready, void* voxel_feats_split, const VoxBatch* voxelize, const VoxGeom* vgeom) {
+                   hipEvent_t* coords_ready, void* voxel_feats_split, const VoxBatch* voxelize, const VoxGeom* vgeom,
+                   const VoxBatch* frames_in) {
   const int F = CIN + 6;
+  const VoxBatch frames = frames_in ? *frames_in : (voxelize ? *voxelize : vox_one_block(points, P));
   OccIndex occ;
   ISF_TRY(occ_create(a, &occ, B, d_alloc > grid[2] ? d_alloc : grid[2], grid[1], grid[0], st, false));
+  uint32_t *occ_sums = nullptr, *cnt = nullptr;
+  ISF_TRY(occ_scan_block_sums(a, occ, &occ_sums));
+  ISF_TRY(a.alloc_n(&cnt, (size_t)P + 1));
   if (voxelize)
-    ISF_TRY(occ_voxelize_mark_bytemap(a, occ, points, P, CIN, *vgeom, *voxelize, const_cast<int32_t*>(coors4), st));
+    ISF_TRY(occ_voxelize_mark_bytemap(a, occ, P, CIN, *vgeom, *voxelize, const_cast<int32_t*>(coors4), st, occ_sums));
   else
-    ISF_TRY(occ_mark_coords4_bytemap(a, occ, coors4, P, st));
-  ISF_TRY(occ_scan(a, occ, st));
+    ISF_TRY(occ_mark_coords4_bytemap(a, occ, coors4, P, st, occ_sums));
+  ISF_TRY(occ_scan(a, occ, st, occ_sums, cnt));
   float *sc1, *sc2;
   uint2* w1p;
   uint4* w2p;
@@ -623,13 +630,11 @@
   if (!pt2vox) ISF_TRY(a.alloc_n(&pt2vox, (size_t)P));
   int32_t* slot;
   float* recs;
-  uint32_t *cnt, *start;
+  uint32_t* start;
   float4* mean4;
   float* vmax1;
   ISF_TRY(a.alloc_n(&slot, (size_t)P));
   ISF_TRY(a.alloc_n(&recs, (size_t)P * kRec));
-  ISF_TRY(a.alloc_n(&cnt, (size_t)P + 1));
-  ISF_HIP_TRY(hipMemsetAsync(cnt, 0, ((size_t)P + 1) * sizeof(uint32_t), st));
   hipLaunchKernelGGL(vfe_count_kernel, dim3(ceil_div(P, 256)), dim3(256), 0, st, coors4, P, occ.D, occ.H, occ.W,
                      occ.bits, occ.prefix, pt2vox, slot, cnt, voxel_coors);
   ISF_LAUNCH_CHECK();
@@ -646,7 +651,7 @@
   ISF_TRY(a.alloc_n(&mean4, (size_t)N));
   ISF_TRY(a.alloc_n(&vmax1, (size_t)N * kC));
   ISF_TRY(scan_u32_exclusive(a, cnt, start, (size_t)N, st));
-  hipLaunchKernelGGL(vfe_order_kernel<CIN>, dim3(ceil_div(P, 256)), dim3(256), 0, st, points, pt2vox, slot, P, start,
+  hipLaunchKernelGGL(vfe_order_kernel<CIN>, dim3(ceil_div(P, 256)), dim3(256), 0, st, frames, pt2vox, slot, P, start,
                      recs);
   hipLaunchKernelGGL(vfe_mean_kernel<CIN>, dim3(ceil_div(P, 256)), dim3(256), 0, st, recs, start, N, mean4);
   const int* n_valid = reinterpret_cast<const int*>(start + N);
@@ -679,7 +684,8 @@
                      const float* shift1, int c1, const float* w2, const float* scale2,
                      const float* shift2, int c2, float* voxel_feats, int32_t* voxel_coors,
                      int32_t* pt2vox, int* num_voxels_host, OccIndex* occ_out, int grid_d_alloc,
-                     hipStream_t st, hipEvent_t* coords_ready, void* voxel_feats_split, const VoxBatch* voxelize) {
+                     hipStream_t st, hipEvent_t* coords_ready, void* voxel_feats_split, const VoxBatch* voxelize,
+                     const VoxBatch* frames) {
   ISF_REQUIRE(c1 == kC && c2 == kC, ISF_ERR_UNSUPPORTED,
               "dynamic_vfe: feat_channels (%d,%d) not built; this build has (64,64)", c1, c2);
   ISF_REQUIRE(Cin == 4 || Cin == 5, ISF_ERR_UNSUPPORTED, "dynamic_vfe: in_channels %d not built (4|5)", Cin);
@@ -694,10 +700,10 @@
   if (Cin == 5)
     return vfe_run<5>(a, points, coors4, P, B, grid, g, w1, scale1, shift1, w2, scale2, shift2,
                       voxel_feats, voxel_coors, pt2vox, num_voxels_host, occ_out, grid_d_alloc, st, coords_ready,
-                      voxel_feats_split, voxelize, &vg);
+                      voxel_feats_split, voxelize, &vg, frames);
   return vfe_run<4>(a, points, coors4, P, B, grid, g, w1, scale1, shift1, w2, scale2, shift2, voxel_feats,
                     voxel_coors, pt2vox, num_voxels_host, occ_out, grid_d_alloc, st, coords_ready, voxel_feats_split,
-                    voxelize, &vg);
+                    voxelize, &vg, frames);
 }
 
 }
diff --git a/is-fusion_amd/lidar_branch.py b/is-fusion_amd/lidar_branch.py
--- a/is-fusion_amd/lidar_branch.py
+++ b/is-fusion_amd/lidar_branch.py
@@ -104,21 +104,26 @@
         return self.pts_middle_encoder.forward_modules(vf, vc, len(points))[0]
 
     def forward(self, points, time_layers=False, want_stats=False, precision=0, conv_diag=0, stage_rows=0,
-                stage_mask=0, out=None, bev_split=False):
+                stage_mask=0, out=None, bev_split=False, by_pointer=True):
         if self.training:
             return self.forward_train(points)
         with torch.no_grad():
             return self.forward_eval(points, time_layers, want_stats, precision, conv_diag, stage_rows, stage_mask, out,
-                                     bev_split)
+                                     bev_split, by_pointer)
 
     def forward_eval(self, points, time_layers=False, want_stats=False, precision=0, conv_diag=0, stage_rows=0,
-                     stage_mask=0, out=None, bev_split=False):
-        pts = torch.cat(points, dim=0).contiguous().float()
-        _lib.require_cuda(pts)
+                     stage_mask=0, out=None, bev_split=False, by_pointer=True):
         vfe = self.pts_voxel_encoder
-        if pts.size(1) != vfe.raw_in_channels:
-            raise _lib.IsfError(f"LidarBranch: points have {pts.size(1)} columns, the voxel encoder expects "
-                                f"{vfe.raw_in_channels}")
+        dev = points[0].device if len(points) else None
+        by_frame = by_pointer and 1 <= len(points) <= 8 and all(
+            p.is_cuda and p.device == dev and p.dtype == torch.float32 and p.dim() == 2 and
+            p.size(1) == vfe.raw_in_channels and p.is_contiguous() for p in points)
+        pts = None if by_frame else torch.cat(points, dim=0).contiguous().float()
+        if pts is not None:
+            _lib.require_cuda(pts)
+            if pts.size(1) != vfe.raw_in_channels:
+                raise _lib.IsfError(f"LidarBranch: points have {pts.size(1)} columns, the voxel encoder expects "
+                                    f"{vfe.raw_in_channels}")
         if not vfe._fusable():
             raise _lib.IsfError("LidarBranch: the one-call engine implements the IS-Fusion DynamicVFE configuration "
                                 "(2 layers of 64, cluster + voxel centre, max pooling, no distance feature); build the "
@@ -132,16 +137,22 @@
         vp, _keep2 = self._vfe_params()
         cd, H, W = me.out_channels_and_shape()
         if out is None:
-            out = torch.empty((B, cd, H, W), dtype=torch.float32, device=pts.device)
+            out = torch.empty((B, cd, H, W), dtype=torch.float32, device=points[0].device if by_frame else pts.device)
         assert tuple(out.shape) == (B, cd, H, W) and out.is_contiguous() and out.dtype == torch.float32
         oshape = (ctypes.c_int * 4)()
         stats = _lib.EncoderStats() if (want_stats or time_layers) else None
         lib = _lib.load()
-        _lib.check(lib.isf_lidar_branch_forward(
-            _lib.ptr(pts), (ctypes.c_int64 * len(offs))(*offs), B, ctypes.byref(vp), _lib.i3(me.sparse_shape),
+        if by_frame:
+            entry, name = lib.isf_lidar_branch_forward_frames, "isf_lidar_branch_forward_frames"
+            src = (ctypes.c_void_p * B)(*[p.data_ptr() if p.size(0) else None for p in points])
+        else:
+            entry, name = lib.isf_lidar_branch_forward, "isf_lidar_branch_forward"
+            src = _lib.ptr(pts)
+        _lib.check(entry(
+            src, (ctypes.c_int64 * len(offs))(*offs), B, ctypes.byref(vp), _lib.i3(me.sparse_shape),
             arr, n, _lib.ptr(out), oshape, ctypes.byref(stats) if stats is not None else None,
             int(bool(time_layers)), _lib.encoder_options(precision, conv_diag, stage_rows, stage_mask, int(bool(bev_split))),
-            _lib.stream()), "isf_lidar_branch_forward")
+            _lib.stream()), name)
         self.last_stats = stats
         if bev_split:
             from .dense_conv import SplitMap
```
